# victorramirez952/tomography_3d_reconstructor

Measured on NVIDIA B200. Metric: Gvoxels/s mask-stack->mesh+volume, higher is better.
Workload: dtype u8 -> bit-packed u32 (topology), f64 field taps -> f32 vertices

## Files before the change

tomography_3d_reconstructor_b200/csrc/t3d_common.cuh:

```cuda
#pragma once
#include <cuda_runtime.h>
#include <stdint.h>
#include <stdio.h>

int t3d_num_sms(void);
#define T3D_NUM_SMS (t3d_num_sms())
bool t3d_first_use_on_device(int slot);
enum { T3D_ONCE_FILL_HOLES_ATTR = 0, T3D_ONCE_MC_LUTS = 1, T3D_ONCE_SORT_ATTR = 2, T3D_ONCE_MORPH4_ATTR = 3, T3D_ONCE_SLOTS = 8 };

extern "C" void t3d_set_error(const char* fmt, ...);
extern "C" void t3d_count_launches(int n);
int t3d_zero_async(void* p, size_t n, cudaStream_t st);
void t3d_prezero_register(const void* p, size_t n);
void t3d_prezero_clear(void);
void t3d_canonicalize_structured_zero_range(int64_t V, int64_t F, uint32_t cap_z, uint32_t cap_g0, int Zs, int64_t* offset,
                                            int64_t* size);

#define T3D_CHECK_LAUNCH(name)                                                                   \
    do {                                                                                         \
        cudaError_t e__ = cudaGetLastError();                                                    \
        if (e__ != cudaSuccess) {                                                                \
            t3d_set_error("%s: launch failed: %s", name, cudaGetErrorString(e__));               \
            return 1;                                                                            \
        }                                                                                        \
// ... 53 lines not shown
    return v;
}

__device__ __forceinline__ uint4 ld_stream_u4(const void* p)
{
    uint4 r;
    asm volatile("ld.global.nc.L1::no_allocate.v4.u32 {%0,%1,%2,%3}, [%4];"
                 : "=r"(r.x), "=r"(r.y), "=r"(r.z), "=r"(r.w)
                 : "l"(p));
    return r;
}
__device__ __forceinline__ void st_stream_u4(void* p, uint4 v)
{
    asm volatile("st.global.L1::no_allocate.v4.u32 [%0], {%1,%2,%3,%4};" ::"l"(p), "r"(v.x), "r"(v.y),
                 "r"(v.z), "r"(v.w)
                 : "memory");
}

__device__ __forceinline__ uint32_t ge4(uint32_t v, uint32_t thr4)
{
    const uint32_t m = __vcmpgeu4(v, thr4) & 0x80808080u;
    return (m * 0x00204081u) >> 28;
}
__device__ __forceinline__ uint32_t ge16(uint4 v, uint32_t thr4)
{
    return ge4(v.x, thr4) | (ge4(v.y, thr4) << 4) | (ge4(v.z, thr4) << 8) | (ge4(v.w, thr4) << 12);
}
__device__ __forceinline__ uint32_t expand4(uint32_t nib) { return (nib * 0x00204081u) & 0x01010101u; }

__device__ __forceinline__ uint4 and4(uint4 a, uint4 b) { return make_uint4(a.x & b.x, a.y & b.y, a.z & b.z, a.w & b.w); }
__device__ __forceinline__ uint4 or4(uint4 a, uint4 b) { return make_uint4(a.x | b.x, a.y | b.y, a.z | b.z, a.w | b.w); }
__device__ __forceinline__ uint4 splat4(uint32_t v) { return make_uint4(v, v, v, v); }
__device__ __forceinline__ uint32_t popc4(uint4 a) { return __popc(a.x) + __popc(a.y) + __popc(a.z) + __popc(a.w); }
__device__ __forceinline__ uint4 valid_mask4(int w4, int W)
{
    return make_uint4(valid_mask(4 * w4, W), valid_mask(4 * w4 + 1, W), valid_mask(4 * w4 + 2, W), valid_mask(4 * w4 + 3, W));
}
__device__ __forceinline__ uint4 shl1_4(uint4 c, uint32_t l)
{
    return make_uint4(__funnelshift_l(l, c.x, 1), __funnelshift_l(c.x, c.y, 1), __funnelshift_l(c.y, c.z, 1), __funnelshift_l(c.z, c.w, 1));
}
__device__ __forceinline__ uint4 shr1_4(uint4 c, uint32_t r)
{
    return make_uint4(__funnelshift_r(c.x, c.y, 1), __funnelshift_r(c.y, c.z, 1), __funnelshift_r(c.z, c.w, 1), __funnelshift_r(c.w, r, 1));
}

__device__ __forceinline__ int64_t dev_n(int64_t cap, const unsigned long long* p)
{
    if (!p) return cap;
    const unsigned long long v = *p;
    return v < (unsigned long long)cap ? (int64_t)v : cap;
}

int t3d_morph_stage(const uint32_t* in, uint32_t* out, int Z, int H, int W, int z0, int nz, int out_rs, long long out_ps,
                    bool erode, bool ring, int ring_tail, unsigned long long* counts, cudaStream_t st);
bool t3d_morph4_eligible(int Z, int H, int W);
int t3d_morph4_launch(const uint32_t* in, uint32_t* out, int Z, int H, int W, int z0, int nz, int out_rs, long long out_ps, int ring_tail,
                      unsigned long long* counts, cudaStream_t st);
void t3d_canon_faces_ready_event(cudaEvent_t e);
bool t3d_canon_faces_ready_pending();
bool t3d_pack_gap_supported(const void* masks_u8, int Z, int H, int W, int threshold);
int t3d_pack_gap_launch(const void* masks_u8, int Z, int H, int W, int threshold, void* out, unsigned long long* counts,
                        unsigned int* bbox_t, int skip_ends, cudaStream_t st, int z_bias = 0);
int t3d_bbox_t_planes_launch(const uint32_t* bits, int n_planes, int H, int W, int z_bias, unsigned int* bbox_t, cudaStream_t st);
int t3d_close_ends_fixup_launch(const void* masks_u8, int Z, int H, int W, int threshold, const void* filled0, const void* filledT,
                                void* out, unsigned long long* counts, cudaStream_t st);
```

tomography_3d_reconstructor_b200/csrc/t3d_mc.cu:

```cuda
#include "mc_tables.h"
#include "mc33_tables.h"
#include "t3d.h"
#include "t3d_field.cuh"

__device__ __align__(16) const int8_t g_tri_table[256][T3D_MC_ROW] = {T3D_TRI_TABLE_ROWS};
static const int8_t h_tri_table[256][T3D_MC_ROW] = {T3D_TRI_TABLE_ROWS};

struct McLuts {
    uint8_t ntri[256];
};
#define MC_AMB 0x80u
__constant__ McLuts c_luts;

__device__ const int8_t g33_rows[T3D_MC33_NROWS][T3D_MC33_ROW] = {T3D_MC33_TRI_ROWS};
__device__ const uint8_t g33_ntri[T3D_MC33_NROWS] = {T3D_MC33_NTRI_VALUES};
__device__ const uint16_t g33_base[256] = {T3D_MC33_BASE_VALUES};
__device__ const uint8_t g33_k[256] = {T3D_MC33_K_VALUES};
__device__ const uint8_t g33_faces[256][6] = {T3D_MC33_FACES_VALUES};
__device__ const unsigned long long g33_need[256] = {T3D_MC33_NEED_VALUES};
__device__ const uint8_t g33_pol[256] = {T3D_MC33_POL_VALUES};
__device__ const int8_t g33_sign[256] = {T3D_MC33_SIGN_VALUES};
__device__ const uint8_t g33_cyc[6][4] = {T3D_MC33_FACE_CYCLE_VALUES};
static const uint16_t h33_base[256] = {T3D_MC33_BASE_VALUES};

// ... 112 lines not shown
                                                uint32_t n01, uint32_t n10, uint32_t n11, bool hy, bool hz, int w, int Ws,
                                                bool own = true)
{
    WordMasks m;
    hz = hz && own;
    const uint32_t vm = valid_mask(w, Ws), em = valid_mask(w, Ws - 1);
    m.s00 = s00; m.s01 = s01; m.s10 = s10; m.s11 = s11;
    m.a00 = shr1(s00, n00); m.a01 = shr1(s01, n01); m.a10 = shr1(s10, n10); m.a11 = shr1(s11, n11);
    m.X00 = (s00 ^ m.a00) & em;
    m.X01 = hy ? (s01 ^ m.a01) & em : 0u;
    m.X10 = hz ? (s10 ^ m.a10) & em : 0u;
    m.X11 = (hy && hz) ? (s11 ^ m.a11) & em : 0u;
    m.Y0 = hy ? (s00 ^ s01) & vm : 0u;
    m.Y1 = (hy && hz) ? (s10 ^ s11) & vm : 0u;
    m.Z0 = hz ? (s00 ^ s10) & vm : 0u;
    m.Z1 = (hy && hz) ? (s01 ^ s11) & vm : 0u;
    m.act = 0u;
    if (hy && hz) {
        const uint32_t o = s00 | s01 | s10 | s11, a = s00 & s01 & s10 & s11;
        const uint32_t oa = m.a00 | m.a01 | m.a10 | m.a11, aa = m.a00 & m.a01 & m.a10 & m.a11;
        m.act = ((o | oa) & ~(a & aa)) & em;
    }
    return m;
}

__device__ __forceinline__ int cube_case(const WordMasks& m, int b)
{
    return (int)(((m.s00 >> b) & 1u) | (((m.a00 >> b) & 1u) << 1) | (((m.a01 >> b) & 1u) << 2) | (((m.s01 >> b) & 1u) << 3) |
                 (((m.s10 >> b) & 1u) << 4) | (((m.a10 >> b) & 1u) << 5) | (((m.a11 >> b) & 1u) << 6) | (((m.s11 >> b) & 1u) << 7));
}

__device__ __forceinline__ WordMasks load_masks(const Grid& g, uint32_t row, int w, int& z, int& y)
{
    z = (int)(row / (uint32_t)g.Hs);
    y = (int)(row - (uint32_t)z * (uint32_t)g.Hs);
    const bool hy = (y + 1 < g.Hs), hz = (z + 1 < g.Zs), hx = (w + 1 < g.nws);
    const uint32_t* p = g.sign + (int64_t)row * g.nws + w;
    const int64_t dy = g.nws, dz = (int64_t)g.Hs * g.nws;
    const uint32_t s00 = p[0], s01 = hy ? p[dy] : 0u, s10 = hz ? p[dz] : 0u, s11 = (hy && hz) ? p[dz + dy] : 0u;
    uint32_t n00 = 0, n01 = 0, n10 = 0, n11 = 0;
    if (hx) {
        n00 = p[1] & 1u;
        if (hy) n01 = p[dy + 1] & 1u;
        if (hz) n10 = p[dz + 1] & 1u;
        if (hy && hz) n11 = p[dz + dy + 1] & 1u;
    }
    return make_masks(s00, s01, s10, s11, n00, n01, n10, n11, hy, hz, w, g.Ws, z < g.z_end);
}

#define GY 16

__global__ void __launch_bounds__(256, 4) k_mc_flags(Grid g, uint32_t* __restrict__ ballots, int lanes_x, int pz_per_block, int gy)
{
    const int lx = threadIdx.x % lanes_x, pz = threadIdx.x / lanes_x;
    const int nws4 = g.nws >> 2;
    const int w4 = blockIdx.x * lanes_x + lx, z = g.z_begin + blockIdx.z * pz_per_block + pz, y0 = blockIdx.y * gy;
    if (pz >= pz_per_block || w4 >= nws4 || z >= g.Zs || z > g.z_end) return;
    const bool hz = (z + 1 < g.Zs) && (z < g.z_end);
    const bool hx = (4 * w4 + 4 < g.nws);
    const uint4 vm = valid_mask4(w4, g.Ws), em = valid_mask4(w4, g.Ws - 1);
    const uint4 zero = make_uint4(0, 0, 0, 0);
    const uint32_t* p0 = g.sign + ((long long)z * g.Hs + y0) * g.nws + 4 * w4;
    const uint32_t* p1 = p0 + (long long)g.Hs * g.nws;
    uint32_t* pb = ballots + ((long long)z * g.Hs + y0) * g.ncr + (w4 >> 3);
    const uint32_t bshift = (4 * w4) & 31;
    uint4 c0 = *reinterpret_cast<const uint4*>(p0), c1 = hz ? *reinterpret_cast<const uint4*>(p1) : zero;
    uint32_t n0 = hx ? p0[4] : 0u, n1 = (hx && hz) ? p1[4] : 0u;
    const int y1 = min(g.Hs, y0 + gy);
    auto load_row = [&](int y, uint4& d0, uint4& d1, uint32_t& m0, uint32_t& m1) {
        const bool hy = (y < g.Hs);
        d0 = hy ? *reinterpret_cast<const uint4*>(p0) : zero;
        d1 = (hy && hz) ? *reinterpret_cast<const uint4*>(p1) : zero;
        m0 = (hy && hx) ? p0[4] : 0u;
        m1 = (hy && hz && hx) ? p1[4] : 0u;
    };
    uint4 e0, e1; uint32_t q0, q1;
    p0 += g.nws; p1 += g.nws;
    load_row(y0 + 1, e0, e1, q0, q1);
    for (int y = y0; y < y1; ++y) {
        const bool hy = (y + 1 < g.Hs);
        const uint4 d0 = e0, d1 = e1;
        const uint32_t m0 = q0, m1 = q1;
        p0 += g.nws; p1 += g.nws;
        if (y + 1 < y1) load_row(y + 2, e0, e1, q0, q1);
        uint4 f;
        if (hy && hz) {
            const uint32_t un = (n0 ^ n1) | (n0 ^ m0) | (m0 ^ m1);
            uint4 yz, u;
            yz.x = (c0.x ^ d0.x) | (c0.x ^ c1.x); yz.y = (c0.y ^ d0.y) | (c0.y ^ c1.y);
            yz.z = (c0.z ^ d0.z) | (c0.z ^ c1.z); yz.w = (c0.w ^ d0.w) | (c0.w ^ c1.w);
            u.x = yz.x | (d0.x ^ d1.x); u.y = yz.y | (d0.y ^ d1.y); u.z = yz.z | (d0.z ^ d1.z); u.w = yz.w | (d0.w ^ d1.w);
            const uint4 us = shr1_4(u, un), a0 = shr1_4(c0, n0);
            f.x = ((u.x | us.x | (c0.x ^ a0.x)) & em.x) | (yz.x & vm.x);
            f.y = ((u.y | us.y | (c0.y ^ a0.y)) & em.y) | (yz.y & vm.y);
            f.z = ((u.z | us.z | (c0.z ^ a0.z)) & em.z) | (yz.z & vm.z);
            f.w = ((u.w | us.w | (c0.w ^ a0.w)) & em.w) | (yz.w & vm.w);
        } else {
            const uint4 a0 = shr1_4(c0, n0);
            f.x = ((c0.x ^ a0.x) & em.x); f.y = ((c0.y ^ a0.y) & em.y); f.z = ((c0.z ^ a0.z) & em.z); f.w = ((c0.w ^ a0.w) & em.w);
            if (hy) { f.x |= (c0.x ^ d0.x) & vm.x; f.y |= (c0.y ^ d0.y) & vm.y; f.z |= (c0.z ^ d0.z) & vm.z; f.w |= (c0.w ^ d0.w) & vm.w; }
            if (hz) { f.x |= (c0.x ^ c1.x) & vm.x; f.y |= (c0.y ^ c1.y) & vm.y; f.z |= (c0.z ^ c1.z) & vm.z; f.w |= (c0.w ^ c1.w) & vm.w; }
        }
        const uint32_t nib = (f.x ? 1u : 0u) | (f.y ? 2u : 0u) | (f.z ? 4u : 0u) | (f.w ? 8u : 0u);
        if (nib) atomicOr(pb, nib << bshift);
        pb += g.ncr;
        c0 = d0; c1 = d1; n0 = m0; n1 = m1;
    }
}

__global__ void __launch_bounds__(256) k_mc_compact(Grid g, const uint32_t* __restrict__ ballots,
                                                    const uint32_t* __restrict__ chunkbase, int64_t n_chunks,
                                                    uint32_t* __restrict__ aw_idx, uint32_t cap_active)
{
    const int64_t c = (int64_t)blockIdx.x * blockDim.x + threadIdx.x;
    if (c >= n_chunks) return;
    uint32_t bal = ballots[c];
    if (!bal) return;
    uint32_t k = chunkbase[c];
    const uint32_t row = (uint32_t)(c / g.ncr);
    const uint32_t base = row * (uint32_t)g.nws + (uint32_t)((c - (int64_t)row * g.ncr) << 5);
    while (bal) {
        const int b = __ffs(bal) - 1;
        bal &= bal - 1;
        if (k < cap_active) aw_idx[k] = base + b;
        ++k;
    }
}

#define AW_AMB 0x80000000u
#define AW_MASK 0x7fffffffu

template <int AMB>
__global__ void __launch_bounds__(128) k_mc_words(Grid g, McField fld, uint32_t* __restrict__ aw_idx, uint32_t cap_active,
                                                  const unsigned long long* __restrict__ n_active_dev, uint32_t* __restrict__ aw_cnt,
                                                  unsigned long long* __restrict__ n_ambiguous)
{
    const uint32_t n_active = cap_active;
    const int64_t n = dev_n(cap_active, n_active_dev);
    if (!AMB) {
        const uint32_t k = blockIdx.x * blockDim.x + threadIdx.x;
        if ((int64_t)k >= n) return;
        const uint32_t i = aw_idx[k];
        const uint32_t row = i / (uint32_t)g.nws;
        const int w = (int)(i - row * (uint32_t)g.nws);
        int z, y;
        const WordMasks m = load_masks(g, row, w, z, y);
        uint32_t nt = 0, amb = 0;
        for (uint32_t a = m.act; a;) {
            const int b = __ffs(a) - 1;
            a &= a - 1;
            const uint32_t c = c_luts.ntri[cube_case(m, b)];
            nt += c & 0x7fu;
            amb |= c;
        }
        aw_cnt[k] = __popc(m.X00);
        aw_cnt[(int64_t)n_active + k] = __popc(m.Y0);
        aw_cnt[2 * (int64_t)n_active + k] = __popc(m.Z0);
        aw_cnt[3 * (int64_t)n_active + k] = nt;
        if (amb & MC_AMB) aw_idx[k] = i | AW_AMB;
    } else {
        uint32_t na = 0;
        auto fix_word = [&](int64_t k, uint32_t iraw) {
            const uint32_t i = iraw & AW_MASK;
            const uint32_t row = i / (uint32_t)g.nws;
            const int w = (int)(i - row * (uint32_t)g.nws);
            int z, y;
            const WordMasks m = load_masks(g, row, w, z, y);
            int delta = 0;
            for (uint32_t a = m.act; a;) {
                const int b = __ffs(a) - 1;
                a &= a - 1;
                const int cs = cube_case(m, b);
                const uint32_t c = c_luts.ntri[cs];
                if (!(c & MC_AMB)) continue;
                delta += (int)g33_ntri[mc33_resolve(fld, z, y, (w << 5) + b, cs)] - (int)(c & 0x7fu);
                ++na;
            }
            aw_cnt[3 * (int64_t)n_active + k] += (uint32_t)delta;
        };
        const int64_t n4 = ((uintptr_t)aw_idx & 15) ? 0 : (n >> 2), stride = (int64_t)gridDim.x * blockDim.x, t0 = (int64_t)blockIdx.x * blockDim.x + threadIdx.x;
        for (int64_t c = t0; c < n4; c += stride) {
            const uint4 v = reinterpret_cast<const uint4*>(aw_idx)[c];
            if (!((v.x | v.y | v.z | v.w) & AW_AMB)) continue;
            if (v.x & AW_AMB) fix_word(4 * c, v.x);
            if (v.y & AW_AMB) fix_word(4 * c + 1, v.y);
            if (v.z & AW_AMB) fix_word(4 * c + 2, v.z);
            if (v.w & AW_AMB) fix_word(4 * c + 3, v.w);
        }
        for (int64_t k = 4 * n4 + t0; k < n; k += stride) {
            const uint32_t iraw = aw_idx[k];
            if (iraw & AW_AMB) fix_word(k, iraw);
        }
        if (na) atomicAdd(n_ambiguous, (unsigned long long)na);
    }
}

static unsigned amb_grid(uint32_t n) { const unsigned want = (n + 127) / 128, cap = (unsigned)T3D_NUM_SMS * 8; return want < cap ? (want ? want : 1) : cap; }

struct EmitArgs {
    Grid g;
    McField fld;
    const uint32_t* ballots;
    const uint32_t* chunkbase;
    const uint32_t* aw_idx;
    const uint32_t* aw_base;
    uint32_t cap_active;
    const unsigned long long* sizes;
    uint32_t cap_verts, cap_faces;
    unsigned long long* vkeys;
    int32_t* faces;
};

__device__ __forceinline__ uint32_t active_rank(const EmitArgs& a, uint32_t row, int w)
{
    const int64_t c = (int64_t)row * a.g.ncr + (w >> 5);
    return a.chunkbase[c] + __popc(a.ballots[c] & ((1u << (w & 31)) - 1u));
}

__device__ __forceinline__ uint32_t lt_mask(int b) { return b >= 32 ? 0xffffffffu : ((1u << b) - 1u); }

__device__ __forceinline__ unsigned long long vkey(int axis, int z, int y, int x)
{
    return (unsigned long long)axis | ((unsigned long long)x << 2) | ((unsigned long long)y << 22) | ((unsigned long long)z << 42);
}

template <int PARTS, int AMB>
__global__ void __launch_bounds__(128) k_mc_emit(EmitArgs a)
{
    __shared__ __align__(16) int8_t s_tri[256][T3D_MC_ROW];
    __shared__ uint32_t s_base[12][128];
    __shared__ uint32_t s_mask[12][128];
    __shared__ uint32_t s_next[4][128];
    if (AMB == 1) {
        int any = 0;
        uint32_t nw_ = a.cap_active;
        if (a.sizes[0] < nw_) nw_ = (uint32_t)a.sizes[0];
        for (uint32_t k = blockIdx.x * blockDim.x + threadIdx.x; k < nw_; k += gridDim.x * blockDim.x) any |= (int)(a.aw_idx[k] >> 31);
        if (!__syncthreads_or(any)) return;
    }
    if (PARTS & 2) {
        const int4* src = reinterpret_cast<const int4*>(&g_tri_table[0][0]);
        int4* dst = reinterpret_cast<int4*>(&s_tri[0][0]);
        for (int i = threadIdx.x; i < 256; i += blockDim.x) {
            dst[i] = src[i];
            if (c_luts.ntri[i] & MC_AMB) s_tri[i][T3D_MC_ROW - 1] = -2;
        }
        __syncthreads();
    }
    const uint32_t tid = threadIdx.x;
    uint32_t n_words = a.cap_active;
    if (a.sizes[0] < n_words) n_words = (uint32_t)a.sizes[0];
    const uint32_t offY = (uint32_t)a.sizes[1], offZ = (uint32_t)(a.sizes[1] + a.sizes[2]);
    if (a.sizes[1] + a.sizes[2] + a.sizes[3] > a.cap_verts || a.sizes[4] > a.cap_faces) return;
    auto emit_word = [&](const uint32_t k, const uint32_t iraw) {
    const uint32_t i = iraw & AW_MASK;
    const uint32_t row = i / (uint32_t)a.g.nws;
    const int w = (int)(i - row * (uint32_t)a.g.nws);
    int z, y;
    const WordMasks m = load_masks(a.g, row, w, z, y);
    const int64_t NA = a.cap_active;
    const uint32_t bX00 = a.aw_base[k], bY0 = offY + a.aw_base[NA + k], bZ0 = offZ + a.aw_base[2 * NA + k];
    uint32_t pT = a.aw_base[3 * NA + k];
    const int x0 = w << 5;

    if (PARTS & 1) {
        uint32_t id = bX00;
        for (uint32_t q = m.X00; q;) { const int b = __ffs(q) - 1; q &= q - 1; a.vkeys[id++] = vkey(2, z, y, x0 + b); }
        id = bY0;
        for (uint32_t q = m.Y0; q;) { const int b = __ffs(q) - 1; q &= q - 1; a.vkeys[id++] = vkey(1, z, y, x0 + b); }
        id = bZ0;
        for (uint32_t q = m.Z0; q;) { const int b = __ffs(q) - 1; q &= q - 1; a.vkeys[id++] = vkey(0, z, y, x0 + b); }
    }
    if (!(PARTS & 2) || !m.act) return;
    if (AMB == 0 && (iraw & AW_AMB)) return;

    const uint32_t Hs = (uint32_t)a.g.Hs;
    uint32_t bX01 = 0, bX10 = 0, bX11 = 0, bY1 = 0, bZ1 = 0;
    if (m.X01 | m.Z1) {
        const uint32_t r = active_rank(a, row + 1, w);
        bX01 = a.aw_base[r];
        bZ1 = offZ + a.aw_base[2 * NA + r];
// ... 97 lines not shown
    float* verts;
};

template <int AXIS>
__device__ __forceinline__ void vertex_body(const VertexArgs& p, const ZLut& zlut, uint32_t id)
{
    const unsigned long long key = p.vkeys[id];
    const int x = (int)((key >> 2) & 0xfffffu) - p.x_off, y = (int)((key >> 22) & 0xfffffu), z = (int)(key >> 42);
    float fa, fb;
    if (p.field) {
        const int64_t i = ((int64_t)z * p.occ.H + y) * p.occ.W + x;
        fa = p.field[i];
        fb = p.field[i + (AXIS == 0 ? (int64_t)p.occ.H * p.occ.W : AXIS == 1 ? p.occ.W : 1)];
    } else {
        edge_field_values<AXIS>(p.occ, zlut, z, y, x, fa, fb);
    }
    const double va = (double)fa - p.level, vb = (double)fb - p.level;
    const double wa = __ddiv_rn(1.0, __dadd_rn(MC33_EPS, fabs(va)));
    const double wb = __ddiv_rn(1.0, __dadd_rn(MC33_EPS, fabs(vb)));
    const double frac = __ddiv_rn(wb, __dadd_rn(wa, wb));
    double pz = (double)(z + p.z_offset), py = (double)y, px = (double)x;
    if (AXIS == 0) pz = __dadd_rn(pz, frac); else if (AXIS == 1) py = __dadd_rn(py, frac); else px = __dadd_rn(px, frac);
    float fz = __fsub_rn(__double2float_rn(pz), p.shift);
    float fy = __fsub_rn(__double2float_rn(py), p.shift);
    float fx = __fsub_rn(__double2float_rn(px), p.shift);
    if (p.n_cum > 0) {
        if (fz < 0.0f) fz = 0.0f;
        else if (fz >= (float)(p.n_cum - 1)) fz = __double2float_rn(p.cum[p.n_cum - 1]);
        else {
            const float fl = floorf(fz);
            const int lo = (int)fl;
            const float fr = __fsub_rn(fz, fl);
            const int ai = min(lo, p.n_cum - 2);
            fz = __double2float_rn(__dadd_rn(p.cum[lo], __dmul_rn((double)fr, p.adj[ai])));
        }
    }
    if (p.scale_f64) {
        fy = __double2float_rn(__dmul_rn((double)fy, p.mm_y));
        fx = __double2float_rn(__dmul_rn((double)fx, p.mm_x));
    } else {
        fy = __fmul_rn(fy, __double2float_rn(p.mm_y));
        fx = __fmul_rn(fx, __double2float_rn(p.mm_x));
    }
    float* o = p.verts + 3 * (int64_t)id;
    o[0] = fz; o[1] = fy; o[2] = fx;
}

__global__ void __launch_bounds__(128) k_mc_vertices_all(VertexArgs p, const unsigned long long* __restrict__ sizes, uint32_t cap_verts,
                                                         int which)
{
    __shared__ ZLut zlut;
    fill_zlut(p.occ, zlut);
    __syncthreads();
    const unsigned long long nx = sizes[1], ny = sizes[2], nz = sizes[3];
    if (nx + ny + nz > cap_verts) return;
    uint32_t t = blockIdx.x * blockDim.x + threadIdx.x;
    if (which & 1) {
        if (t < nx) { vertex_body<2>(p, zlut, t); return; }
        t -= (uint32_t)nx;
    }
    if (which & 2) {
        if (t < ny) { vertex_body<1>(p, zlut, (uint32_t)nx + t); return; }
        t -= (uint32_t)ny;
    }
    if ((which & 4) && t < nz) vertex_body<0>(p, zlut, (uint32_t)(nx + ny) + t);
}

static int make_grid(Grid& g, const void* sign_bits, int Zs, int Hs, int Ws, int z_begin, int z_end, const char* who)
{
    if (Zs <= 0 || Hs <= 0 || Ws <= 0) { t3d_set_error("%s: empty volume", who); return 2; }
    if (z_end < 0 || z_end > Zs) z_end = Zs;
    if (z_begin < 0 || z_begin >= z_end) { t3d_set_error("%s: empty plane range", who); return 2; }
    g.z_begin = z_begin; g.z_end = z_end;
    g.sign = (const uint32_t*)sign_bits;
    g.Zs = Zs; g.Hs = Hs; g.Ws = Ws; g.nws = t3d_wpr(Ws);
    g.ncr = (g.nws + 31) >> 5;
    g.n_rows = (uint32_t)((int64_t)Zs * Hs);
    g.n_words = (int64_t)Zs * Hs * g.nws;
    if (g.n_words >= ((int64_t)1 << 31)) { t3d_set_error("%s: more than 2^31 words in one device slab", who); return 2; }
    return 0;
}

extern "C" int64_t t3d_mc_num_chunks(int Zs, int Hs, int Ws) { return (int64_t)Zs * Hs * ((t3d_wpr(Ws) + 31) >> 5); }

extern "C" int t3d_mc_flags(const void* sign_bits, int Zs, int Hs, int Ws, int z_begin, int z_end, void* ballots_u32,
                            void* stream)
{
    Grid g;
    if (int rc = make_grid(g, sign_bits, Zs, Hs, Ws, z_begin, z_end, "t3d_mc_flags")) return rc;
    cudaStream_t st = (cudaStream_t)stream;
    if (t3d_zero_async(ballots_u32, sizeof(uint32_t) * (size_t)g.n_rows * g.ncr, st)) return 1;
    const int nws4 = g.nws / 4, lanes_x = nws4 < 256 ? nws4 : 256, pzb = 256 / lanes_x;
    const int nz = (g.z_end < Zs ? g.z_end + 1 : Zs) - g.z_begin;
    dim3 grid((nws4 + lanes_x - 1) / lanes_x, (Hs + GY - 1) / GY, (nz + pzb - 1) / pzb);
    k_mc_flags<<<grid, 256, 0, st>>>(g, (uint32_t*)ballots_u32, lanes_x, pzb, GY);
    T3D_CHECK_LAUNCH("t3d_mc_flags");
    t3d_count_launches(1);
    return 0;
}

static int mc_words_dev_impl(const McField& fld, const void* sign_bits, int Zs, int Hs, int Ws, int z_begin, int z_end,
                             const void* ballots_u32, const void* chunkbase_u32, uint32_t cap_active, const void* sizes_u64,
                             void* aw_idx_u32, void* aw_cnt_u32, void* n_ambiguous_u64, void* stream)
{
    Grid g;
    if (int rc = make_grid(g, sign_bits, Zs, Hs, Ws, z_begin, z_end, "t3d_mc_words_dev")) return rc;
    if (ensure_luts()) return 1;
    cudaStream_t st = (cudaStream_t)stream;
    if (t3d_zero_async(n_ambiguous_u64, 8, st)) return 1;
    if (cap_active == 0) return 0;
    const int64_t n_chunks = (int64_t)g.n_rows * g.ncr;
    k_mc_compact<<<(unsigned)((n_chunks + 255) / 256), 256, 0, st>>>(g, (const uint32_t*)ballots_u32, (const uint32_t*)chunkbase_u32,
                                                                      n_chunks, (uint32_t*)aw_idx_u32, cap_active);
    k_mc_words<0><<<(cap_active + 127) / 128, 128, 0, st>>>(g, fld, (uint32_t*)aw_idx_u32, cap_active, (const unsigned long long*)sizes_u64,
                                                            (uint32_t*)aw_cnt_u32, (unsigned long long*)n_ambiguous_u64);
    k_mc_words<1><<<amb_grid(cap_active), 128, 0, st>>>(g, fld, (uint32_t*)aw_idx_u32, cap_active, (const unsigned long long*)sizes_u64,
                                                            (uint32_t*)aw_cnt_u32, (unsigned long long*)n_ambiguous_u64);
    T3D_CHECK_LAUNCH("t3d_mc_words_dev");
    t3d_count_launches(3);
    return 0;
}

extern "C" int t3d_mc_words_dev(const void* sign_bits, int Zs, int Hs, int Ws, int z_begin, int z_end, const void* ballots_u32,
                                const void* chunkbase_u32, uint32_t cap_active, const void* sizes_u64, void* aw_idx_u32,
                                void* aw_cnt_u32, void* n_ambiguous_u64, const t3d_mc_field* mc_field, void* stream)
{
    return mc_words_dev_impl(mc_field_from_abi(mc_field), sign_bits, Zs, Hs, Ws, z_begin, z_end, ballots_u32, chunkbase_u32, cap_active,
                             sizes_u64, aw_idx_u32, aw_cnt_u32, n_ambiguous_u64, stream);
}

static int mc_emit_dev_impl(const McField& fld, const void* sign_bits, int Zs, int Hs, int Ws, int z_begin, int z_end,
                            const void* ballots_u32, const void* chunkbase_u32, const void* aw_idx_u32, const void* aw_base_u32,
                            uint32_t cap_active, const void* sizes_u64, uint32_t cap_verts, uint32_t cap_faces, void* vkeys_u64,
                            void* faces_i32, int parts, void* stream)
{
    EmitArgs a;
    if (int rc = make_grid(a.g, sign_bits, Zs, Hs, Ws, z_begin, z_end, "t3d_mc_emit_dev")) return rc;
    if (ensure_luts()) return 1;
    if (cap_active == 0) return 0;
    a.fld = fld;
    a.ballots = (const uint32_t*)ballots_u32;
    a.chunkbase = (const uint32_t*)chunkbase_u32;
    a.aw_idx = (const uint32_t*)aw_idx_u32;
    a.aw_base = (const uint32_t*)aw_base_u32;
    a.cap_active = cap_active;
    a.sizes = (const unsigned long long*)sizes_u64;
    a.cap_verts = cap_verts;
    a.cap_faces = cap_faces;
    a.vkeys = (unsigned long long*)vkeys_u64;
    a.faces = (int32_t*)faces_i32;
    const unsigned ge = (cap_active + 127) / 128;
    int launches = 1;
    if ((parts & 3) == 1) k_mc_emit<1, 0><<<ge, 128, 0, (cudaStream_t)stream>>>(a);
    else if ((parts & 3) == 2) {
        k_mc_emit<2, 0><<<ge, 128, 0, (cudaStream_t)stream>>>(a);
        k_mc_emit<2, 1><<<amb_grid(cap_active), 128, 0, (cudaStream_t)stream>>>(a);
        launches = 2;
    } else k_mc_emit<3, 2><<<ge, 128, 0, (cudaStream_t)stream>>>(a);
    T3D_CHECK_LAUNCH("t3d_mc_emit_dev");
    t3d_count_launches(launches);
    return 0;
}

extern "C" int t3d_mc_emit_dev(const void* sign_bits, int Zs, int Hs, int Ws, int z_begin, int z_end, const void* ballots_u32,
                               const void* chunkbase_u32, const void* aw_idx_u32, const void* aw_base_u32, uint32_t cap_active,
                               const void* sizes_u64, uint32_t cap_verts, uint32_t cap_faces, void* vkeys_u64, void* faces_i32,
                               int parts, const t3d_mc_field* mc_field, void* stream)
{
    return mc_emit_dev_impl(mc_field_from_abi(mc_field), sign_bits, Zs, Hs, Ws, z_begin, z_end, ballots_u32, chunkbase_u32, aw_idx_u32,
                            aw_base_u32, cap_active, sizes_u64, cap_verts, cap_faces, vkeys_u64, faces_i32, parts, stream);
}

int t3d_mc_words_view_dev(const OccView& view, int x_off, const void* sign_bits, int Zs, int Hs, int Ws, int z_begin, int z_end,
                          const void* ballots_u32, const void* chunkbase_u32, uint32_t cap_active, const void* sizes_u64,
                          void* aw_idx_u32, void* aw_cnt_u32, void* n_ambiguous_u64, void* stream)
{
    McField f;
    f.occ = view; f.field = nullptr; f.level = 0.5; f.x_off = x_off; f.mode = 1;
    return mc_words_dev_impl(f, sign_bits, Zs, Hs, Ws, z_begin, z_end, ballots_u32, chunkbase_u32, cap_active, sizes_u64, aw_idx_u32,
                             aw_cnt_u32, n_ambiguous_u64, stream);
}

int t3d_mc_emit_view_dev(const OccView& view, int x_off, const void* sign_bits, int Zs, int Hs, int Ws, int z_begin, int z_end,
                         const void* ballots_u32, const void* chunkbase_u32, const void* aw_idx_u32, const void* aw_base_u32,
                         uint32_t cap_active, const void* sizes_u64, uint32_t cap_verts, uint32_t cap_faces, void* vkeys_u64,
                         void* faces_i32, int parts, void* stream)
{
    McField f;
    f.occ = view; f.field = nullptr; f.level = 0.5; f.x_off = x_off; f.mode = 1;
    return mc_emit_dev_impl(f, sign_bits, Zs, Hs, Ws, z_begin, z_end, ballots_u32, chunkbase_u32, aw_idx_u32, aw_base_u32, cap_active,
                            sizes_u64, cap_verts, cap_faces, vkeys_u64, faces_i32, parts, stream);
}

static int mc_vertices_impl(const OccView& view, const float* field, double level, int x_off, const void* vkeys_u64, const void* sizes_u64,
                            uint32_t cap_verts, int unpad_shift, int z_offset, const void* cum_f64, const void* adj_f64, int n_cum,
                            double mm_per_pixel_y, double mm_per_pixel_x, int scale_in_f64, int which_blocks, void* verts_f32, void* stream)
{
    if ((which_blocks & 7) == 0) return 0;
    if (cap_verts == 0) return 0;
    VertexArgs p;
    p.occ = view;
    p.vkeys = (const unsigned long long*)vkeys_u64;
    p.field = field;
    p.level = level;
    p.x_off = x_off;
    p.shift = unpad_shift ? 1.0f : 0.0f;
    p.z_offset = z_offset;
    p.cum = (const double*)cum_f64;
    p.adj = (const double*)adj_f64;
    p.n_cum = n_cum;
    p.mm_y = mm_per_pixel_y;
    p.mm_x = mm_per_pixel_x;
    p.scale_f64 = scale_in_f64 ? 1 : 0;
    p.verts = (float*)verts_f32;
    k_mc_vertices_all<<<(cap_verts + 127) / 128, 128, 0, (cudaStream_t)stream>>>(p, (const unsigned long long*)sizes_u64, cap_verts,
                                                                               which_blocks & 7);
    T3D_CHECK_LAUNCH("t3d_mc_vertices_dev");
    t3d_count_launches(1);
    return 0;
}

int t3d_mc_vertices_view_dev(const OccView& view, int x_off, const void* vkeys_u64, const void* sizes_u64, uint32_t cap_verts,
                             int unpad_shift, int z_offset, const void* cum_f64, const void* adj_f64, int n_cum, double mm_per_pixel_y,
                             double mm_per_pixel_x, int scale_in_f64, int which_blocks, void* verts_f32, void* stream)
{
    return mc_vertices_impl(view, nullptr, 0.5, x_off, vkeys_u64, sizes_u64, cap_verts, unpad_shift, z_offset, cum_f64, adj_f64, n_cum,
                            mm_per_pixel_y, mm_per_pixel_x, scale_in_f64, which_blocks, verts_f32, stream);
}

extern "C" int t3d_mc_vertices_dev(const void* occ_bits, int Z, int H, int W, int pad, int gaussian, const double* weights3_host,
                                   const void* field_f32, double level, const void* vkeys_u64, const void* sizes_u64, uint32_t cap_verts,
                                   int unpad_shift, int z_offset, const void* cum_f64, const void* adj_f64, int n_cum,
                                   double mm_per_pixel_y, double mm_per_pixel_x, int scale_in_f64, int which_blocks, void* verts_f32,
                                   void* stream)
{
    if (Z <= 0 || H <= 0 || W <= 0) { t3d_set_error("t3d_mc_vertices_dev: empty volume"); return 2; }
    if (!field_f32 && !gaussian && pad) { t3d_set_error("t3d_mc_vertices_dev: pad requires gaussian"); return 2; }
    const OccView view = field_f32 ? t3d_make_view(nullptr, Z, H, W, 0, 0, nullptr)
                                   : t3d_make_view(occ_bits, Z, H, W, pad, gaussian, weights3_host);
    return mc_vertices_impl(view, (const float*)field_f32, field_f32 ? level : 0.5, 0, vkeys_u64, sizes_u64, cap_verts, unpad_shift,
                            z_offset, cum_f64, adj_f64, n_cum, mm_per_pixel_y, mm_per_pixel_x, scale_in_f64, which_blocks, verts_f32,
                            stream);
}

__global__ void __launch_bounds__(256) k_sign_from_f32(const float* __restrict__ field, int64_t n_rows, int W, int nw, double level,
                                                       uint32_t* __restrict__ bits)
{
    const int64_t i = (int64_t)blockIdx.x * blockDim.x + threadIdx.x;
    if (i >= n_rows * nw) return;
    const int64_t row = i / nw;
    const int w = (int)(i - row * nw);
    const float* p = field + row * W + (w << 5);
    const int n = min(32, W - (w << 5));
    uint32_t v = 0;
    for (int k = 0; k < n; ++k) v |= (uint32_t)(((double)p[k] - level) > 0.0) << k;
    bits[i] = v;
}

extern "C" int t3d_sign_from_f32(const void* field_f32, int Z, int H, int W, double level, void* sign_bits, void* stream)
{
    if (Z <= 0 || H <= 0 || W <= 0) { t3d_set_error("t3d_sign_from_f32: empty volume"); return 2; }
    const int nw = t3d_wpr(W);
    const int64_t rows = (int64_t)Z * H, n = rows * nw;
    k_sign_from_f32<<<(unsigned)((n + 255) / 256), 256, 0, (cudaStream_t)stream>>>((const float*)field_f32, rows, W, nw, level,
                                                                                 (uint32_t*)sign_bits);
    T3D_CHECK_LAUNCH("t3d_sign_from_f32");
    t3d_count_launches(1);
    return 0;
}
// ... 1 lines not shown
```

tomography_3d_reconstructor_b200/csrc/t3d_pipeline.cu:

```cuda
#include <stdint.h>

#include <stdlib.h>

#include <nvtx3/nvToolsExt.h>

#include "t3d.h"
#include "t3d_field.cuh"

struct NvtxRange {
    bool open;
    explicit NvtxRange(const char* name) : open(true) { nvtxRangePushA(name); }
    void end() { if (open) { nvtxRangePop(); open = false; } }
    ~NvtxRange() { end(); }
};

enum {
    R_NACTIVE = 0, R_NX = 1, R_NY = 2, R_NZ = 3, R_NT = 4, R_VCANON = 5, R_FCANON = 6, R_UNVERIFIED = 7, R_OVERFLOW = 8,
    R_NAMBIGUOUS = 9, R_NEXACT = 10, R_VOLUME_F64 = 11, R_AREA_F64 = 12, R_BBOX_I32X6 = 13 , R_VRAW = 16, R_NEXC = 17,
    R_NGHOST = 18, R_NLEAD = 19, R_NG0 = 25,
    R_COUNTS = 32
};

#define EXC_CAP (1u << 20)
#define SURF_HALO 3
// ... 21 lines not shown
    const int64_t nwp = t3d_words_per_row(Wp), n_chunks = t3d_mc_num_chunks(Zp, Hp, Wp);
    int64_t o = 0;
    L.bitsA = o; o += own_bitsA ? al(vol) : 0;
    L.bitsB = o; o += al(vol);
    L.bitsC = o; o += fast ? 0 : al(vol);
    L.morph = o; o += al(t3d_morph_scratch_bytes(Zx, H, W, n_stages));
    L.fill = o; o += al(t3d_fill_holes_scratch_bytes(2, H, W));
    L.sign = o; o += al((int64_t)Zp * Hp * nwp * 4);
    L.exc = o; o += al((int64_t)EXC_CAP * 8);
    L.ballots = o; o += al(n_chunks * 4);
    L.chunkbase = o; o += al(n_chunks * 4);
    L.scan1 = o; o += al(t3d_scan_workspace_bytes(n_chunks, 1));
    L.aw_idx = o; o += al((int64_t)capNA * 4);
    L.aw_cnt = o; o += al((int64_t)capNA * 16);
    L.aw_base = o; o += al((int64_t)capNA * 16);
    L.scan2 = o; o += al(t3d_scan_workspace_bytes(capNA, 4));
    L.vkeys = o; o += al((int64_t)capV * 8);
    L.verts_raw = o; o += al((int64_t)capV * 12);
    L.faces_raw = o; o += al((int64_t)capF * 12);
    L.canon = o; o += al(capZ ? t3d_canonicalize_structured_workspace_bytes(capV, capF, capZ, capG0, Zp)
                              : t3d_canonicalize_fast_workspace_bytes(capV, capF));
    L.measure = o; o += al(t3d_mesh_measure_workspace_bytes());
    L.total = o;
    return L;
}

extern "C" int64_t t3d_reconstruct_workspace_bytes(int Z, int H, int W, int add_padding, int n_stages, uint32_t cap_active,
                                                   uint32_t cap_verts, uint32_t cap_faces, uint32_t cap_zverts, uint32_t cap_g0)
{
    const int pad = add_padding ? 1 : 0;
    const int64_t a = make_layout(Z, Z, H, W, pad, cap_active, cap_verts, cap_faces, cap_zverts, cap_g0, n_stages, true, false).total;
    const int64_t b = make_layout(Z, Z, H, W, pad, cap_active, cap_verts, cap_faces, cap_zverts, cap_g0, n_stages, true, true).total;
    return a > b ? a : b;
}

extern "C" int64_t t3d_reconstruct_results_len(int Z) { return R_COUNTS + 2 * (int64_t)Z; }

static inline int imin(int a, int b) { return a < b ? a : b; }

extern "C" int64_t t3d_reconstruct_slab_workspace_bytes(int halo_lo, int n_own, int halo_hi, int H, int W, int add_padding,
                                                        int n_stages, uint32_t cap_active, uint32_t cap_verts, uint32_t cap_faces,
                                                        uint32_t cap_zverts, uint32_t cap_g0)
{
    const int Zx = halo_lo + n_own + halo_hi, Zl = imin(SURF_HALO, halo_lo) + n_own + imin(SURF_HALO, halo_hi);
    const int pad = add_padding ? 1 : 0;
    const int64_t a = make_layout(Zx, Zl, H, W, pad, cap_active, cap_verts, cap_faces, cap_zverts, cap_g0, n_stages, false, false).total;
    const int64_t b = make_layout(Zx, Zl, H, W, pad, cap_active, cap_verts, cap_faces, cap_zverts, cap_g0, n_stages, false, true).total;
    return a > b ? a : b;
}

__global__ void k_finalize_sizes(unsigned long long* r, unsigned long long capNA, unsigned long long capV, unsigned long long capF,
                                 int bbox_transformed)
{
    if (bbox_transformed) {
        unsigned int* t = (unsigned int*)(r + R_BBOX_I32X6);
        int* b = (int*)(r + R_BBOX_I32X6);
        for (int k = 0; k < 3; ++k) {
            const unsigned lo = t[2 * k], hi = t[2 * k + 1];
            b[2 * k] = 0x7fffffff - (int)lo;
            b[2 * k + 1] = (int)hi - 1;
        }
    }
    unsigned long long of8 = (r[R_NEXC] > EXC_CAP) ? 8ull : 0ull;
    const unsigned long long v = r[R_NX] + r[R_NY] + r[R_NZ];
    r[R_VRAW] = v;
    unsigned long long of = 0;
    if (r[R_NACTIVE] > capNA) of |= 1;
    if (v > capV) of |= 2;
    if (r[R_NT] > capF) of |= 4;
    r[R_OVERFLOW] = of | of8;
    if (of | of8) {
        for (int k = 0; k < 5; ++k) { r[20 + k] = r[R_NACTIVE + k]; r[R_NACTIVE + k] = 0; }
        r[R_VRAW] = 0;
    }
}

__global__ void k_count_plane_vertices(const float* __restrict__ verts, const unsigned long long* n_dev, float z_ghost, float z_lead,
                                       int want_ghost, int want_lead, unsigned long long* out_ghost, unsigned long long* out_lead)
{
    const int w = threadIdx.x >> 5, lane = threadIdx.x & 31;
    const bool want = w == 0 ? want_ghost != 0 : want_lead != 0;
    unsigned long long* out = w == 0 ? out_ghost : out_lead;
    if (!want) {
        if (lane == 0) *out = 0;
        return;
    }
    const float zq = w == 0 ? z_ghost : z_lead;
    const long long n = (long long)*n_dev;
    long long bound[2];
    for (int upper = 0; upper < 2; ++upper) {
        long long lo = 0, hi = n;
        while (hi - lo > 0) {
            const long long span = hi - lo, step = (span + 31) / 32;
            const long long i = lo + (long long)lane * step;
            bool before = false;
            if (i < hi) {
                const float z = verts[3 * i];
                before = upper ? (z <= zq) : (z < zq);
            }
            const unsigned b = __ballot_sync(0xffffffffu, before);
            const int k = __popc(b);
            if (k == 0) { hi = lo; break; }
            const long long last_before = lo + (long long)(k - 1) * step;
            const long long nlo = last_before + 1;
            const long long nhi = (k < 32 && lo + (long long)k * step < hi) ? lo + (long long)k * step : hi;
            lo = nlo; hi = nhi;
        }
        bound[upper] = lo;
    }
    if (lane == 0) *out = (unsigned long long)(bound[1] - bound[0]);
}

#define N_SIDE_EVENTS 8
struct SideStream {
    cudaStream_t s = nullptr;
    cudaEvent_t e[N_SIDE_EVENTS] = {};
};
static SideStream g_side[64];

static int side_for_current_device(SideStream** out)
{
    int dev = 0;
    T3D_CUDA(cudaGetDevice(&dev));
    SideStream& s = g_side[dev & 63];
    if (!s.s) {
        int prio_lo = 0, prio_hi = 0;
        T3D_CUDA(cudaDeviceGetStreamPriorityRange(&prio_lo, &prio_hi));
        T3D_CUDA(cudaStreamCreateWithPriority(&s.s, cudaStreamNonBlocking, prio_hi));
        for (int k = 0; k < N_SIDE_EVENTS; ++k) T3D_CUDA(cudaEventCreateWithFlags(&s.e[k], cudaEventDisableTiming));
    }
    *out = &s;
    return 0;
}

#define RUN(call) do { if (int rc__ = (call)) return rc__; } while (0)

struct ZeroSet {
    uint4* p[6];
    unsigned long long n16[6];
    int n;
};
__global__ void __launch_bounds__(256) k_zero_ranges(ZeroSet z)
{
    for (int k = 0; k < z.n; ++k)
        for (unsigned long long i = (unsigned long long)blockIdx.x * blockDim.x + threadIdx.x; i < z.n16[k];
             i += (unsigned long long)gridDim.x * blockDim.x)
            z.p[k][i] = make_uint4(0, 0, 0, 0);
}
struct PrezeroGuard {
    PrezeroGuard() { t3d_prezero_clear(); }
    ~PrezeroGuard() { t3d_prezero_clear(); }
    ZeroSet z{};
    void add(void* p, size_t bytes)
    {
        const size_t n16 = bytes / 16;
        if (!n16 || z.n >= 6 || ((uintptr_t)p & 15)) return;
        z.p[z.n] = (uint4*)p; z.n16[z.n] = n16; ++z.n;
        t3d_prezero_register(p, n16 * 16);
    }
    int launch(cudaStream_t st)
    {
        if (!z.n) return 0;
        k_zero_ranges<<<T3D_NUM_SMS * 2, 256, 0, st>>>(z);
        T3D_CHECK_LAUNCH("k_zero_ranges");
        t3d_count_launches(1);
        return 0;
    }
};

struct SlabGeom {
    int hl, n, hh;
    int z_begin, z_end;
    int z_offset;
    int want_ghost, want_lead;
    float z_ghost, z_lead;
};

__global__ void __launch_bounds__(256) k_zero_ring(uint4* __restrict__ S, int Zs, int Hs, int nws4)
{
    const long long plane4 = (long long)Hs * nws4;
    const long long nA = 2 * plane4, nB = (long long)(Zs - 2) * 2 * nws4;
    const uint4 zero = make_uint4(0, 0, 0, 0);
    for (long long i = (long long)blockIdx.x * blockDim.x + threadIdx.x; i < nA + nB; i += (long long)gridDim.x * blockDim.x) {
        if (i < nA) {
            S[i < plane4 ? i : (long long)(Zs - 1) * plane4 + (i - plane4)] = zero;
        } else {
            const long long j = i - nA;
            const long long z = 1 + j / (2 * nws4);
            const int r = (int)(j % (2 * nws4));
            S[z * plane4 + (long long)(r < nws4 ? 0 : Hs - 1) * nws4 + (r % nws4)] = zero;
        }
    }
}

struct StageMarks {
    enum { N = 12 };
    cudaEvent_t ev[N];
    const char* name[N];
    int n = 0;
    bool on = false;
    void begin(cudaStream_t st)
    {
        static const bool want = getenv("T3D_STAGE_EVENTS") != nullptr;
        on = false;
        if (!want) return;
        cudaStreamCaptureStatus cs = cudaStreamCaptureStatusNone;
        if (cudaStreamIsCapturing(st, &cs) != cudaSuccess || cs != cudaStreamCaptureStatusNone) return;
        on = true; n = 0;
    }
    void mark(const char* what, cudaStream_t st)
    {
        if (!on || n >= N) return;
        static thread_local cudaEvent_t pool[N] = {};
        if (!pool[n]) cudaEventCreate(&pool[n]);
        ev[n] = pool[n]; name[n] = what;
        cudaEventRecord(ev[n], st);
        ++n;
    }
    void report(cudaStream_t st)
    {
        if (!on) return;
        cudaStreamSynchronize(st);
        fprintf(stderr, "[t3d stages]");
        for (int i = 1; i < n; ++i) { float ms = 0; cudaEventElapsedTime(&ms, ev[i - 1], ev[i]); fprintf(stderr, " %s %.1f us |", name[i], 1e3f * ms); }
        float tot = 0; if (n > 1) cudaEventElapsedTime(&tot, ev[0], ev[n - 1]);
        fprintf(stderr, " total %.1f us\n", 1e3f * tot);
    }
};

static int reconstruct_core(const uint32_t* grid, const SlabGeom& g, int H, int W, int n_stages, unsigned erode_mask, int pad,
                            const double* weights3_host, const void* cum_f64, const void* adj_f64, int n_cum, double mm_y,
                            double mm_x, int scale_in_f64, uint32_t cap_active, uint32_t cap_verts, uint32_t cap_faces,
                            uint32_t cap_zverts, uint32_t cap_g0, int zkey_bits, void* verts_out_f32, void* faces_out_i64,
                            unsigned long long* R, char* ws, const Layout& L, bool fast, int bbox_state, SideStream* side, cudaStream_t st)
{
    const int Zx = g.hl + g.n + g.hh;
    const int64_t nw = t3d_words_per_row(W), plane_words = (int64_t)H * nw, vol_words = (int64_t)Zx * plane_words;
    const int sl = imin(SURF_HALO, g.hl), sh = imin(SURF_HALO, g.hh), Zl = sl + g.n + sh;
    const int Zp = Zl + 2 * pad, Hp = H + 2 * pad, Wp = fast ? W + S_XPAD + 1 : W + 2 * pad;
    const int64_t n_chunks = t3d_mc_num_chunks(Zp, Hp, Wp);

    NvtxRange r_smooth("t3d:smooth_voxel_data");
    StageMarks marks;
    marks.begin(st);
    marks.mark("start", st);
    (void)t3d_canon_faces_ready_pending();
    T3D_CUDA(cudaEventRecord(side->e[2], st));
    T3D_CUDA(cudaStreamWaitEvent(side->s, side->e[2], 0));
    if (bbox_state == 0)
        RUN(t3d_volume_stats(grid + (int64_t)g.hl * plane_words, g.n, H, W, nullptr, R + R_BBOX_I32X6, side->s));
    OccView view;
    int x_off = 0;
    if (fast) {
        const int nws = (int)t3d_words_per_row(Wp);
        uint32_t* S = (uint32_t*)(ws + L.sign);
        const long long s_ps = (long long)Hp * nws;
        {
            const long long items = 2 * (long long)Hp * (nws / 4) + (long long)(Zp - 2) * 2 * (nws / 4);
            long long blocks = (items + 255) / 256;
            if (blocks > (long long)T3D_NUM_SMS * 8) blocks = (long long)T3D_NUM_SMS * 8;
            k_zero_ring<<<(unsigned)(blocks < 1 ? 1 : blocks), 256, 0, side->s>>>((uint4*)S, Zp, Hp, nws / 4);
            t3d_count_launches(1);
        }
        T3D_CUDA(cudaEventRecord(side->e[3], side->s));
        uint32_t* tA = (uint32_t*)(ws + L.morph);
        uint32_t* tB = tA + vol_words;
        uint32_t* S_origin = S + s_ps + nws + S_XPAD / 32;
        const int z0 = g.hl - sl;
        const int ring_tail = (nws - (int)nw - S_XPAD / 32) / 4;
        if (t3d_morph4_eligible(Zx, H, W)) {
            RUN(t3d_morph4_launch(grid, S_origin, Zx, H, W, z0, Zl, nws, s_ps, ring_tail, R + R_COUNTS + Zx + z0, st));
        } else {
            RUN(t3d_morph_stage(grid, tA, Zx, H, W, 0, Zx, (int)nw, plane_words, true, false, 0, nullptr, st));
            RUN(t3d_morph_stage(tA, tB, Zx, H, W, 0, Zx, (int)nw, plane_words, false, false, 0, nullptr, st));
            RUN(t3d_morph_stage(tB, tA, Zx, H, W, 0, Zx, (int)nw, plane_words, false, false, 0, nullptr, st));
            RUN(t3d_morph_stage(tA, S_origin, Zx, H, W, z0, Zl, nws, s_ps, true, true, ring_tail, R + R_COUNTS + Zx + z0, st));
        }
        view = t3d_make_view_strided(S_origin, Zl, H, W, nws, s_ps, 1, 1, weights3_host);
        x_off = S_XPAD - 1;
        T3D_CUDA(cudaStreamWaitEvent(st, side->e[3], 0));
    } else {
        T3D_CUDA(cudaEventRecord(side->e[3], side->s));
        uint32_t* bitsC = (uint32_t*)(ws + L.bitsC);
        const uint32_t* smoothed = grid;
        if (n_stages > 0) {
            RUN(t3d_morph(grid, bitsC, Zx, H, W, n_stages, erode_mask, R + R_COUNTS + Zx, ws + L.morph, st));
            smoothed = bitsC;
        } else {
            T3D_CUDA(cudaMemcpyAsync(R + R_COUNTS + Zx, R + R_COUNTS, sizeof(unsigned long long) * Zx, cudaMemcpyDeviceToDevice, st));
        }
        const uint32_t* surf = smoothed + (int64_t)(g.hl - sl) * plane_words;
        RUN(t3d_field_sign_lean(surf, Zl, H, W, pad, weights3_host, ws + L.sign, R + R_NEXACT, ws + L.exc, EXC_CAP, R + R_NEXC, st));
        view = t3d_make_view(surf, Zl, H, W, pad, 1, weights3_host);
    }

    r_smooth.end();
    marks.mark("smooth", st);
    NvtxRange r_mc("t3d:extract_manifold_surface");
    RUN(t3d_mc_flags(ws + L.sign, Zp, Hp, Wp, g.z_begin, g.z_end, ws + L.ballots, st));
    marks.mark("flags", st);
    RUN(t3d_exclusive_scan_u32_dev(ws + L.ballots, ws + L.chunkbase, n_chunks, n_chunks, 1, 0, 1, nullptr, R + R_NACTIVE,
                                   ws + L.scan1, st));
    RUN(t3d_mc_words_view_dev(view, x_off, ws + L.sign, Zp, Hp, Wp, g.z_begin, g.z_end, ws + L.ballots, ws + L.chunkbase, cap_active,
                              R + R_NACTIVE, ws + L.aw_idx, ws + L.aw_cnt, R + R_NAMBIGUOUS, st));
    RUN(t3d_exclusive_scan_u32_dev(ws + L.aw_cnt, ws + L.aw_base, cap_active, cap_active, 4, 0, 0, R + R_NACTIVE, R + R_NX,
                                   ws + L.scan2, st));
    k_finalize_sizes<<<1, 1, 0, st>>>(R, cap_active, cap_verts, cap_faces, bbox_state == 2 ? 1 : 0);
    t3d_count_launches(1);
    marks.mark("scan+words+scan", st);
    RUN(t3d_mc_emit_view_dev(view, x_off, ws + L.sign, Zp, Hp, Wp, g.z_begin, g.z_end, ws + L.ballots, ws + L.chunkbase, ws + L.aw_idx,
                             ws + L.aw_base, cap_active, R + R_NACTIVE, cap_verts, cap_faces, ws + L.vkeys, ws + L.faces_raw, 1, st));
    marks.mark("keys", st);
    RUN(t3d_mc_vertices_view_dev(view, x_off, ws + L.vkeys, R + R_NACTIVE, cap_verts, 1, g.z_offset, cum_f64, adj_f64, n_cum, mm_y, mm_x,
                                 scale_in_f64, 7, ws + L.verts_raw, st));
    r_mc.end();
    marks.mark("vertices", st);
    NvtxRange r_canon("t3d:ensure_manifold_mesh+measures");
    T3D_CUDA(cudaEventRecord(side->e[4], st));
    T3D_CUDA(cudaStreamWaitEvent(side->s, side->e[4], 0));
    RUN(t3d_mc_emit_view_dev(view, x_off, ws + L.sign, Zp, Hp, Wp, g.z_begin, g.z_end, ws + L.ballots, ws + L.chunkbase, ws + L.aw_idx,
                             ws + L.aw_base, cap_active, R + R_NACTIVE, cap_verts, cap_faces, ws + L.vkeys, ws + L.faces_raw, 2, side->s));
    T3D_CUDA(cudaEventRecord(side->e[6], side->s));
    RUN(t3d_mesh_measure_dev(ws + L.verts_raw, ws + L.faces_raw, cap_faces, R + R_NT, 0, R + R_VOLUME_F64, ws + L.measure, side->s));
    T3D_CUDA(cudaEventRecord(side->e[5], side->s));
    t3d_canon_faces_ready_event(side->e[6]);
    if (cap_zverts)
        RUN(t3d_mesh_canonicalize_structured_dev(ws + L.verts_raw, ws + L.vkeys, cap_verts, R + R_NACTIVE, R + R_VRAW, Zp, Hp, Wp,
                                                 ws + L.chunkbase, ws + L.aw_base, cap_active, g.z_offset, 1, cum_f64, adj_f64, n_cum,
                                                 zkey_bits, cap_zverts, cap_g0, ws + L.faces_raw, cap_faces, R + R_NT, verts_out_f32,
                                                 faces_out_i64, nullptr, R + R_VCANON, R + R_NG0, ws + L.canon, 3, st));
    else
        RUN(t3d_mesh_canonicalize_fast_dev(ws + L.verts_raw, cap_verts, R + R_VRAW, ws + L.faces_raw, cap_faces, R + R_NT,
                                           verts_out_f32, faces_out_i64, nullptr, R + R_VCANON, ws + L.canon, st));
    if (t3d_canon_faces_ready_pending()) T3D_CUDA(cudaStreamWaitEvent(st, side->e[6], 0));
    if (g.want_ghost || g.want_lead)
        k_count_plane_vertices<<<1, 64, 0, st>>>((const float*)verts_out_f32, R + R_VCANON, g.z_ghost, g.z_lead, g.want_ghost,
                                                 g.want_lead, R + R_NGHOST, R + R_NLEAD);
    if (g.want_ghost || g.want_lead) t3d_count_launches(1);
    marks.mark("canonicalize", st);
    T3D_CUDA(cudaStreamWaitEvent(st, side->e[5], 0));
    marks.mark("wait measures", st);
    marks.report(st);
    return 0;
}

extern "C" int t3d_reconstruct(const void* masks_u8, int Z, int H, int W, int threshold, int close_ends, int n_stages,
                               unsigned erode_mask, int add_padding, const double* weights3_host, const void* cum_f64,
                               const void* adj_f64, int n_cum, double mm_per_pixel_y, double mm_per_pixel_x, int scale_in_f64,
                               uint32_t cap_active, uint32_t cap_verts, uint32_t cap_faces, uint32_t cap_zverts, uint32_t cap_g0,
                               int zkey_bits, void* verts_out_f32, void* faces_out_i64, void* results_u64, void* workspace,
                               void* stream)
{
    if (Z <= 0 || H <= 0 || W <= 0) { t3d_set_error("t3d_reconstruct: empty volume"); return 2; }
    if (cap_active == 0 || cap_verts == 0 || cap_faces == 0) { t3d_set_error("t3d_reconstruct: zero capacity"); return 2; }
    cudaStream_t st = (cudaStream_t)stream;
    const int pad = add_padding ? 1 : 0;
    const bool fast = fast_surface(n_stages, erode_mask, pad, Z, H, W);
    const Layout L = make_layout(Z, Z, H, W, pad, cap_active, cap_verts, cap_faces, cap_zverts, cap_g0, n_stages, true, fast);
    char* ws = (char*)workspace;
    unsigned long long* R = (unsigned long long*)results_u64;
    const int64_t nw = t3d_words_per_row(W), plane_words = (int64_t)H * nw, plane_bytes = (int64_t)H * W;
    uint32_t* bitsA = (uint32_t*)(ws + L.bitsA);
    uint32_t* bitsB = (uint32_t*)(ws + L.bitsB);
    const uint8_t* m = (const uint8_t*)masks_u8;
    SideStream* side;
    RUN(side_for_current_device(&side));
    PrezeroGuard zg;
    {
        const int Zp = Z + 2 * pad, Hp = H + 2 * pad, Wp = fast ? W + S_XPAD + 1 : W + 2 * pad;
        const int64_t n_chunks = t3d_mc_num_chunks(Zp, Hp, Wp);
        zg.add(R, sizeof(unsigned long long) * (R_COUNTS + 2 * (size_t)Z));
        zg.add(ws + L.ballots, (size_t)al(n_chunks * 4));
        zg.add(ws + L.scan1, (size_t)al(t3d_scan_workspace_bytes(n_chunks, 1)));
        zg.add(ws + L.scan2, (size_t)al(t3d_scan_workspace_bytes(cap_active, 4)));
        if (cap_zverts) {
            int64_t off = 0, size = 0;
            t3d_canonicalize_structured_zero_range(cap_verts, cap_faces, cap_zverts, cap_g0, Zp, &off, &size);
            zg.add(ws + L.canon + off, (size_t)size);
        }
        RUN(zg.launch(st));
    }

    int bbox_state = 0;
    NvtxRange r_create("t3d:create_voxel_data");
    if (close_ends && t3d_pack_gap_supported(m, Z, H, W, threshold)) {
        uint32_t* f0 = bitsA;
        uint32_t* fT = bitsA + plane_words;
        RUN(t3d_pack_masks(m, 1, H, W, threshold, f0, st));
        RUN(t3d_pack_masks(m + (int64_t)(Z - 1) * plane_bytes, 1, H, W, threshold, fT, st));
        T3D_CUDA(cudaEventRecord(side->e[0], st));
// ... 230 lines not shown
```

tomography_3d_reconstructor_b200/csrc/t3d_surface.cu:

```cuda
#include <stdlib.h>

#include <cub/device/device_radix_sort.cuh>

#include "t3d_field.cuh"

#define FY 8

__device__ __noinline__ uint32_t exact_sign_bits(const OccView* v, int zp, int yp, int wp, uint32_t need, uint32_t s)
{
    while (need) {
        const int b = __ffs(need) - 1;
        need &= need - 1;
        if (field_value(*v, zp, yp, (wp << 5) + b) > 0.5f) s |= 1u << b; else s &= ~(1u << b);
    }
    return s;
}

__device__ __forceinline__ uint4 prow4(const OccView& v, int zp, int yp, int wp4, uint32_t& left, uint32_t& right)
{
    const int z = zp - v.pad, y = yp - v.pad;
    if (z < 0 || z >= v.Z || y < 0 || y >= v.H) { left = right = 0u; return make_uint4(0, 0, 0, 0); }
    const uint32_t* row = v.bits + (z * v.ps + (long long)y * v.rs);
    const int w0 = 4 * wp4;
    const uint4 o = (w0 < v.nw) ? *reinterpret_cast<const uint4*>(row + w0) : make_uint4(0, 0, 0, 0);
// ... 62 lines not shown
                        const unsigned long long k = atomicAdd(exc_count, 1ull);
                        if (k < exc_cap) exc[k] = ((flat + j) << 32) | nd[j];
                    }
                }
            } else {
                if (need.x) s.x = exact_sign_bits(&sv, zp, yp, 4 * wp4, need.x, s.x);
                if (need.y) s.y = exact_sign_bits(&sv, zp, yp, 4 * wp4 + 1, need.y, s.y);
                if (need.z) s.z = exact_sign_bits(&sv, zp, yp, 4 * wp4 + 2, need.z, s.z);
                if (need.w) s.w = exact_sign_bits(&sv, zp, yp, 4 * wp4 + 3, need.w, s.w);
            }
        }
        *reinterpret_cast<uint4*>(sign + ((int64_t)zp * v.Hp + yp) * nwp + 4 * wp4) = and4(s, vm);
        prev = cur;
        cur = next; lc = ln; rc = rn;
    }
}

__global__ void __launch_bounds__(128) k_field_sign_fix(OccView v, uint32_t* __restrict__ sign, int nwp,
                                                        const unsigned long long* __restrict__ exc, unsigned long long exc_cap,
                                                        const unsigned long long* __restrict__ exc_count)
{
    const unsigned long long n = min(*exc_count, exc_cap);
    for (unsigned long long i = (unsigned long long)blockIdx.x * blockDim.x + threadIdx.x; i < n; i += (unsigned long long)gridDim.x * blockDim.x) {
        const unsigned long long e = exc[i];
        const unsigned long long flat = e >> 32;
        uint32_t need = (uint32_t)e;
        const int wp = (int)(flat % nwp);
        const unsigned long long row = flat / nwp;
        const int yp = (int)(row % v.Hp), zp = (int)(row / v.Hp);
        uint32_t s = sign[flat];
        while (need) {
            const int b = __ffs(need) - 1;
            need &= need - 1;
            if (field_value(v, zp, yp, (wp << 5) + b) > 0.5f) s |= 1u << b; else s &= ~(1u << b);
        }
        sign[flat] = s;
    }
}

#define SC_THREADS 256
#define SC_ITEMS 8
#define SC_TILE (SC_THREADS * SC_ITEMS)
#define SC_FLAG_A (1ull << 62)
#define SC_FLAG_P (2ull << 62)
#define SC_VALUE_MASK ((1ull << 62) - 1)

template <typename OutT>
__global__ void __launch_bounds__(SC_THREADS) k_scan_lookback(const uint32_t* __restrict__ in, OutT* __restrict__ out, int64_t n_cap,
                                                              int64_t stride, unsigned long long* __restrict__ desc, int n_tiles,
                                                              unsigned int* __restrict__ tickets, int popc_in,
                                                              const unsigned long long* __restrict__ n_dev,
                                                              unsigned long long* __restrict__ totals)
{
    const int64_t n = dev_n(n_cap, n_dev);
    const uint32_t* a = in + (int64_t)blockIdx.y * stride;
    OutT* o = out + (int64_t)blockIdx.y * stride;
    volatile unsigned long long* d = desc + (int64_t)blockIdx.y * n_tiles;
    __shared__ int s_tile;
    __shared__ uint32_t sh[SC_THREADS / 32];
    __shared__ unsigned long long s_prefix;
    if (threadIdx.x == 0) s_tile = (int)atomicAdd(tickets + blockIdx.y, 1u);
    __syncthreads();
    const int tile = s_tile;
    const int64_t need = (n + SC_TILE - 1) / SC_TILE;
    n_tiles = (int)(need < 1 ? 1 : (need < n_tiles ? need : n_tiles));
    if (tile >= n_tiles) return;
    const int64_t base = (int64_t)tile * SC_TILE + (int64_t)threadIdx.x * SC_ITEMS;
    uint32_t v[SC_ITEMS];
    uint32_t sum = 0;
#pragma unroll
    for (int k = 0; k < SC_ITEMS; ++k) {
        v[k] = (base + k < n) ? (popc_in ? (uint32_t)__popc(a[base + k]) : a[base + k]) : 0u;
        sum += v[k];
    }
    const uint32_t incl = warp_incl_scan(sum);
    if (lane_id() == 31) sh[threadIdx.x >> 5] = incl;
    __syncthreads();
    uint32_t woff = 0, agg = 0;
#pragma unroll
    for (int k = 0; k < SC_THREADS / 32; ++k) {
        if (k < (int)(threadIdx.x >> 5)) woff += sh[k];
        agg += sh[k];
    }
    if (threadIdx.x < 32) {
        unsigned long long prefix = 0;
        if (tile == 0) {
            if (threadIdx.x == 0) { d[0] = SC_FLAG_P | (unsigned long long)agg; }
        } else {
            if (threadIdx.x == 0) { d[tile] = SC_FLAG_A | (unsigned long long)agg; }
            int idx = tile - 1 - (int)threadIdx.x;
            while (true) {
                unsigned long long w = (idx >= 0) ? d[idx] : SC_FLAG_P;
                while (__any_sync(0xffffffffu, (w >> 62) == 0)) {
                    if ((w >> 62) == 0) w = (idx >= 0) ? d[idx] : SC_FLAG_P;
                }
                const uint32_t is_p = __ballot_sync(0xffffffffu, (w >> 62) == 2);
                const int first_p = is_p ? (__ffs(is_p) - 1) : 32;
                unsigned long long val = ((int)threadIdx.x <= first_p) ? (w & SC_VALUE_MASK) : 0ull;
#pragma unroll
                for (int off = 16; off > 0; off >>= 1) val += __shfl_xor_sync(0xffffffffu, val, off);
                prefix += val;
                if (is_p) break;
                idx -= 32;
            }
            if (threadIdx.x == 0) { d[tile] = SC_FLAG_P | ((prefix + agg) & SC_VALUE_MASK); }
        }
        if (threadIdx.x == 0) {
            s_prefix = prefix;
            if (tile == n_tiles - 1) totals[blockIdx.y] = prefix + agg;
        }
    }
    __syncthreads();
    unsigned long long run = s_prefix + woff + (incl - sum);
#pragma unroll
    for (int k = 0; k < SC_ITEMS; ++k) {
        if (base + k < n) o[base + k] = (OutT)run;
        run += v[k];
    }
}

extern "C" int64_t t3d_scan_workspace_bytes(int64_t n, int n_arrays)
{
    const int64_t nb = (n + SC_THREADS * 4 - 1) / (SC_THREADS * 4);
    return (nb * n_arrays + 16) * 8 + 256;
}

extern "C" int t3d_exclusive_scan_u32_dev(const void* in, void* out, int64_t n_cap, int64_t stride, int n_arrays, int out_is_u64,
                                          int popcount_input, const void* n_dev_u64, void* totals_u64, void* workspace, void* stream)
{
    cudaStream_t st = (cudaStream_t)stream;
    if (n_cap <= 0 || n_arrays <= 0) {
        if (n_arrays > 0) T3D_CUDA(cudaMemsetAsync(totals_u64, 0, 8 * n_arrays, st));
        return 0;
    }
    if (n_arrays > 16) { t3d_set_error("t3d_exclusive_scan_u32_dev: at most 16 arrays per call"); return 2; }
    const int64_t nb = (n_cap + SC_TILE - 1) / SC_TILE;
    if (nb > 0x7fffffff) { t3d_set_error("t3d_exclusive_scan_u32_dev: too many elements"); return 2; }
    const size_t desc_bytes = (size_t)nb * n_arrays * 8;
    if (t3d_zero_async(workspace, desc_bytes + 64, st)) return 1;
    unsigned long long* desc = (unsigned long long*)workspace;
    unsigned int* tickets = (unsigned int*)((char*)workspace + desc_bytes);
    const unsigned long long* nd = (const unsigned long long*)n_dev_u64;
    dim3 grid((unsigned)nb, n_arrays);
    if (out_is_u64)
        k_scan_lookback<unsigned long long><<<grid, SC_THREADS, 0, st>>>((const uint32_t*)in, (unsigned long long*)out, n_cap, stride, desc,
                                                                         (int)nb, tickets, popcount_input, nd,
                                                                         (unsigned long long*)totals_u64);
    else
        k_scan_lookback<uint32_t><<<grid, SC_THREADS, 0, st>>>((const uint32_t*)in, (uint32_t*)out, n_cap, stride, desc, (int)nb, tickets,
                                                               popcount_input, nd, (unsigned long long*)totals_u64);
    T3D_CHECK_LAUNCH("t3d_exclusive_scan_u32_dev");
    t3d_count_launches(1);
    return 0;
}

extern "C" int t3d_field_sign(const void* occ_bits, int Z, int H, int W, int pad, const double* weights3, void* sign_bits,
                              void* n_exact_u64, void* stream)
{
    if (Z <= 0 || H <= 0 || W <= 0) { t3d_set_error("t3d_field_sign: empty volume"); return 2; }
    cudaStream_t st = (cudaStream_t)stream;
    const OccView v = t3d_make_view(occ_bits, Z, H, W, pad, 1, weights3);
    const int nwp = t3d_wpr(v.Wp);
    T3D_CUDA(cudaMemsetAsync(n_exact_u64, 0, 8, st));
    const int nwp4 = nwp / 4, lanes_x = nwp4 < 256 ? nwp4 : 256, pzb = 256 / lanes_x;
    dim3 grid((nwp4 + lanes_x - 1) / lanes_x, (v.Hp + FY - 1) / FY, (v.Zp + pzb - 1) / pzb);
    k_field_sign<false><<<grid, 256, 0, st>>>(v, (uint32_t*)sign_bits, nwp, lanes_x, pzb, FY, (unsigned long long*)n_exact_u64, nullptr, 0,
                                              nullptr);
    T3D_CHECK_LAUNCH("t3d_field_sign");
    t3d_count_launches(1);
    return 0;
}

extern "C" int t3d_field_sign_lean(const void* occ_bits, int Z, int H, int W, int pad, const double* weights3, void* sign_bits,
                                   void* n_exact_u64, void* exc_list_u64, uint32_t exc_cap, void* exc_count_u64, void* stream)
{
    if (Z <= 0 || H <= 0 || W <= 0) { t3d_set_error("t3d_field_sign_lean: empty volume"); return 2; }
    cudaStream_t st = (cudaStream_t)stream;
    const OccView v = t3d_make_view(occ_bits, Z, H, W, pad, 1, weights3);
    const int nwp = t3d_wpr(v.Wp);
    if (t3d_zero_async(n_exact_u64, 8, st) || t3d_zero_async(exc_count_u64, 8, st)) return 1;
    const int nwp4 = nwp / 4, lanes_x = nwp4 < 256 ? nwp4 : 256, pzb = 256 / lanes_x;
    dim3 grid((nwp4 + lanes_x - 1) / lanes_x, (v.Hp + FY - 1) / FY, (v.Zp + pzb - 1) / pzb);
    k_field_sign<true><<<grid, 256, 0, st>>>(v, (uint32_t*)sign_bits, nwp, lanes_x, pzb, FY, (unsigned long long*)n_exact_u64,
                                             (unsigned long long*)exc_list_u64, exc_cap, (unsigned long long*)exc_count_u64);
    k_field_sign_fix<<<T3D_NUM_SMS, 128, 0, st>>>(v, (uint32_t*)sign_bits, nwp, (const unsigned long long*)exc_list_u64, exc_cap,
                                                  (const unsigned long long*)exc_count_u64);
    T3D_CHECK_LAUNCH("t3d_field_sign_lean");
    t3d_count_launches(2);
    return 0;
}

__global__ void __launch_bounds__(256) k_field_dense(OccView v, float* __restrict__ out)
{
    const int64_t i = (int64_t)blockIdx.x * blockDim.x + threadIdx.x;
    const int64_t total = (int64_t)v.Zp * v.Hp * v.Wp;
    if (i >= total) return;
    const int x = (int)(i % v.Wp);
    const int64_t r = i / v.Wp;
    out[i] = field_value(v, (int)(r / v.Hp), (int)(r % v.Hp), x);
}

extern "C" int t3d_field_dense(const void* occ_bits, int Z, int H, int W, int pad, int gaussian, const double* weights3,
                               void* out_f32, void* stream)
// ... 47 lines not shown
{
    const int64_t i = (int64_t)blockIdx.x * blockDim.x + threadIdx.x;
    if (i >= V) return;
    const uint32_t src = perm ? perm[i] : (uint32_t)i;
    keys[i] = float_key(verts[3 * (int64_t)src + col]);
    if (iota) iota[i] = (uint32_t)i;
}

__global__ void __launch_bounds__(256) k_unique_heads(const float* __restrict__ verts, const uint32_t* __restrict__ perm, int64_t V,
                                                      uint32_t* __restrict__ head)
{
    const int64_t i = (int64_t)blockIdx.x * blockDim.x + threadIdx.x;
    if (i >= V) return;
    uint32_t h = 1;
    if (i > 0) {
        const float* a = verts + 3 * (int64_t)perm[i];
        const float* b = verts + 3 * (int64_t)perm[i - 1];
        h = (float_key(a[0]) != float_key(b[0]) || float_key(a[1]) != float_key(b[1]) || float_key(a[2]) != float_key(b[2])) ? 1u : 0u;
    }
    head[i] = h;
}

__global__ void __launch_bounds__(256) k_scatter_unique(const float* __restrict__ verts, const uint32_t* __restrict__ perm,
                                                        const uint32_t* __restrict__ head, const uint32_t* __restrict__ pos,
                                                        int64_t V_cap, float* __restrict__ out_verts, uint32_t* __restrict__ newid,
                                                        const unsigned long long* __restrict__ V_dev = nullptr)
{
    const int64_t i = (int64_t)blockIdx.x * blockDim.x + threadIdx.x;
    if (i >= dev_n(V_cap, V_dev)) return;
    const uint32_t u = pos[i] + head[i] - 1u;
    const uint32_t src = perm[i];
    newid[src] = u;
    if (head[i]) {
        const float* a = verts + 3 * (int64_t)src;
        float* o = out_verts + 3 * (int64_t)u;
        o[0] = a[0]; o[1] = a[1]; o[2] = a[2];
    }
}

__global__ void __launch_bounds__(256) k_face_valid(const int32_t* __restrict__ faces, int64_t F_cap, const uint32_t* __restrict__ newid,
                                                    uint32_t* __restrict__ valid, const unsigned long long* __restrict__ F_dev = nullptr)
{
    const int64_t i = (int64_t)blockIdx.x * blockDim.x + threadIdx.x;
    if (i >= dev_n(F_cap, F_dev)) return;
    const uint32_t a = newid[faces[3 * i]], b = newid[faces[3 * i + 1]], c = newid[faces[3 * i + 2]];
    valid[i] = (a != b && b != c && a != c) ? 1u : 0u;
}

__global__ void __launch_bounds__(256) k_face_compact(const int32_t* __restrict__ faces, int64_t F_cap, const uint32_t* __restrict__ newid,
                                                      const uint32_t* __restrict__ valid, const uint32_t* __restrict__ pos,
                                                      long long* __restrict__ out64, int32_t* __restrict__ out32,
                                                      const unsigned long long* __restrict__ F_dev = nullptr)
{
    const int64_t F = dev_n(F_cap, F_dev);
    for (int64_t i = (int64_t)blockIdx.x * blockDim.x + threadIdx.x; i < F; i += (int64_t)gridDim.x * blockDim.x) {
        if (!valid[i]) continue;
        const uint32_t a = newid[faces[3 * i]], b = newid[faces[3 * i + 1]], c = newid[faces[3 * i + 2]];
        const int64_t o = 3 * (int64_t)pos[i];
        if (out64) { out64[o] = a; out64[o + 1] = b; out64[o + 2] = c; }
        if (out32) { out32[o] = (int32_t)a; out32[o + 1] = (int32_t)b; out32[o + 2] = (int32_t)c; }
    }
}

__global__ void __launch_bounds__(256) k_face_remap(const int32_t* __restrict__ faces, int64_t F_cap, const uint32_t* __restrict__ newid,
                                                    uint32_t* __restrict__ valid, long long* __restrict__ out64, int32_t* __restrict__ out32,
                                                    unsigned long long* __restrict__ n_invalid, const unsigned long long* __restrict__ F_dev)
{
    const int64_t i = (int64_t)blockIdx.x * blockDim.x + threadIdx.x;
    const int64_t F = dev_n(F_cap, F_dev);
    bool bad = false;
    if (i < F) {
        const uint32_t a = newid[faces[3 * i]], b = newid[faces[3 * i + 1]], c = newid[faces[3 * i + 2]];
        bad = !(a != b && b != c && a != c);
        valid[i] = bad ? 0u : 1u;
        if (out64) { out64[3 * i] = a; out64[3 * i + 1] = b; out64[3 * i + 2] = c; }
        if (out32) { out32[3 * i] = (int32_t)a; out32[3 * i + 1] = (int32_t)b; out32[3 * i + 2] = (int32_t)c; }
    }
    const uint32_t nb = __popc(__ballot_sync(0xffffffffu, bad));
    if (lane_id() == 0 && nb) atomicAdd(n_invalid, (unsigned long long)nb);
}

__global__ void k_face_plan(const unsigned long long* __restrict__ n_invalid, int64_t F_cap, const unsigned long long* __restrict__ F_dev,
                            unsigned long long* __restrict__ n_to_compact, unsigned long long* __restrict__ f_out)
{
    const unsigned long long F = (unsigned long long)dev_n(F_cap, F_dev);
    *n_to_compact = (*n_invalid) ? F : 0ull;
    *f_out = F - *n_invalid;
}

static size_t sort_temp_bytes(int64_t V)
{
    size_t bytes = 0;
    cub::DeviceRadixSort::SortPairs(nullptr, bytes, (const uint32_t*)nullptr, (uint32_t*)nullptr, (const uint32_t*)nullptr,
                                    (uint32_t*)nullptr, (int)V);
    return bytes;
}

static inline int64_t align256(int64_t x) { return (x + 255) & ~(int64_t)255; }

extern "C" int64_t t3d_canonicalize_workspace_bytes(int64_t V, int64_t F)
{
    const int64_t n = V > F ? V : F;
    int64_t b = 0;
    b += 4 * align256(4 * V);
    b += 2 * align256(4 * n);
    b += align256(4 * V);
    b += align256((int64_t)sort_temp_bytes(V > 0 ? V : 1));
    b += align256(t3d_scan_workspace_bytes(n, 1));
    b += 256;
    return b;
}

extern "C" int t3d_mesh_canonicalize(const void* verts_in, int64_t V, const void* faces_in, int64_t F, void* verts_out,
                                     void* faces_out_i64, void* faces_out_i32, void* counts_u64, void* workspace, void* stream)
{
    cudaStream_t st = (cudaStream_t)stream;
    if (V <= 0 || V > 0x7fffffff || F < 0) { t3d_set_error("t3d_mesh_canonicalize: bad sizes"); return 2; }
    const int64_t n = V > F ? V : F;
    char* ws = (char*)workspace;
    uint32_t* keys_a = (uint32_t*)ws; ws += align256(4 * V);
    uint32_t* keys_b = (uint32_t*)ws; ws += align256(4 * V);
    uint32_t* perm_a = (uint32_t*)ws; ws += align256(4 * V);
    uint32_t* perm_b = (uint32_t*)ws; ws += align256(4 * V);
    uint32_t* flags = (uint32_t*)ws; ws += align256(4 * n);
    uint32_t* pos = (uint32_t*)ws; ws += align256(4 * n);
    uint32_t* newid = (uint32_t*)ws; ws += align256(4 * V);
    size_t temp_bytes = sort_temp_bytes(V);
    void* temp = ws; ws += align256((int64_t)temp_bytes);
    void* scan_ws = ws; ws += align256(t3d_scan_workspace_bytes(n, 1));
    unsigned long long* totals = (unsigned long long*)ws;
    unsigned long long* counts = (unsigned long long*)counts_u64;
    const unsigned gv = (unsigned)((V + 255) / 256);
    const float* vin = (const float*)verts_in;

    uint32_t *pin = nullptr, *pout = perm_a, *pspare = perm_b;
    for (int pass = 0; pass < 3; ++pass) {
        const int col = 2 - pass;
        k_make_keys<<<gv, 256, 0, st>>>(vin, V, col, pin, keys_a, pass == 0 ? pspare : nullptr);
        const uint32_t* vals_in = (pass == 0) ? pspare : pin;
        T3D_CUDA(cub::DeviceRadixSort::SortPairs(temp, temp_bytes, (const uint32_t*)keys_a, keys_b, vals_in, pout, (int)V, 0, 32, st));
        uint32_t* old_in = pin;
        pin = pout;
        pout = (pass == 0) ? pspare : old_in;
        if (pass == 0) pspare = nullptr;
    }
    const uint32_t* perm = pin;
    k_unique_heads<<<gv, 256, 0, st>>>(vin, perm, V, flags);
    if (t3d_exclusive_scan_u32_dev(flags, pos, V, V, 1, 0, 0, nullptr, totals, scan_ws, stream)) return 1;
    T3D_CUDA(cudaMemcpyAsync(counts, totals, 8, cudaMemcpyDeviceToDevice, st));
    k_scatter_unique<<<gv, 256, 0, st>>>(vin, perm, flags, pos, V, (float*)verts_out, newid);
    if (F > 0) {
        const unsigned gf = (unsigned)((F + 255) / 256);
        k_face_valid<<<gf, 256, 0, st>>>((const int32_t*)faces_in, F, newid, flags);
        if (t3d_exclusive_scan_u32_dev(flags, pos, F, F, 1, 0, 0, nullptr, totals, scan_ws, stream)) return 1;
        T3D_CUDA(cudaMemcpyAsync(counts + 1, totals, 8, cudaMemcpyDeviceToDevice, st));
        k_face_compact<<<gf, 256, 0, st>>>((const int32_t*)faces_in, F, newid, flags, pos, (long long*)faces_out_i64,
                                           (int32_t*)faces_out_i32);
    } else {
        T3D_CUDA(cudaMemsetAsync(counts + 1, 0, 8, st));
    }
    T3D_CHECK_LAUNCH("t3d_mesh_canonicalize");
    t3d_count_launches(F > 0 ? 7 : 5);
    return 0;
}

__global__ void __launch_bounds__(256) k_make_keys64(const float* __restrict__ verts, int64_t V_cap, const unsigned long long* __restrict__ V_dev,
                                                     unsigned long long* __restrict__ keys, uint32_t* __restrict__ iota)
{
    const int64_t i = (int64_t)blockIdx.x * blockDim.x + threadIdx.x;
    if (i >= V_cap) return;
    keys[i] = (i < dev_n(V_cap, V_dev)) ? (((unsigned long long)float_key(verts[3 * i]) << 32) | float_key(verts[3 * i + 1]))
                                        : 0xffffffffffffffffull;
    iota[i] = (uint32_t)i;
}

__global__ void __launch_bounds__(256) k_heads_checked(const float* __restrict__ verts, const uint32_t* __restrict__ perm, int64_t V_cap,
                                                       const unsigned long long* __restrict__ V_dev, uint32_t* __restrict__ head,
                                                       unsigned long long* __restrict__ bad)
{
    const int64_t i = (int64_t)blockIdx.x * blockDim.x + threadIdx.x;
    if (i >= dev_n(V_cap, V_dev)) return;
    uint32_t h = 1;
    if (i > 0) {
        const float* a = verts + 3 * (int64_t)perm[i];
        const float* b = verts + 3 * (int64_t)perm[i - 1];
        const uint32_t az = float_key(a[0]), ay = float_key(a[1]), ax = float_key(a[2]);
        const uint32_t bz = float_key(b[0]), by = float_key(b[1]), bx = float_key(b[2]);
        h = (az != bz || ay != by || ax != bx) ? 1u : 0u;
        const bool lt = (az < bz) || (az == bz && (ay < by || (ay == by && ax < bx)));
        if (lt) atomicOr(bad, 1ull);
    }
    head[i] = h;
}

static size_t sort64_temp_bytes(int64_t V)
{
    size_t bytes = 0;
    cub::DeviceRadixSort::SortPairs(nullptr, bytes, (const unsigned long long*)nullptr, (unsigned long long*)nullptr,
                                    (const uint32_t*)nullptr, (uint32_t*)nullptr, (int)V);
    return bytes;
}

extern "C" int64_t t3d_canonicalize_fast_workspace_bytes(int64_t V, int64_t F)
{
    const int64_t n = V > F ? V : F;
    int64_t b = 0;
    b += 2 * align256(8 * V);
    b += 2 * align256(4 * V);
    b += 2 * align256(4 * n);
    b += align256(4 * V);
    b += align256((int64_t)sort64_temp_bytes(V > 0 ? V : 1));
    b += align256(t3d_scan_workspace_bytes(n, 1));
    b += 256;
    return b;
}

#define UQ_ITEMS 4
#define UQ_TILE (SC_THREADS * UQ_ITEMS)
__global__ void __launch_bounds__(SC_THREADS) k_unique_fused(const float* __restrict__ verts, const uint32_t* __restrict__ perm, int64_t V_cap,
                                                             const unsigned long long* __restrict__ V_dev, float* __restrict__ out_verts,
                                                             uint32_t* __restrict__ newid, unsigned long long* __restrict__ desc, int n_tiles,
                                                             unsigned int* __restrict__ ticket, unsigned long long* __restrict__ bad,
                                                             unsigned long long* __restrict__ n_unique_out,
                                                             const unsigned long long* __restrict__ skip_unless)
{
    if (skip_unless && *skip_unless == 0) return;
    const int64_t n = dev_n(V_cap, V_dev);
    volatile unsigned long long* d = desc;
    __shared__ int s_tile;
    __shared__ uint32_t s_kz[UQ_TILE + 1], s_ky[UQ_TILE + 1], s_kx[UQ_TILE + 1];
    __shared__ uint32_t s_part[UQ_ITEMS * (SC_THREADS / 32)];
    __shared__ unsigned long long s_prefix;
    if (threadIdx.x == 0) s_tile = (int)atomicAdd(ticket, 1u);
    __syncthreads();
    const int tile = s_tile;
    const int64_t need = (n + UQ_TILE - 1) / UQ_TILE;
    n_tiles = (int)(need < 1 ? 1 : (need < n_tiles ? need : n_tiles));
    if (tile >= n_tiles) return;
    const int64_t base = (int64_t)tile * UQ_TILE;
    const int tid = threadIdx.x, lane = tid & 31, warp = tid >> 5;
    uint32_t src[UQ_ITEMS];
    float vz[UQ_ITEMS], vy[UQ_ITEMS], vx[UQ_ITEMS];
#pragma unroll
    for (int k = 0; k < UQ_ITEMS; ++k) {
        const int e = k * SC_THREADS + tid;
        if (base + e < n) {
            src[k] = perm[base + e];
            const float* a = verts + 3 * (int64_t)src[k];
            vz[k] = a[0]; vy[k] = a[1]; vx[k] = a[2];
            s_kz[e + 1] = float_key(vz[k]); s_ky[e + 1] = float_key(vy[k]); s_kx[e + 1] = float_key(vx[k]);
        }
    }
    if (tid == 0 && base > 0) {
        const float* b = verts + 3 * (int64_t)perm[base - 1];
        s_kz[0] = float_key(b[0]); s_ky[0] = float_key(b[1]); s_kx[0] = float_key(b[2]);
    }
    __syncthreads();
    uint32_t ball[UQ_ITEMS];
    uint32_t myhead = 0;
    bool out_of_order = false;
#pragma unroll
    for (int k = 0; k < UQ_ITEMS; ++k) {
        const int e = k * SC_THREADS + tid;
        bool h = false;
        if (base + e < n) {
            h = true;
            if (base + e > 0) {
                const uint32_t az = s_kz[e + 1], ay = s_ky[e + 1], ax = s_kx[e + 1], pz = s_kz[e], py = s_ky[e], px = s_kx[e];
                h = (az != pz || ay != py || ax != px);
                out_of_order |= (az < pz) || (az == pz && (ay < py || (ay == py && ax < px)));
            }
        }
        ball[k] = __ballot_sync(0xffffffffu, h);
        myhead |= (h ? 1u : 0u) << k;
        if (lane == 0) s_part[k * (SC_THREADS / 32) + warp] = __popc(ball[k]);
    }
    if (out_of_order) atomicOr(bad, 1ull);
    __syncthreads();
// ... 8 lines not shown
        uint32_t runp = incl - psum;
#pragma unroll
        for (int t = 0; t < PER_LANE; ++t) { s_part[PER_LANE * lane + t] = runp; runp += pv[t]; }
        unsigned long long prefix = 0;
        if (tile == 0) {
            if (tid == 0) { d[0] = SC_FLAG_P | (unsigned long long)agg; }
        } else {
            if (tid == 0) { d[tile] = SC_FLAG_A | (unsigned long long)agg; }
            int idx = tile - 1 - tid;
            while (true) {
                unsigned long long w = (idx >= 0) ? d[idx] : SC_FLAG_P;
                while (__any_sync(0xffffffffu, (w >> 62) == 0)) {
                    if ((w >> 62) == 0) w = (idx >= 0) ? d[idx] : SC_FLAG_P;
                }
                const uint32_t is_p = __ballot_sync(0xffffffffu, (w >> 62) == 2);
                const int first_p = is_p ? (__ffs(is_p) - 1) : 32;
                unsigned long long val = (tid <= first_p) ? (w & SC_VALUE_MASK) : 0ull;
#pragma unroll
                for (int off = 16; off > 0; off >>= 1) val += __shfl_xor_sync(0xffffffffu, val, off);
                prefix += val;
                if (is_p) break;
                idx -= 32;
            }
            if (tid == 0) { d[tile] = SC_FLAG_P | ((prefix + agg) & SC_VALUE_MASK); }
        }
        if (tid == 0) {
            s_prefix = prefix;
            if (tile == n_tiles - 1) *n_unique_out = prefix + agg;
        }
    }
    __syncthreads();
    const uint32_t tile_prefix = (uint32_t)s_prefix;
    const uint32_t lt = (1u << lane) - 1u;
#pragma unroll
    for (int k = 0; k < UQ_ITEMS; ++k) {
        const int e = k * SC_THREADS + tid;
        if (base + e < n) {
            const uint32_t h = (myhead >> k) & 1u;
            const uint32_t u = tile_prefix + s_part[k * (SC_THREADS / 32) + warp] + __popc(ball[k] & lt) + h - 1u;
            newid[src[k]] = u;
            if (h) {
                float* o = out_verts + 3 * (int64_t)u;
                o[0] = vz[k]; o[1] = vy[k]; o[2] = vx[k];
            }
        }
    }
}

__global__ void __launch_bounds__(256) k_unique_optimistic(const float* __restrict__ verts, const uint32_t* __restrict__ perm, int64_t V_cap,
                                                           const unsigned long long* __restrict__ V_dev, float* __restrict__ out_verts,
                                                           uint32_t* __restrict__ newid, unsigned long long* __restrict__ bad,
                                                           unsigned long long* __restrict__ n_unique_out, unsigned long long* __restrict__ dup)
{
    const int64_t n = dev_n(V_cap, V_dev);
    const int64_t i = (int64_t)blockIdx.x * blockDim.x + threadIdx.x;
    if (i == 0) *n_unique_out = (unsigned long long)n;
    const bool ok = i < n;
    uint32_t src = 0, kz = 0, ky = 0, kx = 0;
    if (ok) {
        src = perm[i];
        const float* a = verts + 3 * (int64_t)src;
        const float z = a[0], y = a[1], x = a[2];
        float* o = out_verts + 3 * i;
        o[0] = z; o[1] = y; o[2] = x;
        newid[src] = (uint32_t)i;
        kz = float_key(z); ky = float_key(y); kx = float_key(x);
    }
    uint32_t pz = __shfl_up_sync(0xffffffffu, kz, 1), py = __shfl_up_sync(0xffffffffu, ky, 1), px = __shfl_up_sync(0xffffffffu, kx, 1);
    if ((threadIdx.x & 31) == 0 && ok && i > 0) {
        const float* b = verts + 3 * (int64_t)perm[i - 1];
        pz = float_key(b[0]); py = float_key(b[1]); px = float_key(b[2]);
    }
    if (ok && i > 0) {
        if (kz == pz && ky == py && kx == px) atomicOr(dup, 1ull);
        else if ((kz < pz) || (kz == pz && (ky < py || (ky == py && kx < px)))) atomicOr(bad, 1ull);
    }
}

static thread_local cudaEvent_t g_faces_ready = nullptr;
void t3d_canon_faces_ready_event(cudaEvent_t e) { g_faces_ready = e; }
bool t3d_canon_faces_ready_pending() { const bool p = g_faces_ready != nullptr; g_faces_ready = nullptr; return p; }

static int canonical_tail(const float* vin, const uint32_t* perm, int64_t V, const unsigned long long* V_dev, const void* faces_in,
                          int64_t F, const unsigned long long* F_dev, void* verts_out, void* faces_out_i64, void* faces_out_i32,
                          unsigned long long* counts, uint32_t* flags, uint32_t* pos, uint32_t* newid, void* scan_ws,
                          void* scan_ws_faces, unsigned long long* totals, cudaStream_t st)
{
    void* stream = (void*)st;
    {
        const int64_t nb = (V + UQ_TILE - 1) / UQ_TILE;
        const size_t desc_bytes = (size_t)nb * 8;
        if (t3d_zero_async(scan_ws, desc_bytes + 64, st)) return 1;
        unsigned long long* dup = totals + 8;
        if (t3d_zero_async(dup, 8, st)) return 1;
        k_unique_optimistic<<<(unsigned)((V + 255) / 256), 256, 0, st>>>(vin, perm, V, V_dev, (float*)verts_out, newid, counts + 2, counts, dup);
        t3d_count_launches(1);
        k_unique_fused<<<(unsigned)nb, SC_THREADS, 0, st>>>(vin, perm, V, V_dev, (float*)verts_out, newid, (unsigned long long*)scan_ws,
                                                           (int)nb, (unsigned int*)((char*)scan_ws + desc_bytes), counts + 2, counts, dup);
    }
    if (g_faces_ready) {
        T3D_CUDA(cudaStreamWaitEvent(st, g_faces_ready, 0));
        g_faces_ready = nullptr;
    }
    if (F > 0) {
        const unsigned gf = (unsigned)((F + 255) / 256);
        if (t3d_zero_async(totals + 1, 16, st)) return 1;
        k_face_remap<<<gf, 256, 0, st>>>((const int32_t*)faces_in, F, newid, flags, (long long*)faces_out_i64, (int32_t*)faces_out_i32,
                                         totals + 1, F_dev);
        k_face_plan<<<1, 1, 0, st>>>(totals + 1, F, F_dev, totals + 2, counts + 1);
        if (t3d_exclusive_scan_u32_dev(flags, pos, F, F, 1, 0, 0, totals + 2, totals + 3, scan_ws_faces, stream)) return 1;
        const unsigned gc = gf < (unsigned)(T3D_NUM_SMS * 8) ? gf : (unsigned)(T3D_NUM_SMS * 8);
        k_face_compact<<<gc, 256, 0, st>>>((const int32_t*)faces_in, F, newid, flags, pos, (long long*)faces_out_i64,
                                           (int32_t*)faces_out_i32, totals + 2);
    } else {
        T3D_CUDA(cudaMemsetAsync(counts + 1, 0, 8, st));
    }
    return 0;
}

extern "C" int t3d_mesh_canonicalize_fast_dev(const void* verts_in, int64_t V, const void* V_dev_u64, const void* faces_in, int64_t F,
                                              const void* F_dev_u64, void* verts_out, void* faces_out_i64, void* faces_out_i32,
                                              void* counts_u64, void* workspace, void* stream)
{
    cudaStream_t st = (cudaStream_t)stream;
    if (V <= 0 || V > 0x7fffffff || F < 0) { t3d_set_error("t3d_mesh_canonicalize_fast_dev: bad sizes"); return 2; }
    const unsigned long long* V_dev = (const unsigned long long*)V_dev_u64;
    const unsigned long long* F_dev = (const unsigned long long*)F_dev_u64;
    const int64_t n = V > F ? V : F;
    char* ws = (char*)workspace;
    unsigned long long* keys_a = (unsigned long long*)ws; ws += align256(8 * V);
    unsigned long long* keys_b = (unsigned long long*)ws; ws += align256(8 * V);
    uint32_t* iota = (uint32_t*)ws; ws += align256(4 * V);
    uint32_t* perm = (uint32_t*)ws; ws += align256(4 * V);
    uint32_t* flags = (uint32_t*)ws; ws += align256(4 * n);
    uint32_t* pos = (uint32_t*)ws; ws += align256(4 * n);
    uint32_t* newid = (uint32_t*)ws; ws += align256(4 * V);
    size_t temp_bytes = sort64_temp_bytes(V);
    void* temp = ws; ws += align256((int64_t)temp_bytes);
    void* scan_ws = ws; ws += align256(t3d_scan_workspace_bytes(n, 1));
    unsigned long long* totals = (unsigned long long*)ws;
    unsigned long long* counts = (unsigned long long*)counts_u64;
    const unsigned gv = (unsigned)((V + 255) / 256);
    const float* vin = (const float*)verts_in;
    T3D_CUDA(cudaMemsetAsync(counts + 2, 0, 8, st));
    k_make_keys64<<<gv, 256, 0, st>>>(vin, V, V_dev, keys_a, iota);
    T3D_CUDA(cub::DeviceRadixSort::SortPairs(temp, temp_bytes, (const unsigned long long*)keys_a, keys_b, (const uint32_t*)iota, perm,
                                             (int)V, 0, 64, st));
    if (canonical_tail(vin, perm, V, V_dev, faces_in, F, F_dev, verts_out, faces_out_i64, faces_out_i32, counts, flags, pos, newid,
                       scan_ws, scan_ws, totals, st)) return 1;
    T3D_CHECK_LAUNCH("t3d_mesh_canonicalize_fast_dev");
    t3d_count_launches(F > 0 ? 5 : 3);
    return 0;
}

struct CanonS {
    const float* verts;
    const unsigned long long* vkeys;
    const unsigned long long* sizes;
    uint32_t cap_verts, cap_z, cap_g0;
    int Zs, Hs;
    int ncr;
    const uint32_t* chunkbase;
    const uint32_t* aw_base;
    uint32_t stride;
    int g_plane;
    int z_offset; float shift;
// ... 103 lines not shown
            if (lane == 31) s_carry[w] = incl;
            asm volatile("bar.sync 1, 256;" ::: "memory");
            uint32_t carry = 0;
            for (int ww = 0; ww < w; ++ww) carry += s_carry[ww];
            uint32_t run = carry + incl - v;
            for (int ww = 0; ww < ZS_WARPS; ++ww) { const uint32_t h = s_hist[ww][tid]; s_hist[ww][tid] = run; run += h; }
        }
        __syncthreads();
        for (uint32_t c0 = ws; c0 < we; c0 += 32 * ZS_U) {
            KeyT kk[ZS_U];
            uint32_t ii[ZS_U];
#pragma unroll
            for (int u = 0; u < ZS_U; ++u) {
                const uint32_t i = c0 + 32 * u + lane;
                kk[u] = 0; ii[u] = 0;
                if (i < we) {
                    kk[u] = first ? keyA[i] : kin[i];
                    ii[u] = first ? value_of(i) : iin[i];
                }
            }
#pragma unroll
            for (int u = 0; u < ZS_U; ++u) {
                if (c0 + 32 * u >= we) break;
                const uint32_t i = c0 + 32 * u + lane;
                const bool ok = i < we;
                const KeyT key = kk[u];
                const uint32_t idx = ii[u];
                const uint32_t d = ok ? ((uint32_t)(key >> shift) & 255u) : 0xffffffffu;
                const uint32_t peers = __match_any_sync(0xffffffffu, d);
                const uint32_t rank = __popc(peers & ((1u << lane) - 1u));
                uint32_t pos = 0;
                if (ok) pos = s_hist[w][d] + rank;
                __syncwarp();
                if (ok && rank == 0) s_hist[w][d] += __popc(peers);
                __syncwarp();
                if (ok) {
                    if (last) out[pos] = idx;
                    else { kout[pos] = key; iout[pos] = idx; }
                }
            }
        }
        __syncthreads();
        const KeyT* tk = kin; const uint32_t* ti = iin;
        kin = kout; iin = iout;
        kout = (KeyT*)tk; iout = (uint32_t*)ti;
    }
}

template <int ZS_U>
__global__ void __launch_bounds__(ZS_THREADS) k_zsort_layers(CanonS c, uint32_t* __restrict__ keyA, uint32_t* __restrict__ keyB,
                                                            uint32_t* __restrict__ idxA, uint32_t* __restrict__ idxB,
                                                            uint32_t* __restrict__ zperm)
{
    const uint32_t nx = (uint32_t)c.sizes[1], ny = (uint32_t)c.sizes[2], nz = (uint32_t)c.sizes[3];
    if ((unsigned long long)nx + ny + nz > c.cap_verts || nz > c.cap_z) return;
    const int layer = blockIdx.x;
    uint32_t s = before_row<2>(c, (int64_t)layer * c.Hs), e = before_row<2>(c, (int64_t)(layer + 1) * c.Hs);
    if (e > nz) e = nz;
    if (s >= e) return;
    const uint32_t n = e - s;
    uint32_t gX, gY, gZ;
    g0_sizes(c, gX, gY, gZ);
    if (n == 1 || e <= gZ) {
        for (uint32_t i = s + threadIdx.x; i < e; i += ZS_THREADS) zperm[i] = i;
        return;
    }
    cta_radix_sort_u<ZS_U, uint32_t>(n, (c.zkey_bits + 7) / 8, [&](uint32_t i) { return canon_zkey(c, s + i, nx, ny, gZ); },
                                     [&](uint32_t i) { return s + i; }, keyA + s, keyB + s, idxA + s, idxB + s, zperm + s);
}

__global__ void __launch_bounds__(ZS_THREADS) k_gsort(CanonS c, unsigned long long* __restrict__ keyA, unsigned long long* __restrict__ keyB,
                                                     uint32_t* __restrict__ idxA, uint32_t* __restrict__ idxB, uint32_t* __restrict__ gperm)
{
    const uint32_t nx = (uint32_t)c.sizes[1], ny = (uint32_t)c.sizes[2], nz = (uint32_t)c.sizes[3];
    if ((unsigned long long)nx + ny + nz > c.cap_verts) return;
    uint32_t gX, gY, gZ;
    g0_sizes(c, gX, gY, gZ);
    const uint32_t n = gX + gY + gZ;
    if (n == 0 || n > c.cap_g0) return;
    auto raw_of = [&](uint32_t t) -> uint32_t { return t < gX ? t : t < gX + gY ? nx + (t - gX) : nx + ny + (t - gX - gY); };
    if (n == 1) { if (threadIdx.x == 0) gperm[0] = raw_of(0); return; }
    cta_radix_sort_u<1, unsigned long long>(n, 8, [&](uint32_t t) {
        const float* v = c.verts + 3 * (int64_t)raw_of(t);
        return ((unsigned long long)float_key(v[1]) << 32) | float_key(v[2]);
    }, raw_of, keyA, keyB, idxA, idxB, gperm);
}

__global__ void __launch_bounds__(256) k_canon_positions(CanonS c)
{
    __shared__ uint32_t s_g[3];
    const uint32_t i = blockIdx.x * blockDim.x + threadIdx.x;
    const uint32_t nx = (uint32_t)c.sizes[1], ny = (uint32_t)c.sizes[2], nz = (uint32_t)c.sizes[3];
    const unsigned long long V64 = (unsigned long long)nx + ny + nz;
    if (V64 > c.cap_verts) return;
    if (threadIdx.x == 0) g0_sizes(c, s_g[0], s_g[1], s_g[2]);
    __syncthreads();
    if (i >= (uint32_t)V64) return;
    if (nz > c.cap_z) { c.perm[i] = i; return; }
    const uint32_t gX = s_g[0], gY = s_g[1], gZ = s_g[2];
    const uint32_t nG = gX + gY + gZ;
    if (i == 0 && c.n_g0_out) *c.n_g0_out = nG;
    if (i < nG) c.perm[i] = (nG <= c.cap_g0) ? c.gperm[i] : (i < gX ? i : i < gX + gY ? nx + (i - gX) : nx + ny + (i - gX - gY));
    if (i < nx) {
        if (i < gX) return;
        const unsigned long long key = c.vkeys[i];
        const int k = (int)(key >> 42), j = (int)((key >> 22) & 0xfffffu);
        c.perm[i + before_row<1>(c, (int64_t)k * c.Hs + j) + before_row<2>(c, (int64_t)k * c.Hs)] = i;
    } else if (i < nx + ny) {
        const uint32_t iy = i - nx;
        if (iy < gY) return;
        const unsigned long long key = c.vkeys[i];
        const int k = (int)(key >> 42), j = (int)((key >> 22) & 0xfffffu);
        const int64_t row = (int64_t)k * c.Hs + j;
        const uint32_t lo = before_row<1>(c, row), hi = before_row<1>(c, row + 1);
        const uint32_t mine = float_key(c.verts[3 * (int64_t)i + 1]);
        uint32_t r = 0;
        for (uint32_t e = lo; e < hi; ++e) {
            const uint32_t ke = float_key(c.verts[3 * (int64_t)(nx + e) + 1]);
            r += (ke < mine || (ke == mine && e < iy)) ? 1u : 0u;
        }
        c.perm[before_row<0>(c, row + 1) + lo + r + before_row<2>(c, (int64_t)k * c.Hs)] = i;
    } else {
        const uint32_t R = i - nx - ny;
        if (R < gZ) return;
        const uint32_t raw = nx + ny + c.zperm[R];
        const int64_t next_plane = ((int64_t)(c.vkeys[raw] >> 42) + 1) * c.Hs;
        c.perm[before_row<0>(c, next_plane) + before_row<1>(c, next_plane) + R] = raw;
    }
}

extern "C" int64_t t3d_canonicalize_structured_workspace_bytes(int64_t V, int64_t F, uint32_t cap_z, uint32_t cap_g0, int Zs)
{
    const int64_t n = V > F ? V : F;
    int64_t b = 0;
    b += 2 * align256(8 * (int64_t)cap_z) + 2 * align256(4 * (int64_t)cap_z);
    b += 2 * align256(8 * (int64_t)cap_g0) + 2 * align256(4 * (int64_t)cap_g0);
    b += align256(4 * V);
    b += 2 * align256(4 * n);
    b += align256(4 * V);
    b += align256(4 * (int64_t)cap_g0 + 256);
    b += 2 * align256(t3d_scan_workspace_bytes(n, 1)) + 256;
    return b;
// ... 46 lines not shown
                                                    const void* aw_base_u32, uint32_t aw_stride, int z_offset, int unpad_shift,
                                                    const void* cum_f64, const void* adj_f64, int n_cum, int zkey_bits,
                                                    uint32_t cap_z, uint32_t cap_g0, const void* faces_in, int64_t F_cap,
                                                    const void* F_dev_u64, void* verts_out, void* faces_out_i64, void* faces_out_i32,
                                                    void* counts_u64, void* n_g0_u64, void* workspace, int phases, void* stream)
{
    cudaStream_t st = (cudaStream_t)stream;
    if (zkey_bits <= 0 || zkey_bits > 32) zkey_bits = 32;
    if (V_cap <= 0 || V_cap > 0x7fffffff || F_cap < 0 || Zs <= 0 || Hs <= 0 || Ws <= 0 || cap_z == 0 || (phases & 3) == 0) {
        t3d_set_error("t3d_mesh_canonicalize_structured: bad sizes");
        return 2;
    }
    const int64_t V = V_cap, F = F_cap, n = V > F ? V : F;
    char* ws = (char*)workspace;
    CanonS c;
    c.verts = (const float*)verts_in;
    c.vkeys = (const unsigned long long*)vkeys_u64;
    c.sizes = (const unsigned long long*)sizes_u64;
    c.cap_verts = (uint32_t)V; c.cap_z = cap_z; c.cap_g0 = cap_g0;
    c.Zs = Zs; c.Hs = Hs;
    c.ncr = (t3d_wpr(Ws) + 31) >> 5;
    c.chunkbase = (const uint32_t*)chunkbase_u32;
    c.aw_base = (const uint32_t*)aw_base_u32;
    c.stride = aw_stride;
    c.g_plane = (n_cum > 0 && unpad_shift > 0) ? unpad_shift - z_offset : -1;
    c.z_offset = z_offset; c.shift = unpad_shift ? 1.0f : 0.0f;
    c.cum = (const double*)cum_f64; c.adj = (const double*)adj_f64; c.n_cum = n_cum;
    c.zkey_bits = zkey_bits;
    unsigned long long* zkeys_b; uint32_t* zperm; unsigned long long* gkeys_b; uint32_t* gperm;
    c.zkeys = (unsigned long long*)ws; ws += align256(8 * (int64_t)cap_z);
    zkeys_b = (unsigned long long*)ws; ws += align256(8 * (int64_t)cap_z);
    c.zval = (uint32_t*)ws; ws += align256(4 * (int64_t)cap_z);
    zperm = (uint32_t*)ws; ws += align256(4 * (int64_t)cap_z);
    c.gkeys = (unsigned long long*)ws; ws += align256(8 * (int64_t)cap_g0);
    gkeys_b = (unsigned long long*)ws; ws += align256(8 * (int64_t)cap_g0);
    c.gval = (uint32_t*)ws; ws += align256(4 * (int64_t)cap_g0);
    gperm = (uint32_t*)ws; ws += align256(4 * (int64_t)cap_g0);
    c.perm = (uint32_t*)ws; ws += align256(4 * V);
    uint32_t* flags = (uint32_t*)ws; ws += align256(4 * n);
    uint32_t* pos = (uint32_t*)ws; ws += align256(4 * n);
    uint32_t* newid = (uint32_t*)ws; ws += align256(4 * V);
    void* temp = ws; ws += align256(4 * (int64_t)cap_g0 + 256);
    void* scan_ws = ws; ws += align256(t3d_scan_workspace_bytes(n, 1));
    void* scan_ws_f = ws; ws += align256(t3d_scan_workspace_bytes(n, 1));
    unsigned long long* totals = (unsigned long long*)ws;
    unsigned long long* counts = (unsigned long long*)counts_u64;
    c.zperm = zperm; c.gperm = gperm;
    c.n_g0_out = (unsigned long long*)n_g0_u64;
    if (phases & 1) {
        uint32_t* keyA = (uint32_t*)c.zkeys;
        uint32_t* keyB = keyA + cap_z;
        uint32_t* idxA = (uint32_t*)zkeys_b;
        uint32_t* idxB = idxA + cap_z;
        if ((int64_t)cap_z >= 4096 * (int64_t)Zs) k_zsort_layers<8><<<Zs, ZS_THREADS, 0, st>>>(c, keyA, keyB, idxA, idxB, zperm);
        else k_zsort_layers<1><<<Zs, ZS_THREADS, 0, st>>>(c, keyA, keyB, idxA, idxB, zperm);
        t3d_count_launches(1);
    }
    if (phases & 2) {
        if (t3d_zero_async(counts + 2, 8, st)) return 1;
        if (cap_g0 > 0) {
            k_gsort<<<1, ZS_THREADS, 0, st>>>(c, c.gkeys, gkeys_b, c.gval, (uint32_t*)temp, gperm);
        }
        k_canon_positions<<<(unsigned)((V + 255) / 256), 256, 0, st>>>(c);
        if (canonical_tail(c.verts, c.perm, V, (const unsigned long long*)V_dev_u64, faces_in, F, (const unsigned long long*)F_dev_u64,
                           verts_out, faces_out_i64, faces_out_i32, counts, flags, pos, newid, scan_ws, scan_ws_f, totals, st)) return 1;
        t3d_count_launches((F > 0 ? 5 : 3) + (cap_g0 > 0 ? 1 : 0));
    }
    T3D_CHECK_LAUNCH("t3d_mesh_canonicalize_structured");
    return 0;
}

template <typename IdxT>
__global__ void __launch_bounds__(256) k_mesh_measure(const float* __restrict__ verts, const IdxT* __restrict__ faces, int64_t F_cap,
                                                      double* __restrict__ partials, const unsigned long long* __restrict__ F_dev = nullptr)
{
    const int64_t F = dev_n(F_cap, F_dev);
    double vol = 0.0, area = 0.0;
    for (int64_t i = (int64_t)blockIdx.x * blockDim.x + threadIdx.x; i < F; i += (int64_t)gridDim.x * blockDim.x) {
        const float* a = verts + 3 * (int64_t)faces[3 * i];
        const float* b = verts + 3 * (int64_t)faces[3 * i + 1];
        const float* c = verts + 3 * (int64_t)faces[3 * i + 2];
        const double ax = a[0], ay = a[1], az = a[2], bx = b[0], by = b[1], bz = b[2], cx = c[0], cy = c[1], cz = c[2];
        const double nx = by * cz - bz * cy, ny = bz * cx - bx * cz, nz = bx * cy - by * cx;
        vol += (ax * nx + ay * ny + az * nz) / 6.0;
        const double ux = bx - ax, uy = by - ay, uz = bz - az, vx = cx - ax, vy = cy - ay, vz = cz - az;
        const double px = uy * vz - uz * vy, py = uz * vx - ux * vz, pz = ux * vy - uy * vx;
        area += 0.5 * sqrt(px * px + py * py + pz * pz);
    }
    vol = warp_sum(vol); area = warp_sum(area);
    __shared__ double sv[8], sa[8];
    if (lane_id() == 0) { sv[threadIdx.x >> 5] = vol; sa[threadIdx.x >> 5] = area; }
    __syncthreads();
    if (threadIdx.x == 0) {
        double v = 0, a = 0;
        for (int k = 0; k < 8; ++k) { v += sv[k]; a += sa[k]; }
        partials[2 * blockIdx.x] = v; partials[2 * blockIdx.x + 1] = a;
    }
}

__global__ void __launch_bounds__(256) k_reduce_partials(const double* __restrict__ partials, int n, double* __restrict__ out)
{
    double v = 0, a = 0;
    for (int i = threadIdx.x; i < n; i += 256) { v += partials[2 * i]; a += partials[2 * i + 1]; }
    v = warp_sum(v); a = warp_sum(a);
    __shared__ double sv[8], sa[8];
    if (lane_id() == 0) { sv[threadIdx.x >> 5] = v; sa[threadIdx.x >> 5] = a; }
    __syncthreads();
    if (threadIdx.x == 0) {
        double tv = 0, ta = 0;
        for (int k = 0; k < 8; ++k) { tv += sv[k]; ta += sa[k]; }
        out[0] = tv; out[1] = ta;
    }
}

#define MM_BLOCKS (T3D_NUM_SMS * 4)

extern "C" int64_t t3d_mesh_measure_workspace_bytes(void) { return (int64_t)MM_BLOCKS * 2 * 8; }

extern "C" int t3d_mesh_measure_dev(const void* verts_f32, const void* faces, int64_t F, const void* F_dev_u64, int faces_are_i64,
                                    void* out_f64, void* workspace, void* stream)
{
    cudaStream_t st = (cudaStream_t)stream;
    const unsigned long long* F_dev = (const unsigned long long*)F_dev_u64;
    if (F <= 0) { T3D_CUDA(cudaMemsetAsync(out_f64, 0, 16, st)); return 0; }
    int blocks = (int)((F + 255) / 256);
    if (blocks > MM_BLOCKS) blocks = MM_BLOCKS;
    if (faces_are_i64)
        k_mesh_measure<long long><<<blocks, 256, 0, st>>>((const float*)verts_f32, (const long long*)faces, F, (double*)workspace, F_dev);
    else
        k_mesh_measure<int32_t><<<blocks, 256, 0, st>>>((const float*)verts_f32, (const int32_t*)faces, F, (double*)workspace, F_dev);
    k_reduce_partials<<<1, 256, 0, st>>>((const double*)workspace, blocks, (double*)out_f64);
    T3D_CHECK_LAUNCH("t3d_mesh_measure_dev");
    t3d_count_launches(2);
    return 0;
}
```

tomography_3d_reconstructor_b200/csrc/t3d_voxel.cu:

```cuda
#include <stdarg.h>
#include <stdlib.h>
#include <string.h>

#include "t3d_common.cuh"

static thread_local char g_err[512] = "";

extern "C" void t3d_set_error(const char* fmt, ...)
{
    va_list ap;
    va_start(ap, fmt);
    vsnprintf(g_err, sizeof(g_err), fmt, ap);
    va_end(ap);
}
extern "C" const char* t3d_last_error(void) { return g_err; }
static long long g_launches = 0;
extern "C" void t3d_count_launches(int n) { g_launches += n; }
extern "C" int64_t t3d_launch_count(void) { return g_launches; }

struct ZeroRange { const char* p; size_t n; };
static thread_local ZeroRange g_zero[8];
static thread_local int g_nzero = 0;
void t3d_prezero_register(const void* p, size_t n) { if (g_nzero < 8) g_zero[g_nzero++] = {(const char*)p, n}; }
void t3d_prezero_clear(void) { g_nzero = 0; }
int t3d_zero_async(void* p, size_t n, cudaStream_t st)
{
    for (int k = 0; k < g_nzero; ++k)
        if ((const char*)p >= g_zero[k].p && (const char*)p + n <= g_zero[k].p + g_zero[k].n) return 0;
    T3D_CUDA(cudaMemsetAsync(p, 0, n, st));
    return 0;
}

int t3d_num_sms(void)
{
    static int sms[64] = {0};
    int dev = 0;
    if (cudaGetDevice(&dev) != cudaSuccess) { cudaGetLastError(); return 148; }
    int& n = sms[dev & 63];
    if (n <= 0) {
        int v = 0;
        if (cudaDeviceGetAttribute(&v, cudaDevAttrMultiProcessorCount, dev) != cudaSuccess || v <= 0) { cudaGetLastError(); v = 148; }
        n = v;
    }
    return n;
}

bool t3d_first_use_on_device(int slot)
{
    static bool done[T3D_ONCE_SLOTS][64] = {};
    int dev = 0;
    if (cudaGetDevice(&dev) != cudaSuccess) { cudaGetLastError(); dev = 0; }
    bool& d = done[slot][dev & 63];
    const bool first = !d;
    d = true;
    return first;
}

extern "C" int t3d_version(void) { return 100; }
extern "C" int64_t t3d_words_per_row(int W) { return t3d_wpr(W); }

__global__ void __launch_bounds__(256) k_pack_flat(const uint8_t* __restrict__ src, uint32_t* __restrict__ dst,
                                                   int64_t n_words, uint32_t thr4)
{
    const int64_t warp = ((int64_t)blockIdx.x * blockDim.x + threadIdx.x) >> 5;
    const int64_t n_warps = ((int64_t)gridDim.x * blockDim.x) >> 5;
    const uint32_t l = lane_id();
    const int64_t n_chunks = n_words >> 5;
    for (int64_t c = warp; c < n_chunks; c += n_warps) {
        const uint8_t* p = src + (c << 10);
        const uint4 a = ld_stream_u4(p + 16 * l);
        const uint4 b = ld_stream_u4(p + 512 + 16 * l);
        const uint32_t ha = ge16(a, thr4), hb = ge16(b, thr4);
        const int s0 = (2 * l) & 31;
        const uint32_t a0 = __shfl_sync(0xffffffffu, ha, s0), a1 = __shfl_sync(0xffffffffu, ha, s0 + 1);
        const uint32_t b0 = __shfl_sync(0xffffffffu, hb, s0), b1 = __shfl_sync(0xffffffffu, hb, s0 + 1);
        dst[(c << 5) + l] = (l < 16) ? (a0 | (a1 << 16)) : (b0 | (b1 << 16));
    }
    const int64_t tail0 = n_chunks << 5;
    const int64_t t = tail0 + (int64_t)blockIdx.x * blockDim.x + threadIdx.x;
    if (t < n_words) {
        const uint4* p = reinterpret_cast<const uint4*>(src + (t << 5));
        dst[t] = ge16(p[0], thr4) | (ge16(p[1], thr4) << 16);
    }
}

__global__ void __launch_bounds__(256) k_pack_generic(const uint8_t* __restrict__ src, uint32_t* __restrict__ dst,
                                                      int64_t n_rows, int W, int wpr, int thr)
{
    const int64_t i = (int64_t)blockIdx.x * blockDim.x + threadIdx.x;
    if (i >= n_rows * wpr) return;
    const int64_t row = i / wpr;
    const int w = (int)(i - row * wpr);
    const uint8_t* p = src + row * W + (w << 5);
    const int n = min(32, W - (w << 5));
    uint32_t v = 0;
    for (int k = 0; k < n; ++k) v |= (uint32_t)(p[k] >= thr) << k;
    dst[i] = v;
}

extern "C" int t3d_pack_masks(const void* masks_u8, int Z, int H, int W, int threshold, void* bits, void* stream)
{
    if (Z <= 0 || H <= 0 || W <= 0) { t3d_set_error("t3d_pack_masks: empty volume"); return 2; }
    if (threshold < 0) threshold = 0;
    if (threshold > 256) threshold = 256;
    cudaStream_t st = (cudaStream_t)stream;
    const int wpr = t3d_wpr(W);
    const int64_t rows = (int64_t)Z * H;
    if ((W & 127) == 0 && ((uintptr_t)masks_u8 & 15) == 0 && threshold >= 1 && threshold <= 255) {
        const int64_t n_words = rows * wpr;
        const uint32_t thr4 = 0x01010101u * (uint32_t)threshold;
        int64_t blocks = (n_words / 32 + 7) / 8;
        const int64_t cap = (int64_t)T3D_NUM_SMS * 16;
        if (blocks > cap) blocks = cap;
        if (blocks < 1) blocks = 1;
        k_pack_flat<<<(unsigned)blocks, 256, 0, st>>>((const uint8_t*)masks_u8, (uint32_t*)bits, n_words, thr4);
    } else {
        const int64_t n = rows * wpr;
        k_pack_generic<<<(unsigned)((n + 255) / 256), 256, 0, st>>>((const uint8_t*)masks_u8, (uint32_t*)bits, rows, W,
                                                                    wpr, threshold);
    }
    T3D_CHECK_LAUNCH("t3d_pack_masks");
    t3d_count_launches(1);
    return 0;
}

__global__ void __launch_bounds__(256) k_unpack_flat(const uint32_t* __restrict__ src, uint8_t* __restrict__ dst,
                                                     int64_t n_words)
{
    const int64_t warp = ((int64_t)blockIdx.x * blockDim.x + threadIdx.x) >> 5;
    const int64_t n_warps = ((int64_t)gridDim.x * blockDim.x) >> 5;
    const uint32_t l = lane_id();
    const int64_t n_chunks = (n_words + 31) >> 5;
    for (int64_t c = warp; c < n_chunks; c += n_warps) {
        const int64_t wi = (c << 5) + l;
        const uint32_t w = wi < n_words ? src[wi] : 0u;
#pragma unroll
        for (int half = 0; half < 2; ++half) {
            const uint32_t ww = __shfl_sync(0xffffffffu, w, 16 * half + (l >> 1));
            const uint32_t h = (ww >> (16 * (l & 1))) & 0xffffu;
            uint4 o;
            o.x = expand4(h & 15u); o.y = expand4((h >> 4) & 15u);
            o.z = expand4((h >> 8) & 15u); o.w = expand4((h >> 12) & 15u);
            const int64_t word_of_lane = (c << 5) + 16 * half + (l >> 1);
            if (word_of_lane < n_words) st_stream_u4(dst + (c << 10) + 512 * half + 16 * l, o);
        }
    }
}

__global__ void __launch_bounds__(256) k_unpack_generic(const uint32_t* __restrict__ src, uint8_t* __restrict__ dst,
                                                        int64_t n_rows, int W, int wpr)
{
    const int64_t i = (int64_t)blockIdx.x * blockDim.x + threadIdx.x;
    if (i >= n_rows * wpr) return;
    const int64_t row = i / wpr;
    const int w = (int)(i - row * wpr);
    const uint32_t v = src[i];
    uint8_t* p = dst + row * W + (w << 5);
    const int n = min(32, W - (w << 5));
    for (int k = 0; k < n; ++k) p[k] = (v >> k) & 1u;
}

extern "C" int t3d_unpack_bits(const void* bits, int Z, int H, int W, void* out_u8, void* stream)
{
    if (Z <= 0 || H <= 0 || W <= 0) { t3d_set_error("t3d_unpack_bits: empty volume"); return 2; }
    cudaStream_t st = (cudaStream_t)stream;
    const int wpr = t3d_wpr(W);
    const int64_t rows = (int64_t)Z * H;
    const int64_t n = rows * wpr;
// ... 38 lines not shown
{
    const uint32_t l = lane_id();
    const int rsub = l >> 4, wsub = l & 15;
    const int n_tiles = (nwv + FH_TW - 1) / FH_TW;
    for (int dir = 0; dir < 2; ++dir) {
        uint32_t carry = 0;
        for (int t = 0; t < n_tiles; ++t) {
            const int c = dir == 0 ? t : n_tiles - 1 - t;
            const int w = c * FH_TW + wsub;
#pragma unroll
            for (int j = 0; j < 16; ++j) {
                const int rr = 2 * j + rsub, y = y0 + rr;
                const bool ok = (y < H) && (w < nwv);
                tm[rr * FH_PITCH + wsub] = ok ? m[(int64_t)y * nw + w] : 0u;
                tr[rr * FH_PITCH + wsub] = ok ? r[(int64_t)y * nw + w] : 0u;
            }
            __syncwarp();
            uint32_t* mr = tm + l * FH_PITCH;
            uint32_t* rr_ = tr + l * FH_PITCH;
            if (dir == 0) {
#pragma unroll
                for (int k = 0; k < FH_TW; ++k) {
                    const uint32_t mm = mr[k];
                    const uint32_t f = fill_up(mm, rr_[k] | (carry & mm & 1u));
                    carry = f >> 31;
                    rr_[k] = f;
                }
            } else {
#pragma unroll
                for (int k = FH_TW - 1; k >= 0; --k) {
                    const uint32_t mm = mr[k];
                    const uint32_t f = fill_dn(mm, rr_[k] | ((carry << 31) & mm));
                    carry = f & 1u;
                    rr_[k] = f;
                }
            }
            __syncwarp();
#pragma unroll
            for (int j = 0; j < 16; ++j) {
                const int rr = 2 * j + rsub, y = y0 + rr;
                if (y < H && w < nwv) r[(int64_t)y * nw + w] = tr[rr * FH_PITCH + wsub];
            }
            __syncwarp();
        }
    }
}

#define FH_THREADS 1024
#define FH_MAXSEG 64

__global__ void __launch_bounds__(FH_THREADS) k_fill_holes(uint32_t* bits_planes, int64_t plane_stride_words,
                                                           uint32_t* scratch, int H, int W, int nw)
{
    uint32_t* bits = bits_planes + (int64_t)blockIdx.x * plane_stride_words;
    const int64_t pw = (int64_t)H * nw;
    uint32_t* m = scratch + (int64_t)blockIdx.x * 2 * pw;
    uint32_t* r = m + pw;
    const int tid = threadIdx.x;
    const int warp = tid >> 5;

    for (int64_t i = tid; i < pw; i += FH_THREADS) {
        const int y = (int)(i / nw), w = (int)(i - (int64_t)y * nw);
        const uint32_t vm = valid_mask(w, W);
        const uint32_t bg = ~bits[i] & vm;
        uint32_t seed = 0;
        if (y == 0 || y == H - 1) seed = bg;
        if (w == 0) seed |= bg & 1u;
        if (w == ((W - 1) >> 5)) seed |= bg & (1u << ((W - 1) & 31));
        m[i] = bg;
        r[i] = seed;
    }
    __syncthreads();

    extern __shared__ uint32_t tile[];
    __shared__ uint32_t sG[FH_MAXSEG][32];
    __shared__ uint32_t sP[FH_MAXSEG][32];
    const int nseg = min(FH_MAXSEG, min(FH_THREADS / 32, H));
    const int L = (H + nseg - 1) / nseg;

    for (int iter = 0; iter < 4 * (H + W) + 8; ++iter) {
        int changed = 0;
        for (int y0 = warp * 32; y0 < H; y0 += (FH_THREADS / 32) * 32)
            rows_closure_tile(m, r, nw, (W + 31) >> 5, y0, H, tile + warp * 2 * 32 * FH_PITCH,
                              tile + warp * 2 * 32 * FH_PITCH + 32 * FH_PITCH);
        __syncthreads();
        for (int c0 = 0; c0 < nw; c0 += 32) {
            const int c = c0 + (tid & 31), seg = warp;
            const bool act = (c < nw) && (seg < nseg);
            const int y0 = seg * L, y1 = min(H, y0 + L);
            for (int dir = 0; dir < 2; ++dir) {
                uint32_t G = 0, P = 0xffffffffu;
                if (act && y0 < y1) {
                    if (dir == 0) for (int y = y0; y < y1; ++y) { const uint32_t mm = m[(int64_t)y * nw + c]; G = r[(int64_t)y * nw + c] | (G & mm); P &= mm; }
                    else          for (int y = y1 - 1; y >= y0; --y) { const uint32_t mm = m[(int64_t)y * nw + c]; G = r[(int64_t)y * nw + c] | (G & mm); P &= mm; }
                } else { P = 0xffffffffu; G = 0; }
                if (seg < FH_MAXSEG) { sG[seg][tid & 31] = G; sP[seg][tid & 31] = (act && y0 < y1) ? P : 0xffffffffu; }
                __syncthreads();
                uint32_t cin = 0;
                if (act) {
                    if (dir == 0) for (int s = 0; s < seg; ++s) cin = sG[s][tid & 31] | (sP[s][tid & 31] & cin);
                    else          for (int s = nseg - 1; s > seg; --s) cin = sG[s][tid & 31] | (sP[s][tid & 31] & cin);
                }
                if (act && y0 < y1) {
                    uint32_t carry = cin;
                    const int n = y1 - y0;
                    for (int k0 = 0; k0 < n; k0 += 8) {
                        uint32_t mm[8], rr[8];
#pragma unroll
                        for (int k = 0; k < 8; ++k) {
                            const int kk = k0 + k;
                            const int y = dir == 0 ? y0 + kk : y1 - 1 - kk;
                            const bool ok = kk < n;
                            mm[k] = ok ? m[(int64_t)y * nw + c] : 0u;
                            rr[k] = ok ? r[(int64_t)y * nw + c] : 0u;
                        }
#pragma unroll
                        for (int k = 0; k < 8; ++k) {
                            const int kk = k0 + k;
                            if (kk < n) {
                                const int y = dir == 0 ? y0 + kk : y1 - 1 - kk;
                                const uint32_t nv = rr[k] | (carry & mm[k]);
                                if (nv != rr[k]) { r[(int64_t)y * nw + c] = nv; changed = 1; }
                                carry = nv;
                            }
                        }
                    }
                }
                __syncthreads();
            }
        }
        if (!__syncthreads_or(changed)) break;
    }
    for (int64_t i = tid; i < pw; i += FH_THREADS) bits[i] |= m[i] & ~r[i];
}

extern "C" int64_t t3d_fill_holes_scratch_bytes(int n_planes, int H, int W)
{
    return (int64_t)n_planes * 2 * H * t3d_wpr(W) * 4;
}

extern "C" int t3d_fill_holes_2d(void* bits, int n_planes, int64_t plane_stride_words, int H, int W, void* scratch,
                                 void* stream)
{
    if (n_planes <= 0) return 0;
    if (H <= 0 || W <= 0) { t3d_set_error("t3d_fill_holes_2d: empty plane"); return 2; }
    const size_t smem = (size_t)(FH_THREADS / 32) * 2 * 32 * FH_PITCH * sizeof(uint32_t);
    if (t3d_first_use_on_device(T3D_ONCE_FILL_HOLES_ATTR))
        T3D_CUDA(cudaFuncSetAttribute(k_fill_holes, cudaFuncAttributeMaxDynamicSharedMemorySize, (int)smem));
    k_fill_holes<<<n_planes, FH_THREADS, smem, (cudaStream_t)stream>>>((uint32_t*)bits, plane_stride_words,
                                                                      (uint32_t*)scratch, H, W, t3d_wpr(W));
    T3D_CHECK_LAUNCH("t3d_fill_holes_2d");
    t3d_count_launches(1);
    return 0;
}

__global__ void __launch_bounds__(256) k_gap_fill(const uint4* __restrict__ in, uint4* __restrict__ out,
                                                  const uint4* __restrict__ lo, const uint4* __restrict__ hi, int Z,
                                                  int64_t pw4, unsigned long long* __restrict__ counts)
{
    const int z = blockIdx.y;
    const uint4* c = in + (int64_t)z * pw4;
    const uint4* a = (z > 0) ? c - pw4 : lo;
    const uint4* b = (z < Z - 1) ? c + pw4 : hi;
    uint4* o = out + (int64_t)z * pw4;
    uint32_t cnt = 0;
    const bool fill = (a != nullptr) && (b != nullptr);
    const int64_t stride = (int64_t)gridDim.x * 256;
    for (int64_t i = (int64_t)blockIdx.x * 256 + threadIdx.x; i < pw4; i += 2 * stride) {
        const int64_t j = i + stride;
        const bool two = j < pw4;
        uint4 v0 = c[i], v1 = two ? c[j] : make_uint4(0, 0, 0, 0);
        if (fill) {
            const uint4 a0 = a[i], b0 = b[i];
            v0 = or4(v0, and4(a0, b0));
            if (two) { const uint4 a1 = a[j], b1 = b[j]; v1 = or4(v1, and4(a1, b1)); }
        }
        o[i] = v0;
        if (two) o[j] = v1;
        cnt += popc4(v0) + popc4(v1);
    }
    if (counts) {
        cnt = warp_sum(cnt);
        __shared__ uint32_t s[8];
        if (lane_id() == 0) s[threadIdx.x >> 5] = cnt;
        __syncthreads();
        if (threadIdx.x == 0) {
            unsigned long long t = 0;
            for (int k = 0; k < 8; ++k) t += s[k];
            if (t) atomicAdd(counts + z, t);
        }
    }
}

extern "C" int t3d_gap_fill(const void* in_bits, void* out_bits, const void* lo_plane, const void* hi_plane, int Z, int H,
                            int W, void* slice_counts_u64, void* stream)
{
    if (Z <= 0 || H <= 0 || W <= 0) { t3d_set_error("t3d_gap_fill: empty volume"); return 2; }
    cudaStream_t st = (cudaStream_t)stream;
    const int64_t pw4 = (int64_t)H * (t3d_wpr(W) / 4);
    if (slice_counts_u64 && t3d_zero_async(slice_counts_u64, sizeof(unsigned long long) * Z, st)) return 1;
    int bx = (int)min((int64_t)32, (pw4 + 511) / 512);
    dim3 grid(bx, Z);
    k_gap_fill<<<grid, 256, 0, st>>>((const uint4*)in_bits, (uint4*)out_bits, (const uint4*)lo_plane, (const uint4*)hi_plane, Z,
                                     pw4, (unsigned long long*)slice_counts_u64);
    T3D_CHECK_LAUNCH("t3d_gap_fill");
    t3d_count_launches(1);
    return 0;
}

#define PG_ZC 128

struct PackGapArgs {
    const uint8_t* src;
    uint32_t* dst;
    int Z, nw;
    long long plane_words, plane_bytes;
    uint32_t thr4;
    int zc;
    int skip_ends;
    int z_bias;
    unsigned long long* counts;
    unsigned int* bbox_t;
};

struct ThrK { uint32_t add7, n7; };
__device__ __forceinline__ ThrK make_thrk(uint32_t thr4)
{
    ThrK k;
    k.add7 = 0x80808080u - (thr4 & 0x7f7f7f7fu);
    k.n7 = ~thr4 & 0x80808080u;
    return k;
}
__device__ __forceinline__ uint32_t ge4_top(uint32_t v, const ThrK& k)
{
    const uint32_t c = (v & 0x7f7f7f7fu) + k.add7;
    uint32_t r;
    asm("lop3.b32 %0, %1, %2, %3, 0xE8;" : "=r"(r) : "r"(c), "r"(v), "r"(k.n7));
    return (r & 0x80808080u) * 0x00204081u;
}
__device__ __forceinline__ uint32_t ge16k(const uint4& v, const ThrK& k)
{
    uint32_t acc = ge4_top(v.w, k) >> 28;
    acc = __funnelshift_l(ge4_top(v.z, k), acc, 4);
    acc = __funnelshift_l(ge4_top(v.y, k), acc, 4);
    acc = __funnelshift_l(ge4_top(v.x, k), acc, 4);
    return acc;
}

template <bool FULL>
__global__ void __launch_bounds__(256) k_pack_gap(PackGapArgs a)
{
    __shared__ unsigned int s_cnt[PG_ZC];
    __shared__ unsigned int s_bb[6];
    const int tid = threadIdx.x, warp = tid >> 5;
    const uint32_t l = lane_id();
    if (tid < PG_ZC) s_cnt[tid] = 0;
    if (tid < 6) s_bb[tid] = 0;
    __syncthreads();
    const long long span = (long long)blockIdx.x * 8 + warp;
    const int za = blockIdx.y * a.zc, zb = min(a.Z, za + a.zc);
    const long long wi = span * 32 + l;
    const bool wvalid = FULL || wi < a.plane_words;
    const long long boff = span * 1024 + 16 * l;
    const bool va = FULL || boff + 16 <= a.plane_bytes, vb = FULL || boff + 512 + 16 <= a.plane_bytes;
    const ThrK tk = make_thrk(a.thr4);
    const int s0 = (2 * l) & 31;
    const uint32_t sel = l < 16 ? 0x5410u : 0x7632u;
    auto load_raw = [&](int z, uint4& x, uint4& y) {
        const uint8_t* p = a.src + (long long)z * a.plane_bytes + boff;
        const uint4 zero = make_uint4(0, 0, 0, 0);
        x = va ? ld_stream_u4(p) : zero;
        y = vb ? ld_stream_u4(p + 512) : zero;
    };
    auto to_word = [&](const uint4& x, const uint4& y) -> uint32_t {
        const uint32_t hab = ge16k(x, tk) | (ge16k(y, tk) << 16);
        const uint32_t x0 = __shfl_sync(0xffffffffu, hab, s0), x1 = __shfl_sync(0xffffffffu, hab, s0 + 1);
        return __byte_perm(x0, x1, sel);
    };
    uint32_t acc = 0;
    int zmin = 0x7fffffff, zmax = -1;
    if (span * 1024 < a.plane_bytes) {
        uint4 r0x, r0y, r1x, r1y, r2x, r2y;
        const int p_hi = min(zb, a.Z - 1);
        uint32_t prev = 0u;
        if (za > 0) { load_raw(za - 1, r0x, r0y); prev = to_word(r0x, r0y); }
        load_raw(za, r0x, r0y);
        uint32_t cur = to_word(r0x, r0y);
        if (za + 1 <= p_hi) load_raw(za + 1, r0x, r0y);
        if (za + 2 <= p_hi) load_raw(za + 2, r1x, r1y);
        if (za + 3 <= p_hi) load_raw(za + 3, r2x, r2y);
        uint32_t* dp = a.dst + (long long)za * a.plane_words + wi;
        auto step = [&](int z, uint4& rx, uint4& ry) {
            const bool hn = z + 1 < a.Z;
            const uint32_t next = hn ? to_word(rx, ry) : 0u;
            if (z + 4 <= p_hi) load_raw(z + 4, rx, ry);
            uint32_t v = cur;
            if (z > 0 && hn) v |= prev & next;
            if (wvalid) *dp = v;
            dp += a.plane_words;
            acc |= v;
            const unsigned wc = __reduce_add_sync(0xffffffffu, (unsigned)__popc(v));
            if (wc) {
                zmin = min(zmin, z);
                zmax = z;
                const bool counted = !(a.skip_ends && (z < 2 || z >= a.Z - 2));
                if (l == 0 && counted) atomicAdd(&s_cnt[z - za], wc);
            }
            prev = cur;
            cur = next;
        };
        for (int z = za; z < zb; z += 3) {
            step(z, r0x, r0y);
            if (z + 1 < zb) step(z + 1, r1x, r1y);
            if (z + 2 < zb) step(z + 2, r2x, r2y);
        }
    }
    if (a.bbox_t && zmax >= 0) {
        int ymin = 0x7fffffff, ymax = -1, xmin = 0x7fffffff, xmax = -1;
        if (acc) {
            const int y = (int)(wi / a.nw), w = (int)(wi - (long long)y * a.nw);
            ymin = ymax = y;
            xmin = (w << 5) + __ffs(acc) - 1;
            xmax = (w << 5) + 31 - __clz(acc);
        }
        ymin = __reduce_min_sync(0xffffffffu, ymin); ymax = __reduce_max_sync(0xffffffffu, ymax);
        xmin = __reduce_min_sync(0xffffffffu, xmin); xmax = __reduce_max_sync(0xffffffffu, xmax);
        if (l == 0) {
            atomicMax(&s_bb[0], (unsigned)(0x7fffffff - (zmin + a.z_bias))); atomicMax(&s_bb[1], (unsigned)(zmax + a.z_bias + 1));
            atomicMax(&s_bb[2], (unsigned)(0x7fffffff - ymin)); atomicMax(&s_bb[3], (unsigned)(ymax + 1));
            atomicMax(&s_bb[4], (unsigned)(0x7fffffff - xmin)); atomicMax(&s_bb[5], (unsigned)(xmax + 1));
        }
    }
    __syncthreads();
    if (a.counts && tid < zb - za && s_cnt[tid]) atomicAdd(a.counts + za + tid, (unsigned long long)s_cnt[tid]);
    if (a.bbox_t && tid < 6 && s_bb[tid]) atomicMax(a.bbox_t + tid, s_bb[tid]);
}

struct EndsFixArgs {
    const uint8_t* src;
    const uint32_t* f0;
    const uint32_t* fT;
    uint32_t* dst;
    int Z;
    long long plane_words, plane_bytes;
    uint32_t thr4;
    unsigned long long* counts;
};

__global__ void __launch_bounds__(256) k_close_ends_fixup(EndsFixArgs a)
{
    const long long i = (long long)blockIdx.x * 256 + threadIdx.x;
    const long long pw = a.plane_words;
    const int Z = a.Z;
    unsigned c[4] = {0, 0, 0, 0};
    if (i < pw) {
        auto raw = [&](int z) -> uint32_t {
            const uint4* p = reinterpret_cast<const uint4*>(a.src + (long long)z * a.plane_bytes + 32 * i);
            return ge16(p[0], a.thr4) | (ge16(p[1], a.thr4) << 16);
        };
        const uint32_t b = a.f0[i], t = a.fT[i];
        a.dst[i] = b;
        a.dst[(long long)(Z - 1) * pw + i] = t;
        c[0] = __popc(b); c[3] = __popc(t);
        const uint32_t v1 = raw(1) | (b & ((Z - 1 == 2) ? t : raw(2)));
        a.dst[pw + i] = v1;
        c[1] = __popc(v1);
        if (Z - 2 != 1) {
            const uint32_t vT = raw(Z - 2) | (((Z - 3 == 0) ? b : raw(Z - 3)) & t);
            a.dst[(long long)(Z - 2) * pw + i] = vT;
            c[2] = __popc(vT);
        }
    }
    if (!a.counts) return;
    __shared__ unsigned s[4];
    if (threadIdx.x < 4) s[threadIdx.x] = 0;
    __syncthreads();
#pragma unroll
    for (int k = 0; k < 4; ++k) {
        const unsigned w = __reduce_add_sync(0xffffffffu, c[k]);
        if (lane_id() == 0 && w) atomicAdd(&s[k], w);
    }
    __syncthreads();
    if (threadIdx.x < 4 && s[threadIdx.x]) {
        const int zz = threadIdx.x == 0 ? 0 : threadIdx.x == 1 ? 1 : threadIdx.x == 2 ? Z - 2 : Z - 1;
        atomicAdd(a.counts + zz, (unsigned long long)s[threadIdx.x]);
    }
}

bool t3d_pack_gap_supported(const void* masks_u8, int Z, int H, int W, int threshold)
{
    return Z >= 3 && H > 0 && (W & 127) == 0 && ((uintptr_t)masks_u8 & 15) == 0 && threshold >= 1 && threshold <= 255;
}

int t3d_pack_gap_launch(const void* masks_u8, int Z, int H, int W, int threshold, void* out, unsigned long long* counts,
                        unsigned int* bbox_t, int skip_ends, cudaStream_t st, int z_bias)
{
    PackGapArgs a;
    a.z_bias = z_bias;
    a.src = (const uint8_t*)masks_u8; a.dst = (uint32_t*)out;
    a.Z = Z; a.nw = t3d_wpr(W);
    a.plane_words = (long long)H * a.nw; a.plane_bytes = (long long)H * W;
    a.thr4 = 0x01010101u * (uint32_t)threshold;
    const long long n_spans = (a.plane_bytes + 1023) / 1024;
    long long chunks = ((long long)T3D_NUM_SMS * 64 + n_spans - 1) / n_spans;
    if (chunks < 1) chunks = 1;
    int zc = (int)((Z + chunks - 1) / chunks);
    if (zc < 16) zc = 16;
    if (zc > PG_ZC) zc = PG_ZC;
    a.zc = zc;
    a.skip_ends = skip_ends;
    a.counts = counts; a.bbox_t = bbox_t;
    dim3 grid((unsigned)((n_spans + 7) / 8), (unsigned)((Z + zc - 1) / zc));
    if (a.plane_bytes % 1024 == 0) k_pack_gap<true><<<grid, 256, 0, st>>>(a);
    else k_pack_gap<false><<<grid, 256, 0, st>>>(a);
    T3D_CHECK_LAUNCH("t3d_pack_gap");
    t3d_count_launches(1);
    return 0;
}

extern "C" int t3d_pack_gap(const void* masks_u8, int Z, int H, int W, int threshold, void* bits, void* counts_u64, void* bbox_u32x6,
                            void* stream)
{
    if (!t3d_pack_gap_supported(masks_u8, Z, H, W, threshold)) {
        t3d_set_error("t3d_pack_gap: needs Z >= 3, W %% 128 == 0, a 16-byte aligned stack and 1 <= threshold <= 255");
        return 2;
    }
    cudaStream_t st = (cudaStream_t)stream;
    return t3d_pack_gap_launch(masks_u8, Z, H, W, threshold, bits, (unsigned long long*)counts_u64, (unsigned int*)bbox_u32x6, 0, st);
}

__global__ void __launch_bounds__(256) k_bbox_t_planes(const uint32_t* __restrict__ bits, int H, int nw, int z_bias, unsigned int* __restrict__ bbox_t)
{
    const int z = blockIdx.y;
    const uint32_t* p = bits + (long long)z * H * nw;
    const int rows_per = (H + gridDim.x - 1) / gridDim.x;
    const int ya = blockIdx.x * rows_per, yb = min(H, ya + rows_per);
    int ymin = 0x7fffffff, ymax = -1, xmin = 0x7fffffff, xmax = -1;
    for (long long i = (long long)ya * nw + threadIdx.x; i < (long long)yb * nw; i += 256) {
        const uint32_t v = p[i];
        if (v) {
            const int y = (int)(i / nw), w = (int)(i - (long long)y * nw);
            ymin = min(ymin, y); ymax = max(ymax, y);
            xmin = min(xmin, (w << 5) + __ffs(v) - 1);
            xmax = max(xmax, (w << 5) + 31 - __clz(v));
        }
    }
    ymin = __reduce_min_sync(0xffffffffu, ymin); ymax = __reduce_max_sync(0xffffffffu, ymax);
    xmin = __reduce_min_sync(0xffffffffu, xmin); xmax = __reduce_max_sync(0xffffffffu, xmax);
    if ((threadIdx.x & 31) == 0 && ymax >= 0) {
        atomicMax(bbox_t + 0, (unsigned)(0x7fffffff - (z + z_bias))); atomicMax(bbox_t + 1, (unsigned)(z + z_bias + 1));
        atomicMax(bbox_t + 2, (unsigned)(0x7fffffff - ymin)); atomicMax(bbox_t + 3, (unsigned)(ymax + 1));
        atomicMax(bbox_t + 4, (unsigned)(0x7fffffff - xmin)); atomicMax(bbox_t + 5, (unsigned)(xmax + 1));
    }
}

int t3d_bbox_t_planes_launch(const uint32_t* bits, int n_planes, int H, int W, int z_bias, unsigned int* bbox_t, cudaStream_t st)
{
    if (n_planes <= 0) return 0;
    dim3 grid((unsigned)min(8, H), (unsigned)n_planes);
    k_bbox_t_planes<<<grid, 256, 0, st>>>(bits, H, t3d_wpr(W), z_bias, bbox_t);
    T3D_CHECK_LAUNCH("t3d_bbox_t_planes");
    t3d_count_launches(1);
    return 0;
}

int t3d_close_ends_fixup_launch(const void* masks_u8, int Z, int H, int W, int threshold, const void* filled0, const void* filledT,
                                void* out, unsigned long long* counts, cudaStream_t st)
{
    EndsFixArgs a;
    a.src = (const uint8_t*)masks_u8; a.f0 = (const uint32_t*)filled0; a.fT = (const uint32_t*)filledT; a.dst = (uint32_t*)out;
    a.Z = Z; a.plane_words = (long long)H * t3d_wpr(W); a.plane_bytes = (long long)H * W;
    a.thr4 = 0x01010101u * (uint32_t)threshold;
    a.counts = counts;
    k_close_ends_fixup<<<(unsigned)((a.plane_words + 255) / 256), 256, 0, st>>>(a);
    T3D_CHECK_LAUNCH("t3d_close_ends_fixup");
    t3d_count_launches(1);
    return 0;
}

#define MY 8

struct MorphArgs {
    const uint32_t* in;
    uint32_t* out;
    int Z, H, W, nw;
    int z0, nz;
    int out_rs;
    long long out_ps;
    int lanes_x, pz_per_block, my;
    int ring_tail;
    unsigned long long* counts;
};

__device__ __align__(16) const uint32_t g_border_row[8] = {0u, 0u, 0u, 0u, 0xffffffffu, 0xffffffffu, 0xffffffffu, 0xffffffffu};

template <bool ER, bool FIX, bool COUNT, bool RING>
__global__ void __launch_bounds__(256, 4) k_morph(MorphArgs a)
{
    const int lx = threadIdx.x % a.lanes_x, pz = threadIdx.x / a.lanes_x;
    const int nw4 = a.nw >> 2, nwv = (a.W + 31) >> 5;
    const int w4 = blockIdx.x * a.lanes_x + lx, zi = blockIdx.z * a.pz_per_block + pz, y0 = blockIdx.y * a.my;
    extern __shared__ unsigned int s_cnt[];
    if (COUNT) {
        if ((int)threadIdx.x < a.pz_per_block) s_cnt[threadIdx.x] = 0;
        __syncthreads();
    }
    if (pz < a.pz_per_block && w4 < nw4 && zi < a.nz) {
        const int z = a.z0 + zi;
        const uint4 vm = valid_mask4(w4, a.W);
        const bool fix = FIX && ER && (4 * w4 + 4 > (a.W >> 5));
        const uint4 fixm = fix ? make_uint4(~vm.x, ~vm.y, ~vm.z, ~vm.w) : make_uint4(0, 0, 0, 0);
        auto ld4 = [&](const uint32_t* p) -> uint4 {
            uint4 v = *reinterpret_cast<const uint4*>(p);
            if (FIX && ER) v = or4(v, fixm);
            return v;
        };
        const uint32_t* border = g_border_row + (ER ? 4 : 0);
        const bool has_l = (w4 > 0), has_r = (4 * w4 + 4 < nwv);
        const bool fix_r = FIX && ER && has_r && (4 * w4 + 5 >= nwv);
        const uint32_t fix_r_bits = fix_r ? ~valid_mask(4 * w4 + 4, a.W) : 0u;
        const long long in_ps = (long long)a.H * a.nw;
        const uint32_t* pc = a.in + (long long)z * in_ps + (long long)y0 * a.nw + 4 * w4;
        const uint32_t* pm = (z > 0) ? pc - in_ps : border;
        const uint32_t* pp = (z + 1 < a.Z) ? pc + in_ps : border;
        const uint32_t* pl = has_l ? pc - 1 : border;
        const uint32_t* pr = has_r ? pc + 4 : border;
        const int sm = (z > 0) ? a.nw : 0, sp = (z + 1 < a.Z) ? a.nw : 0, sl = has_l ? a.nw : 0, sr = has_r ? a.nw : 0;
// ... 57 lines not shown
    } else {
        if (erode) { if (fixw) { if (counts) T3D_MORPH_LAUNCH(true, true, true, false); else T3D_MORPH_LAUNCH(true, true, false, false); }
                     else { if (counts) T3D_MORPH_LAUNCH(true, false, true, false); else T3D_MORPH_LAUNCH(true, false, false, false); } }
        else { if (counts) T3D_MORPH_LAUNCH(false, false, true, false); else T3D_MORPH_LAUNCH(false, false, false, false); }
    }
#undef T3D_MORPH_LAUNCH
    T3D_CHECK_LAUNCH("t3d_morph_stage");
    t3d_count_launches(1);
    return 0;
}

#define M4_R 2
#define M4_PF 4
#define M4_ZC_MAX 128
#define M4_EM 9u

struct Morph4Args {
    const uint32_t* in;
    uint32_t* out;
    int Z, H, nw4;
    int z0, nz;
    int out_rs;
    long long out_ps;
    int ty, zc;
    int ring_tail;
    unsigned long long* counts;
};

__device__ __forceinline__ void cp_async16(void* smem_dst, const void* gsrc)
{
    asm volatile("cp.async.cg.shared.global [%0], [%1], 16;\n" ::"r"((uint32_t)__cvta_generic_to_shared(smem_dst)), "l"(gsrc) : "memory");
}
__device__ __forceinline__ void cp_async_commit() { asm volatile("cp.async.commit_group;\n" ::: "memory"); }
template <int N>
__device__ __forceinline__ void cp_async_wait() { asm volatile("cp.async.wait_group %0;\n" ::"n"(N) : "memory"); }

__device__ __forceinline__ uint4 lds128(uint32_t addr)
{
    uint4 v;
    asm volatile("ld.shared.v4.u32 {%0, %1, %2, %3}, [%4];\n" : "=r"(v.x), "=r"(v.y), "=r"(v.z), "=r"(v.w) : "r"(addr) : "memory");
    return v;
}
__device__ __forceinline__ void sts128(uint32_t addr, uint4 v)
{
    asm volatile("st.shared.v4.u32 [%0], {%1, %2, %3, %4};\n" ::"r"(addr), "r"(v.x), "r"(v.y), "r"(v.z), "r"(v.w) : "memory");
}
__device__ __forceinline__ void cp_async16s(uint32_t saddr, const void* gsrc)
{
    asm volatile("cp.async.cg.shared.global [%0], [%1], 16;\n" ::"r"(saddr), "l"(gsrc) : "memory");
}

__global__ void __launch_bounds__(512, 1) k_morph4(Morph4Args a)
{
    extern __shared__ __align__(16) uint32_t m4_smem[];
    __shared__ unsigned int s_cnt[M4_ZC_MAX];
    const int nw4 = a.nw4;
    const uint32_t row_b = 16u * nw4;
    const int tid = threadIdx.x, x4 = tid % nw4, rg = tid / nw4;
    const int rows = a.ty + 8;
    const int yl0 = rg * M4_R;
    const int y0 = blockIdx.x * a.ty - 4;
    const int za = a.z0 + blockIdx.y * a.zc, zb = min(a.z0 + a.nz, za + a.zc);
    const uint32_t tile_b = (uint32_t)rows * row_b;
    const uint32_t me = (uint32_t)__cvta_generic_to_shared(m4_smem) + (uint32_t)yl0 * row_b + 16u * x4;
    const uint32_t xb0 = me + M4_PF * tile_b;
    for (int i = tid; i < M4_ZC_MAX; i += blockDim.x) s_cnt[i] = 0;
    __syncthreads();

    const uint4 ones = splat4(0xffffffffu), zeros = splat4(0u);
    bool rowin[M4_R], rowst[M4_R];
    uint32_t rowout[M4_R];
#pragma unroll
    for (int r = 0; r < M4_R; ++r) {
        const int yl = yl0 + r, y = y0 + yl;
        rowin[r] = y >= 0 && y < a.H;
        rowst[r] = rowin[r] && yl >= 4 && yl < 4 + a.ty;
        rowout[r] = rowin[r] ? 0u : 0xffffffffu;
    }
    const long long in_ps = (long long)a.H * 4 * nw4;
    const int t0 = za - 4, t_last = zb + 3;
    const uint32_t* gnext = a.in + (long long)t0 * in_ps + (long long)(y0 + yl0) * 4 * nw4 + 4 * x4;
    int pnext = t0;
    const int p_hi = min(a.Z - 1, t_last);

    auto issue = [&](uint32_t saddr) {
        const bool need = pnext >= 0 && pnext <= p_hi;
#pragma unroll
        for (int r = 0; r < M4_R; ++r) {
            if (need && rowin[r]) cp_async16s(saddr + r * row_b, gnext + r * 4 * nw4);
            else sts128(saddr + r * row_b, (M4_EM & 1u) ? ones : zeros);
        }
        cp_async_commit();
        gnext += in_ps;
        ++pnext;
    };

    uint4 Q[4][M4_R], Xp[4][M4_R];
#pragma unroll
    for (int s = 0; s < 4; ++s)
#pragma unroll
        for (int r = 0; r < M4_R; ++r) { Q[s][r] = zeros; Xp[s][r] = zeros; }

#pragma unroll
    for (int k = 0; k < M4_PF - 1; ++k) issue(me + k * tile_b);
    uint32_t slot_a = me;
    uint32_t slot_w = me + (M4_PF - 1) * tile_b;
// ... 78 lines not shown
            if (s_cnt[i]) atomicAdd(a.counts + (za - a.z0) + i, (unsigned long long)s_cnt[i]);
    }
}

bool t3d_morph4_eligible(int Z, int H, int W)
{
    if ((W & 127) || W > 4096 || W < 512) return false;
    const int nw4 = W / 128;
    return (32 % nw4) == 0 && Z >= 1 && H >= 1;
}

int t3d_morph4_launch(const uint32_t* in, uint32_t* out, int Z, int H, int W, int z0, int nz, int out_rs, long long out_ps, int ring_tail,
                      unsigned long long* counts, cudaStream_t st)
{
    Morph4Args a;
    a.in = in; a.out = out; a.Z = Z; a.H = H; a.nw4 = W / 128;
    a.z0 = z0; a.nz = nz; a.out_rs = out_rs; a.out_ps = out_ps; a.ring_tail = ring_tail; a.counts = counts;
    const int nw = 4 * a.nw4;
    const int warp_rows = M4_R * (32 / a.nw4);
    int rows_max = 512 / a.nw4 * M4_R;
    const int by_smem = (200 * 1024) / ((M4_PF + 6) * nw * 4);
    if (rows_max > by_smem) rows_max = by_smem;
    rows_max -= rows_max % warp_rows;
    if (rows_max < 9 || rows_max < warp_rows) { t3d_set_error("t3d_morph4: tile does not fit"); return 2; }
    const int sms = T3D_NUM_SMS;
    int rows = 0, zc = 0;
    double best = 1e300;
    for (int rr = rows_max; rr >= 16 && rr >= warp_rows; rr -= warp_rows) {
        const int ty = rr - 8, bands = (H + ty - 1) / ty, thr = rr / M4_R * a.nw4;
        int per_sm = 512 / thr;
        const int smem_fit = (int)((220 * 1024) / ((size_t)(M4_PF + 6) * rr * nw * 4));
        if (per_sm > smem_fit) per_sm = smem_fit;
        if (per_sm < 1) continue;
        static const int zcs[] = {16, 24, 32, 48, 64, 96, 128};
        for (int zi = 0; zi < 7; ++zi) {
            const int c = zcs[zi];
            if (c > M4_ZC_MAX) continue;
            const long long ctas = (long long)bands * ((nz + c - 1) / c);
            const double load = (double)((ctas + sms - 1) / sms) * rr;
            const double floor_ = 48.0 * (double)((ctas + (long long)sms * per_sm - 1) / ((long long)sms * per_sm));
            const double cost = (load > floor_ ? load : floor_) * (c + 8);
            if (cost < best) { best = cost; rows = rr; zc = c; }
        }
    }
    if (rows == 0) { t3d_set_error("t3d_morph4: no tile configuration"); return 2; }
    a.ty = rows - 8;
    const int bands = (H + a.ty - 1) / a.ty;
    a.zc = zc;
    const int threads = rows / M4_R * a.nw4;
    const size_t smem = (size_t)(M4_PF + 6) * rows * nw * 4;
    if (t3d_first_use_on_device(T3D_ONCE_MORPH4_ATTR))
        T3D_CUDA(cudaFuncSetAttribute(k_morph4, cudaFuncAttributeMaxDynamicSharedMemorySize, 200 * 1024));
    dim3 grid(bands, (nz + zc - 1) / zc);
    k_morph4<<<grid, threads, smem, st>>>(a);
    T3D_CHECK_LAUNCH("t3d_morph4");
    t3d_count_launches(1);
    return 0;
}

extern "C" int64_t t3d_morph_scratch_bytes(int Z, int H, int W, int n_stages)
{
    return n_stages > 1 ? (int64_t)Z * H * t3d_wpr(W) * 4 * (n_stages > 2 ? 2 : 1) : 0;
}

extern "C" int t3d_morph(const void* in_bits, void* out_bits, int Z, int H, int W, int n_stages, unsigned erode_mask,
                         void* slice_counts_u64, void* scratch, void* stream)
{
    if (Z <= 0 || H <= 0 || W <= 0) { t3d_set_error("t3d_morph: empty volume"); return 2; }
    if (n_stages < 1 || n_stages > 32) { t3d_set_error("t3d_morph: n_stages must be 1..32"); return 2; }
    if (in_bits == out_bits) { t3d_set_error("t3d_morph: in-place is not supported"); return 2; }
    if (n_stages > 1 && !scratch) { t3d_set_error("t3d_morph: scratch required for more than one stage"); return 2; }
    cudaStream_t st = (cudaStream_t)stream;
    const int nw = t3d_wpr(W);
    const int64_t vol_words = (int64_t)Z * H * nw;
    if (slice_counts_u64 && t3d_zero_async(slice_counts_u64, sizeof(unsigned long long) * Z, st)) return 1;
    uint32_t* tmp[2] = {(uint32_t*)scratch, (uint32_t*)scratch + vol_words};
    const uint32_t* src = (const uint32_t*)in_bits;
    for (int s = 0; s < n_stages; ++s) {
        const bool last = (s == n_stages - 1);
        uint32_t* dst = last ? (uint32_t*)out_bits : tmp[s & 1];
        unsigned long long* cnt = last ? (unsigned long long*)slice_counts_u64 : nullptr;
        if (int rc = t3d_morph_stage(src, dst, Z, H, W, 0, Z, nw, (long long)H * nw, (erode_mask >> s) & 1u, false, 0, cnt, st)) return rc;
        src = dst;
    }
    return 0;
}

__global__ void k_stats_init(unsigned long long* counts, int Z, int* bbox)
{
    const int i = blockIdx.x * blockDim.x + threadIdx.x;
    if (counts && i < Z) counts[i] = 0;
    if (bbox && i < 6) bbox[i] = (i & 1) ? -1 : 0x7fffffff;
}

#define ST_YSPLIT 4

__global__ void __launch_bounds__(256) k_stats(const uint32_t* __restrict__ bits, int H, int nw,
                                               unsigned long long* __restrict__ counts, int* __restrict__ bbox)
{
    const int z = blockIdx.z;
    const int w = blockIdx.x * 32 + threadIdx.x;
    const int rows_per = (H + ST_YSPLIT - 1) / ST_YSPLIT;
    const int ya = blockIdx.y * rows_per, yb = min(H, ya + rows_per);
    const uint32_t* p = bits + (int64_t)z * H * nw;
    unsigned long long cnt = 0;
    int ymin = 0x7fffffff, ymax = -1, xmin = 0x7fffffff, xmax = -1;
    if (w < nw) {
// ... 116 lines not shown
```

Before: 857.4.

## Launch pipeline kernels with programmatic dependent launch and griddepcontrol.wait

Moves most pipeline kernels to cudaLaunchKernelEx with the programmatic stream serialization attribute, and puts a griddepcontrol.wait at the start of each kernel. The next kernel's blocks can then be scheduled and do their prologue before the previous grid finishes, hiding launch and tail latency across the long chain of small kernels. No kernel triggers an early launch_dependents, so the overlap is limited to launch setup. It also makes every kernel depend on correct wait placement; in k_mc_vertices_all some shared-memory setup now runs before the wait.

Measured after the change: 858.2 (median of 6 runs). No clear change (+0.1%).

```diff
diff --git a/tomography_3d_reconstructor_b200/csrc/t3d_common.cuh b/tomography_3d_reconstructor_b200/csrc/t3d_common.cuh
--- a/tomography_3d_reconstructor_b200/csrc/t3d_common.cuh
+++ b/tomography_3d_reconstructor_b200/csrc/t3d_common.cuh
@@ -129,6 +129,24 @@
     return v < (unsigned long long)cap ? (int64_t)v : cap;
 }
 
+__device__ __forceinline__ void t3d_dep_wait() { asm volatile("griddepcontrol.wait;" ::: "memory"); }
+
+template <typename... KArgs, typename... Args>
+static inline cudaError_t t3d_launch_dep(void (*kernel)(KArgs...), dim3 grid, dim3 block, size_t smem, cudaStream_t st, Args&&... args)
+{
+    cudaLaunchAttribute attr[1];
+    attr[0].id = cudaLaunchAttributeProgrammaticStreamSerialization;
+    attr[0].val.programmaticStreamSerializationAllowed = 1;
+    cudaLaunchConfig_t cfg = {};
+    cfg.gridDim = grid;
+    cfg.blockDim = block;
+    cfg.dynamicSmemBytes = smem;
+    cfg.stream = st;
+    cfg.attrs = attr;
+    cfg.numAttrs = 1;
+    return cudaLaunchKernelEx(&cfg, kernel, static_cast<Args&&>(args)...);
+}
+
 int t3d_morph_stage(const uint32_t* in, uint32_t* out, int Z, int H, int W, int z0, int nz, int out_rs, long long out_ps,
                     bool erode, bool ring, int ring_tail, unsigned long long* counts, cudaStream_t st);
 bool t3d_morph4_eligible(int Z, int H, int W);
diff --git a/tomography_3d_reconstructor_b200/csrc/t3d_mc.cu b/tomography_3d_reconstructor_b200/csrc/t3d_mc.cu
--- a/tomography_3d_reconstructor_b200/csrc/t3d_mc.cu
+++ b/tomography_3d_reconstructor_b200/csrc/t3d_mc.cu
@@ -188,6 +188,7 @@
 
 __global__ void __launch_bounds__(256, 4) k_mc_flags(Grid g, uint32_t* __restrict__ ballots, int lanes_x, int pz_per_block, int gy)
 {
+    t3d_dep_wait();
     const int lx = threadIdx.x % lanes_x, pz = threadIdx.x / lanes_x;
     const int nws4 = g.nws >> 2;
     const int w4 = blockIdx.x * lanes_x + lx, z = g.z_begin + blockIdx.z * pz_per_block + pz, y0 = blockIdx.y * gy;
@@ -248,6 +249,7 @@
                                                     const uint32_t* __restrict__ chunkbase, int64_t n_chunks,
                                                     uint32_t* __restrict__ aw_idx, uint32_t cap_active)
 {
+    t3d_dep_wait();
     const int64_t c = (int64_t)blockIdx.x * blockDim.x + threadIdx.x;
     if (c >= n_chunks) return;
     uint32_t bal = ballots[c];
@@ -271,6 +273,7 @@
                                                   const unsigned long long* __restrict__ n_active_dev, uint32_t* __restrict__ aw_cnt,
                                                   unsigned long long* __restrict__ n_ambiguous)
 {
+    t3d_dep_wait();
     const uint32_t n_active = cap_active;
     const int64_t n = dev_n(cap_active, n_active_dev);
     if (!AMB) {
@@ -363,6 +366,7 @@
 template <int PARTS, int AMB>
 __global__ void __launch_bounds__(128) k_mc_emit(EmitArgs a)
 {
+    t3d_dep_wait();
     __shared__ __align__(16) int8_t s_tri[256][T3D_MC_ROW];
     __shared__ uint32_t s_base[12][128];
     __shared__ uint32_t s_mask[12][128];
@@ -566,6 +570,7 @@
     __shared__ ZLut zlut;
     fill_zlut(p.occ, zlut);
     __syncthreads();
+    t3d_dep_wait();
     const unsigned long long nx = sizes[1], ny = sizes[2], nz = sizes[3];
     if (nx + ny + nz > cap_verts) return;
     uint32_t t = blockIdx.x * blockDim.x + threadIdx.x;
@@ -607,7 +612,7 @@
     const int nws4 = g.nws / 4, lanes_x = nws4 < 256 ? nws4 : 256, pzb = 256 / lanes_x;
     const int nz = (g.z_end < Zs ? g.z_end + 1 : Zs) - g.z_begin;
     dim3 grid((nws4 + lanes_x - 1) / lanes_x, (Hs + GY - 1) / GY, (nz + pzb - 1) / pzb);
-    k_mc_flags<<<grid, 256, 0, st>>>(g, (uint32_t*)ballots_u32, lanes_x, pzb, GY);
+    T3D_CUDA(t3d_launch_dep(k_mc_flags, grid, 256, 0, st, g, (uint32_t*)ballots_u32, lanes_x, pzb, GY));
     T3D_CHECK_LAUNCH("t3d_mc_flags");
     t3d_count_launches(1);
     return 0;
@@ -624,12 +629,12 @@
     if (t3d_zero_async(n_ambiguous_u64, 8, st)) return 1;
     if (cap_active == 0) return 0;
     const int64_t n_chunks = (int64_t)g.n_rows * g.ncr;
-    k_mc_compact<<<(unsigned)((n_chunks + 255) / 256), 256, 0, st>>>(g, (const uint32_t*)ballots_u32, (const uint32_t*)chunkbase_u32,
-                                                                      n_chunks, (uint32_t*)aw_idx_u32, cap_active);
-    k_mc_words<0><<<(cap_active + 127) / 128, 128, 0, st>>>(g, fld, (uint32_t*)aw_idx_u32, cap_active, (const unsigned long long*)sizes_u64,
-                                                            (uint32_t*)aw_cnt_u32, (unsigned long long*)n_ambiguous_u64);
-    k_mc_words<1><<<amb_grid(cap_active), 128, 0, st>>>(g, fld, (uint32_t*)aw_idx_u32, cap_active, (const unsigned long long*)sizes_u64,
-                                                            (uint32_t*)aw_cnt_u32, (unsigned long long*)n_ambiguous_u64);
+    T3D_CUDA(t3d_launch_dep(k_mc_compact, (unsigned)((n_chunks + 255) / 256), 256, 0, st, g, (const uint32_t*)ballots_u32, (const uint32_t*)chunkbase_u32,
+                                                                      n_chunks, (uint32_t*)aw_idx_u32, cap_active));
+    T3D_CUDA(t3d_launch_dep(k_mc_words<0>, (cap_active + 127) / 128, 128, 0, st, g, fld, (uint32_t*)aw_idx_u32, cap_active, (const unsigned long long*)sizes_u64,
+                                                            (uint32_t*)aw_cnt_u32, (unsigned long long*)n_ambiguous_u64));
+    T3D_CUDA(t3d_launch_dep(k_mc_words<1>, amb_grid(cap_active), 128, 0, st, g, fld, (uint32_t*)aw_idx_u32, cap_active, (const unsigned long long*)sizes_u64,
+                                                            (uint32_t*)aw_cnt_u32, (unsigned long long*)n_ambiguous_u64));
     T3D_CHECK_LAUNCH("t3d_mc_words_dev");
     t3d_count_launches(3);
     return 0;
@@ -665,12 +670,12 @@
     a.faces = (int32_t*)faces_i32;
     const unsigned ge = (cap_active + 127) / 128;
     int launches = 1;
-    if ((parts & 3) == 1) k_mc_emit<1, 0><<<ge, 128, 0, (cudaStream_t)stream>>>(a);
+    if ((parts & 3) == 1) T3D_CUDA(t3d_launch_dep(k_mc_emit<1, 0>, ge, 128, 0, (cudaStream_t)stream, a));
     else if ((parts & 3) == 2) {
-        k_mc_emit<2, 0><<<ge, 128, 0, (cudaStream_t)stream>>>(a);
-        k_mc_emit<2, 1><<<amb_grid(cap_active), 128, 0, (cudaStream_t)stream>>>(a);
+        T3D_CUDA(t3d_launch_dep(k_mc_emit<2, 0>, ge, 128, 0, (cudaStream_t)stream, a));
+        T3D_CUDA(t3d_launch_dep(k_mc_emit<2, 1>, amb_grid(cap_active), 128, 0, (cudaStream_t)stream, a));
         launches = 2;
-    } else k_mc_emit<3, 2><<<ge, 128, 0, (cudaStream_t)stream>>>(a);
+    } else T3D_CUDA(t3d_launch_dep(k_mc_emit<3, 2>, ge, 128, 0, (cudaStream_t)stream, a));
     T3D_CHECK_LAUNCH("t3d_mc_emit_dev");
     t3d_count_launches(launches);
     return 0;
@@ -727,8 +732,8 @@
     p.mm_x = mm_per_pixel_x;
     p.scale_f64 = scale_in_f64 ? 1 : 0;
     p.verts = (float*)verts_f32;
-    k_mc_vertices_all<<<(cap_verts + 127) / 128, 128, 0, (cudaStream_t)stream>>>(p, (const unsigned long long*)sizes_u64, cap_verts,
-                                                                               which_blocks & 7);
+    T3D_CUDA(t3d_launch_dep(k_mc_vertices_all, (cap_verts + 127) / 128, 128, 0, (cudaStream_t)stream, p, (const unsigned long long*)sizes_u64, cap_verts,
+                                                                               which_blocks & 7));
     T3D_CHECK_LAUNCH("t3d_mc_vertices_dev");
     t3d_count_launches(1);
     return 0;
diff --git a/tomography_3d_reconstructor_b200/csrc/t3d_pipeline.cu b/tomography_3d_reconstructor_b200/csrc/t3d_pipeline.cu
--- a/tomography_3d_reconstructor_b200/csrc/t3d_pipeline.cu
+++ b/tomography_3d_reconstructor_b200/csrc/t3d_pipeline.cu
@@ -97,6 +97,7 @@
 __global__ void k_finalize_sizes(unsigned long long* r, unsigned long long capNA, unsigned long long capV, unsigned long long capF,
                                  int bbox_transformed)
 {
+    t3d_dep_wait();
     if (bbox_transformed) {
         unsigned int* t = (unsigned int*)(r + R_BBOX_I32X6);
         int* b = (int*)(r + R_BBOX_I32X6);
@@ -123,6 +124,7 @@
 __global__ void k_count_plane_vertices(const float* __restrict__ verts, const unsigned long long* n_dev, float z_ghost, float z_lead,
                                        int want_ghost, int want_lead, unsigned long long* out_ghost, unsigned long long* out_lead)
 {
+    t3d_dep_wait();
     const int w = threadIdx.x >> 5, lane = threadIdx.x & 31;
     const bool want = w == 0 ? want_ghost != 0 : want_lead != 0;
     unsigned long long* out = w == 0 ? out_ghost : out_lead;
@@ -187,6 +189,7 @@
 };
 __global__ void __launch_bounds__(256) k_zero_ranges(ZeroSet z)
 {
+    t3d_dep_wait();
     for (int k = 0; k < z.n; ++k)
         for (unsigned long long i = (unsigned long long)blockIdx.x * blockDim.x + threadIdx.x; i < z.n16[k];
              i += (unsigned long long)gridDim.x * blockDim.x)
@@ -206,8 +209,7 @@
     int launch(cudaStream_t st)
     {
         if (!z.n) return 0;
-        k_zero_ranges<<<T3D_NUM_SMS * 2, 256, 0, st>>>(z);
-        T3D_CHECK_LAUNCH("k_zero_ranges");
+        T3D_CUDA(t3d_launch_dep(k_zero_ranges, T3D_NUM_SMS * 2, 256, 0, st, z));
         t3d_count_launches(1);
         return 0;
     }
@@ -223,6 +225,7 @@
 
 __global__ void __launch_bounds__(256) k_zero_ring(uint4* __restrict__ S, int Zs, int Hs, int nws4)
 {
+    t3d_dep_wait();
     const long long plane4 = (long long)Hs * nws4;
     const long long nA = 2 * plane4, nB = (long long)(Zs - 2) * 2 * nws4;
     const uint4 zero = make_uint4(0, 0, 0, 0);
@@ -304,7 +307,7 @@
             const long long items = 2 * (long long)Hp * (nws / 4) + (long long)(Zp - 2) * 2 * (nws / 4);
             long long blocks = (items + 255) / 256;
             if (blocks > (long long)T3D_NUM_SMS * 8) blocks = (long long)T3D_NUM_SMS * 8;
-            k_zero_ring<<<(unsigned)(blocks < 1 ? 1 : blocks), 256, 0, side->s>>>((uint4*)S, Zp, Hp, nws / 4);
+            T3D_CUDA(t3d_launch_dep(k_zero_ring, (unsigned)(blocks < 1 ? 1 : blocks), 256, 0, side->s, (uint4*)S, Zp, Hp, nws / 4));
             t3d_count_launches(1);
         }
         T3D_CUDA(cudaEventRecord(side->e[3], side->s));
@@ -350,7 +353,8 @@
                               R + R_NACTIVE, ws + L.aw_idx, ws + L.aw_cnt, R + R_NAMBIGUOUS, st));
     RUN(t3d_exclusive_scan_u32_dev(ws + L.aw_cnt, ws + L.aw_base, cap_active, cap_active, 4, 0, 0, R + R_NACTIVE, R + R_NX,
                                    ws + L.scan2, st));
-    k_finalize_sizes<<<1, 1, 0, st>>>(R, cap_active, cap_verts, cap_faces, bbox_state == 2 ? 1 : 0);
+    T3D_CUDA(t3d_launch_dep(k_finalize_sizes, 1, 1, 0, st, R, (unsigned long long)cap_active, (unsigned long long)cap_verts,
+                            (unsigned long long)cap_faces, bbox_state == 2 ? 1 : 0));
     t3d_count_launches(1);
     marks.mark("scan+words+scan", st);
     RUN(t3d_mc_emit_view_dev(view, x_off, ws + L.sign, Zp, Hp, Wp, g.z_begin, g.z_end, ws + L.ballots, ws + L.chunkbase, ws + L.aw_idx,
@@ -379,8 +383,8 @@
                                            verts_out_f32, faces_out_i64, nullptr, R + R_VCANON, ws + L.canon, st));
     if (t3d_canon_faces_ready_pending()) T3D_CUDA(cudaStreamWaitEvent(st, side->e[6], 0));
     if (g.want_ghost || g.want_lead)
-        k_count_plane_vertices<<<1, 64, 0, st>>>((const float*)verts_out_f32, R + R_VCANON, g.z_ghost, g.z_lead, g.want_ghost,
-                                                 g.want_lead, R + R_NGHOST, R + R_NLEAD);
+        T3D_CUDA(t3d_launch_dep(k_count_plane_vertices, 1, 64, 0, st, (const float*)verts_out_f32, R + R_VCANON, g.z_ghost, g.z_lead,
+                                g.want_ghost, g.want_lead, R + R_NGHOST, R + R_NLEAD));
     if (g.want_ghost || g.want_lead) t3d_count_launches(1);
     marks.mark("canonicalize", st);
     T3D_CUDA(cudaStreamWaitEvent(st, side->e[5], 0));
diff --git a/tomography_3d_reconstructor_b200/csrc/t3d_surface.cu b/tomography_3d_reconstructor_b200/csrc/t3d_surface.cu
--- a/tomography_3d_reconstructor_b200/csrc/t3d_surface.cu
+++ b/tomography_3d_reconstructor_b200/csrc/t3d_surface.cu
@@ -138,6 +138,7 @@
                                                               const unsigned long long* __restrict__ n_dev,
                                                               unsigned long long* __restrict__ totals)
 {
+    t3d_dep_wait();
     const int64_t n = dev_n(n_cap, n_dev);
     const uint32_t* a = in + (int64_t)blockIdx.y * stride;
     OutT* o = out + (int64_t)blockIdx.y * stride;
@@ -229,12 +230,12 @@
     const unsigned long long* nd = (const unsigned long long*)n_dev_u64;
     dim3 grid((unsigned)nb, n_arrays);
     if (out_is_u64)
-        k_scan_lookback<unsigned long long><<<grid, SC_THREADS, 0, st>>>((const uint32_t*)in, (unsigned long long*)out, n_cap, stride, desc,
+        T3D_CUDA(t3d_launch_dep(k_scan_lookback<unsigned long long>, grid, SC_THREADS, 0, st, (const uint32_t*)in, (unsigned long long*)out, n_cap, stride, desc,
                                                                          (int)nb, tickets, popcount_input, nd,
-                                                                         (unsigned long long*)totals_u64);
+                                                                         (unsigned long long*)totals_u64));
     else
-        k_scan_lookback<uint32_t><<<grid, SC_THREADS, 0, st>>>((const uint32_t*)in, (uint32_t*)out, n_cap, stride, desc, (int)nb, tickets,
-                                                               popcount_input, nd, (unsigned long long*)totals_u64);
+        T3D_CUDA(t3d_launch_dep(k_scan_lookback<uint32_t>, grid, SC_THREADS, 0, st, (const uint32_t*)in, (uint32_t*)out, n_cap, stride, desc, (int)nb, tickets,
+                                                               popcount_input, nd, (unsigned long long*)totals_u64));
     T3D_CHECK_LAUNCH("t3d_exclusive_scan_u32_dev");
     t3d_count_launches(1);
     return 0;
@@ -388,6 +389,7 @@
                                                       long long* __restrict__ out64, int32_t* __restrict__ out32,
                                                       const unsigned long long* __restrict__ F_dev = nullptr)
 {
+    t3d_dep_wait();
     const int64_t F = dev_n(F_cap, F_dev);
     for (int64_t i = (int64_t)blockIdx.x * blockDim.x + threadIdx.x; i < F; i += (int64_t)gridDim.x * blockDim.x) {
         if (!valid[i]) continue;
@@ -402,6 +404,7 @@
                                                     uint32_t* __restrict__ valid, long long* __restrict__ out64, int32_t* __restrict__ out32,
                                                     unsigned long long* __restrict__ n_invalid, const unsigned long long* __restrict__ F_dev)
 {
+    t3d_dep_wait();
     const int64_t i = (int64_t)blockIdx.x * blockDim.x + threadIdx.x;
     const int64_t F = dev_n(F_cap, F_dev);
     bool bad = false;
@@ -419,6 +422,7 @@
 __global__ void k_face_plan(const unsigned long long* __restrict__ n_invalid, int64_t F_cap, const unsigned long long* __restrict__ F_dev,
                             unsigned long long* __restrict__ n_to_compact, unsigned long long* __restrict__ f_out)
 {
+    t3d_dep_wait();
     const unsigned long long F = (unsigned long long)dev_n(F_cap, F_dev);
     *n_to_compact = (*n_invalid) ? F : 0ull;
     *f_out = F - *n_invalid;
@@ -490,8 +494,8 @@
         k_face_valid<<<gf, 256, 0, st>>>((const int32_t*)faces_in, F, newid, flags);
         if (t3d_exclusive_scan_u32_dev(flags, pos, F, F, 1, 0, 0, nullptr, totals, scan_ws, stream)) return 1;
         T3D_CUDA(cudaMemcpyAsync(counts + 1, totals, 8, cudaMemcpyDeviceToDevice, st));
-        k_face_compact<<<gf, 256, 0, st>>>((const int32_t*)faces_in, F, newid, flags, pos, (long long*)faces_out_i64,
-                                           (int32_t*)faces_out_i32);
+        T3D_CUDA(t3d_launch_dep(k_face_compact, gf, 256, 0, st, (const int32_t*)faces_in, F, newid, flags, pos, (long long*)faces_out_i64,
+                                (int32_t*)faces_out_i32, (const unsigned long long*)nullptr));
     } else {
         T3D_CUDA(cudaMemsetAsync(counts + 1, 0, 8, st));
     }
@@ -560,6 +564,7 @@
                                                              unsigned long long* __restrict__ n_unique_out,
                                                              const unsigned long long* __restrict__ skip_unless)
 {
+    t3d_dep_wait();
     if (skip_unless && *skip_unless == 0) return;
     const int64_t n = dev_n(V_cap, V_dev);
     volatile unsigned long long* d = desc;
@@ -674,6 +679,7 @@
                                                            uint32_t* __restrict__ newid, unsigned long long* __restrict__ bad,
                                                            unsigned long long* __restrict__ n_unique_out, unsigned long long* __restrict__ dup)
 {
+    t3d_dep_wait();
     const int64_t n = dev_n(V_cap, V_dev);
     const int64_t i = (int64_t)blockIdx.x * blockDim.x + threadIdx.x;
     if (i == 0) *n_unique_out = (unsigned long long)n;
@@ -715,10 +721,10 @@
         if (t3d_zero_async(scan_ws, desc_bytes + 64, st)) return 1;
         unsigned long long* dup = totals + 8;
         if (t3d_zero_async(dup, 8, st)) return 1;
-        k_unique_optimistic<<<(unsigned)((V + 255) / 256), 256, 0, st>>>(vin, perm, V, V_dev, (float*)verts_out, newid, counts + 2, counts, dup);
+        T3D_CUDA(t3d_launch_dep(k_unique_optimistic, (unsigned)((V + 255) / 256), 256, 0, st, vin, perm, V, V_dev, (float*)verts_out, newid, counts + 2, counts, dup));
         t3d_count_launches(1);
-        k_unique_fused<<<(unsigned)nb, SC_THREADS, 0, st>>>(vin, perm, V, V_dev, (float*)verts_out, newid, (unsigned long long*)scan_ws,
-                                                           (int)nb, (unsigned int*)((char*)scan_ws + desc_bytes), counts + 2, counts, dup);
+        T3D_CUDA(t3d_launch_dep(k_unique_fused, (unsigned)nb, SC_THREADS, 0, st, vin, perm, V, V_dev, (float*)verts_out, newid, (unsigned long long*)scan_ws,
+                                                           (int)nb, (unsigned int*)((char*)scan_ws + desc_bytes), counts + 2, counts, dup));
     }
     if (g_faces_ready) {
         T3D_CUDA(cudaStreamWaitEvent(st, g_faces_ready, 0));
@@ -727,13 +733,13 @@
     if (F > 0) {
         const unsigned gf = (unsigned)((F + 255) / 256);
         if (t3d_zero_async(totals + 1, 16, st)) return 1;
-        k_face_remap<<<gf, 256, 0, st>>>((const int32_t*)faces_in, F, newid, flags, (long long*)faces_out_i64, (int32_t*)faces_out_i32,
-                                         totals + 1, F_dev);
-        k_face_plan<<<1, 1, 0, st>>>(totals + 1, F, F_dev, totals + 2, counts + 1);
+        T3D_CUDA(t3d_launch_dep(k_face_remap, gf, 256, 0, st, (const int32_t*)faces_in, F, newid, flags, (long long*)faces_out_i64, (int32_t*)faces_out_i32,
+                                         totals + 1, F_dev));
+        T3D_CUDA(t3d_launch_dep(k_face_plan, 1, 1, 0, st, totals + 1, F, F_dev, totals + 2, counts + 1));
         if (t3d_exclusive_scan_u32_dev(flags, pos, F, F, 1, 0, 0, totals + 2, totals + 3, scan_ws_faces, stream)) return 1;
         const unsigned gc = gf < (unsigned)(T3D_NUM_SMS * 8) ? gf : (unsigned)(T3D_NUM_SMS * 8);
-        k_face_compact<<<gc, 256, 0, st>>>((const int32_t*)faces_in, F, newid, flags, pos, (long long*)faces_out_i64,
-                                           (int32_t*)faces_out_i32, totals + 2);
+        T3D_CUDA(t3d_launch_dep(k_face_compact, gc, 256, 0, st, (const int32_t*)faces_in, F, newid, flags, pos, (long long*)faces_out_i64,
+                                           (int32_t*)faces_out_i32, totals + 2));
     } else {
         T3D_CUDA(cudaMemsetAsync(counts + 1, 0, 8, st));
     }
@@ -943,6 +949,7 @@
                                                             uint32_t* __restrict__ idxA, uint32_t* __restrict__ idxB,
                                                             uint32_t* __restrict__ zperm)
 {
+    t3d_dep_wait();
     const uint32_t nx = (uint32_t)c.sizes[1], ny = (uint32_t)c.sizes[2], nz = (uint32_t)c.sizes[3];
     if ((unsigned long long)nx + ny + nz > c.cap_verts || nz > c.cap_z) return;
     const int layer = blockIdx.x;
@@ -963,6 +970,7 @@
 __global__ void __launch_bounds__(ZS_THREADS) k_gsort(CanonS c, unsigned long long* __restrict__ keyA, unsigned long long* __restrict__ keyB,
                                                      uint32_t* __restrict__ idxA, uint32_t* __restrict__ idxB, uint32_t* __restrict__ gperm)
 {
+    t3d_dep_wait();
     const uint32_t nx = (uint32_t)c.sizes[1], ny = (uint32_t)c.sizes[2], nz = (uint32_t)c.sizes[3];
     if ((unsigned long long)nx + ny + nz > c.cap_verts) return;
     uint32_t gX, gY, gZ;
@@ -979,6 +987,7 @@
 
 __global__ void __launch_bounds__(256) k_canon_positions(CanonS c)
 {
+    t3d_dep_wait();
     __shared__ uint32_t s_g[3];
     const uint32_t i = blockIdx.x * blockDim.x + threadIdx.x;
     const uint32_t nx = (uint32_t)c.sizes[1], ny = (uint32_t)c.sizes[2], nz = (uint32_t)c.sizes[3];
@@ -1131,16 +1140,16 @@
         uint32_t* keyB = keyA + cap_z;
         uint32_t* idxA = (uint32_t*)zkeys_b;
         uint32_t* idxB = idxA + cap_z;
-        if ((int64_t)cap_z >= 4096 * (int64_t)Zs) k_zsort_layers<8><<<Zs, ZS_THREADS, 0, st>>>(c, keyA, keyB, idxA, idxB, zperm);
-        else k_zsort_layers<1><<<Zs, ZS_THREADS, 0, st>>>(c, keyA, keyB, idxA, idxB, zperm);
+        if ((int64_t)cap_z >= 4096 * (int64_t)Zs) T3D_CUDA(t3d_launch_dep(k_zsort_layers<8>, Zs, ZS_THREADS, 0, st, c, keyA, keyB, idxA, idxB, zperm));
+        else T3D_CUDA(t3d_launch_dep(k_zsort_layers<1>, Zs, ZS_THREADS, 0, st, c, keyA, keyB, idxA, idxB, zperm));
         t3d_count_launches(1);
     }
     if (phases & 2) {
         if (t3d_zero_async(counts + 2, 8, st)) return 1;
         if (cap_g0 > 0) {
-            k_gsort<<<1, ZS_THREADS, 0, st>>>(c, c.gkeys, gkeys_b, c.gval, (uint32_t*)temp, gperm);
-        }
-        k_canon_positions<<<(unsigned)((V + 255) / 256), 256, 0, st>>>(c);
+            T3D_CUDA(t3d_launch_dep(k_gsort, 1, ZS_THREADS, 0, st, c, c.gkeys, gkeys_b, c.gval, (uint32_t*)temp, gperm));
+        }
+        T3D_CUDA(t3d_launch_dep(k_canon_positions, (unsigned)((V + 255) / 256), 256, 0, st, c));
         if (canonical_tail(c.verts, c.perm, V, (const unsigned long long*)V_dev_u64, faces_in, F, (const unsigned long long*)F_dev_u64,
                            verts_out, faces_out_i64, faces_out_i32, counts, flags, pos, newid, scan_ws, scan_ws_f, totals, st)) return 1;
         t3d_count_launches((F > 0 ? 5 : 3) + (cap_g0 > 0 ? 1 : 0));
@@ -1153,6 +1162,7 @@
 __global__ void __launch_bounds__(256) k_mesh_measure(const float* __restrict__ verts, const IdxT* __restrict__ faces, int64_t F_cap,
                                                       double* __restrict__ partials, const unsigned long long* __restrict__ F_dev = nullptr)
 {
+    t3d_dep_wait();
     const int64_t F = dev_n(F_cap, F_dev);
     double vol = 0.0, area = 0.0;
     for (int64_t i = (int64_t)blockIdx.x * blockDim.x + threadIdx.x; i < F; i += (int64_t)gridDim.x * blockDim.x) {
@@ -1179,6 +1189,7 @@
 
 __global__ void __launch_bounds__(256) k_reduce_partials(const double* __restrict__ partials, int n, double* __restrict__ out)
 {
+    t3d_dep_wait();
     double v = 0, a = 0;
     for (int i = threadIdx.x; i < n; i += 256) { v += partials[2 * i]; a += partials[2 * i + 1]; }
     v = warp_sum(v); a = warp_sum(a);
@@ -1205,10 +1216,10 @@
     int blocks = (int)((F + 255) / 256);
     if (blocks > MM_BLOCKS) blocks = MM_BLOCKS;
     if (faces_are_i64)
-        k_mesh_measure<long long><<<blocks, 256, 0, st>>>((const float*)verts_f32, (const long long*)faces, F, (double*)workspace, F_dev);
+        T3D_CUDA(t3d_launch_dep(k_mesh_measure<long long>, blocks, 256, 0, st, (const float*)verts_f32, (const long long*)faces, F, (double*)workspace, F_dev));
     else
-        k_mesh_measure<int32_t><<<blocks, 256, 0, st>>>((const float*)verts_f32, (const int32_t*)faces, F, (double*)workspace, F_dev);
-    k_reduce_partials<<<1, 256, 0, st>>>((const double*)workspace, blocks, (double*)out_f64);
+        T3D_CUDA(t3d_launch_dep(k_mesh_measure<int32_t>, blocks, 256, 0, st, (const float*)verts_f32, (const int32_t*)faces, F, (double*)workspace, F_dev));
+    T3D_CUDA(t3d_launch_dep(k_reduce_partials, 1, 256, 0, st, (const double*)workspace, blocks, (double*)out_f64));
     T3D_CHECK_LAUNCH("t3d_mesh_measure_dev");
     t3d_count_launches(2);
     return 0;
diff --git a/tomography_3d_reconstructor_b200/csrc/t3d_voxel.cu b/tomography_3d_reconstructor_b200/csrc/t3d_voxel.cu
--- a/tomography_3d_reconstructor_b200/csrc/t3d_voxel.cu
+++ b/tomography_3d_reconstructor_b200/csrc/t3d_voxel.cu
@@ -62,6 +62,7 @@
 __global__ void __launch_bounds__(256) k_pack_flat(const uint8_t* __restrict__ src, uint32_t* __restrict__ dst,
                                                    int64_t n_words, uint32_t thr4)
 {
+    t3d_dep_wait();
     const int64_t warp = ((int64_t)blockIdx.x * blockDim.x + threadIdx.x) >> 5;
     const int64_t n_warps = ((int64_t)gridDim.x * blockDim.x) >> 5;
     const uint32_t l = lane_id();
@@ -113,7 +114,7 @@
         const int64_t cap = (int64_t)T3D_NUM_SMS * 16;
         if (blocks > cap) blocks = cap;
         if (blocks < 1) blocks = 1;
-        k_pack_flat<<<(unsigned)blocks, 256, 0, st>>>((const uint8_t*)masks_u8, (uint32_t*)bits, n_words, thr4);
+        T3D_CUDA(t3d_launch_dep(k_pack_flat, (unsigned)blocks, 256, 0, st, (const uint8_t*)masks_u8, (uint32_t*)bits, n_words, thr4));
     } else {
         const int64_t n = rows * wpr;
         k_pack_generic<<<(unsigned)((n + 255) / 256), 256, 0, st>>>((const uint8_t*)masks_u8, (uint32_t*)bits, rows, W,
@@ -258,6 +259,7 @@
 __global__ void __launch_bounds__(FH_THREADS) k_fill_holes(uint32_t* bits_planes, int64_t plane_stride_words,
                                                            uint32_t* scratch, int H, int W, int nw)
 {
+    t3d_dep_wait();
     uint32_t* bits = bits_planes + (int64_t)blockIdx.x * plane_stride_words;
     const int64_t pw = (int64_t)H * nw;
     uint32_t* m = scratch + (int64_t)blockIdx.x * 2 * pw;
@@ -353,8 +355,8 @@
     const size_t smem = (size_t)(FH_THREADS / 32) * 2 * 32 * FH_PITCH * sizeof(uint32_t);
     if (t3d_first_use_on_device(T3D_ONCE_FILL_HOLES_ATTR))
         T3D_CUDA(cudaFuncSetAttribute(k_fill_holes, cudaFuncAttributeMaxDynamicSharedMemorySize, (int)smem));
-    k_fill_holes<<<n_planes, FH_THREADS, smem, (cudaStream_t)stream>>>((uint32_t*)bits, plane_stride_words,
-                                                                      (uint32_t*)scratch, H, W, t3d_wpr(W));
+    T3D_CUDA(t3d_launch_dep(k_fill_holes, n_planes, FH_THREADS, smem, (cudaStream_t)stream, (uint32_t*)bits, plane_stride_words,
+                                                                      (uint32_t*)scratch, H, W, t3d_wpr(W)));
     T3D_CHECK_LAUNCH("t3d_fill_holes_2d");
     t3d_count_launches(1);
     return 0;
@@ -456,6 +458,7 @@
 template <bool FULL>
 __global__ void __launch_bounds__(256) k_pack_gap(PackGapArgs a)
 {
+    t3d_dep_wait();
     __shared__ unsigned int s_cnt[PG_ZC];
     __shared__ unsigned int s_bb[6];
     const int tid = threadIdx.x, warp = tid >> 5;
@@ -555,6 +558,7 @@
 
 __global__ void __launch_bounds__(256) k_close_ends_fixup(EndsFixArgs a)
 {
+    t3d_dep_wait();
     const long long i = (long long)blockIdx.x * 256 + threadIdx.x;
     const long long pw = a.plane_words;
     const int Z = a.Z;
@@ -617,8 +621,8 @@
     a.skip_ends = skip_ends;
     a.counts = counts; a.bbox_t = bbox_t;
     dim3 grid((unsigned)((n_spans + 7) / 8), (unsigned)((Z + zc - 1) / zc));
-    if (a.plane_bytes % 1024 == 0) k_pack_gap<true><<<grid, 256, 0, st>>>(a);
-    else k_pack_gap<false><<<grid, 256, 0, st>>>(a);
+    if (a.plane_bytes % 1024 == 0) T3D_CUDA(t3d_launch_dep(k_pack_gap<true>, grid, 256, 0, st, a));
+    else T3D_CUDA(t3d_launch_dep(k_pack_gap<false>, grid, 256, 0, st, a));
     T3D_CHECK_LAUNCH("t3d_pack_gap");
     t3d_count_launches(1);
     return 0;
@@ -678,7 +682,7 @@
     a.Z = Z; a.plane_words = (long long)H * t3d_wpr(W); a.plane_bytes = (long long)H * W;
     a.thr4 = 0x01010101u * (uint32_t)threshold;
     a.counts = counts;
-    k_close_ends_fixup<<<(unsigned)((a.plane_words + 255) / 256), 256, 0, st>>>(a);
+    T3D_CUDA(t3d_launch_dep(k_close_ends_fixup, (unsigned)((a.plane_words + 255) / 256), 256, 0, st, a));
     T3D_CHECK_LAUNCH("t3d_close_ends_fixup");
     t3d_count_launches(1);
     return 0;
@@ -842,6 +846,7 @@
 
 __global__ void __launch_bounds__(512, 1) k_morph4(Morph4Args a)
 {
+    t3d_dep_wait();
     extern __shared__ __align__(16) uint32_t m4_smem[];
     __shared__ unsigned int s_cnt[M4_ZC_MAX];
     const int nw4 = a.nw4;
@@ -1026,7 +1031,7 @@
     if (t3d_first_use_on_device(T3D_ONCE_MORPH4_ATTR))
         T3D_CUDA(cudaFuncSetAttribute(k_morph4, cudaFuncAttributeMaxDynamicSharedMemorySize, 200 * 1024));
     dim3 grid(bands, (nz + zc - 1) / zc);
-    k_morph4<<<grid, threads, smem, st>>>(a);
+    T3D_CUDA(t3d_launch_dep(k_morph4, grid, threads, smem, st, a));
     T3D_CHECK_LAUNCH("t3d_morph4");
     t3d_count_launches(1);
     return 0;
```
